# tusen-ai/RangeDet

Measured on AMD Instinct MI355X. Metric: range-image frames/sec (64x2650, 8ch) at 1/2/4/8 GPU; Meta-Kernel HBM GB/s vs peak, higher is better.
Workload: dtype bf16

## Files before the change

__graft_entry__.py:

```python
import os
import sys

ROOT = os.path.dirname(os.path.abspath(__file__))
if ROOT not in sys.path:
    sys.path.insert(0, ROOT)


def build():
    from rangedet_amd import build as rdbuild
    rdbuild.build()
    if rdbuild.packed_swap_lint():
        rdbuild.build(force=True)
    bad = rdbuild.packed_swap_lint()
    assert not bad, "librangedet_hip.so: %d packed-fp32 instructions with swapped source halves, first %r" % (len(bad), bad[0])
    from oracle import cpu_ops
    cpu_ops.build(with_ref=True)
    import rangedet_amd
    from rangedet_amd import lib as rdlib
    rdlib.Lib(rdlib.DEFAULT_PATH)


def smoke():
    import numpy as np
    import torch
    from rangedet_amd import lib as rdlib, synth
    from rangedet_amd.pipeline import RangeDetPipeline
    from oracle import graph_ref, input_ref
    assert torch.cuda.is_available(), "smoke() needs a GPU"
    H, Wr, W, k = 16, 250, 256, 2000
    P = synth.make_weights(seed=18, width=W, cls_bias=-1.0)
    frame = input_ref.make_frame(0, W=Wr, pad_W=W, H=H)
    pipe = RangeDetPipeline(P, dtype=rdlib.RD_F32, feat_size=(H, Wr), pad_field=(H, W), pre_nms_top_n=k, wnms_cap=2048)
    res = pipe.run(frame)
    ref = graph_ref.forward(frame, P, num_fgs=k)
    sc = res["fg_cls_score"].cpu().numpy()
    bx = res["decoded_bbox"].cpu().numpy()
    valid = ref["fg_cls_score"] > 1e-6
    assert np.abs(sc - ref["fg_cls_score"]).max() < 1e-4, np.abs(sc - ref["fg_cls_score"]).max()
    gap = np.abs(np.diff(ref["fg_cls_score"][0]))
    ok = np.ones(k, bool)
    ok[1:] &= gap > 1e-5
    ok[:-1] &= gap > 1e-5
    ok &= valid[0]
    err = np.abs(bx[0][ok] - ref["decoded_bbox"][0][ok]).max()
    assert err < 1e-3, err
    dets, rows, keep, d8 = graph_ref.postprocess(sc[0], bx[0])
    got_keep = res["keep_inds"]
    assert list(got_keep) == list(keep), (len(got_keep), len(keep))
    print("smoke ok: %d detections kept of %d candidates; box maxerr %.2e" % (len(keep), dets.shape[0], err))
    pipe16 = RangeDetPipeline(P, dtype=rdlib.RD_BF16, feat_size=(H, Wr), pad_field=(H, W), pre_nms_top_n=k, wnms_cap=2048,
                              batch=2)
    batch = {kk: np.concatenate([v, v], 0) for kk, v in frame.items()}
    r16 = pipe16.run(batch)
    s16 = r16["fg_cls_score"].cpu().numpy()
    assert np.all(np.diff(s16, axis=1) <= 0) and np.array_equal(s16[0], s16[1])
    d16 = np.abs(s16[0] - ref["fg_cls_score"][0]).max()
    assert d16 < 0.05, d16
    print("smoke ok (bf16, batch 2): sorted-score maxdiff vs fp32 oracle %.3f, kept %s" %
          (d16, [len(f["keep_inds"]) for f in r16["frames"]]))


if __name__ == "__main__":
    build()
    if len(sys.argv) > 1 and sys.argv[1] == "smoke":
        smoke()
```

include/rangedet_hip.h:

```cpp
#ifndef RANGEDET_HIP_H_
#define RANGEDET_HIP_H_
#include <stddef.h>
#include <stdint.h>

#ifdef __cplusplus
extern "C" {
#endif

#define RD_OK 0
#define RD_EINVAL (-1)
#define RD_ESHAPE (-2)
#define RD_EWORKSPACE (-3)
#define RD_EHIP (-4)

#define RD_F32 0
#define RD_BF16 1
#define RD_F16 2

#define RD_RELU_PRE 1
#define RD_ADD 2
#define RD_RELU_POST 4
#define RD_SCALE_FOLDED 8
#define RD_MFMA16 16

int rd_version(void);
const char* rd_last_error_string(void);

int rd_nchw_to_nhwc(const float* src, void* dst, int B, int C, int H, int W, int dst_cstride, int dst_coff,
                    int zero_pad, int dst_dtype, void* stream);
int rd_nhwc_to_nchw(const void* src, float* dst, int B, int C, int H, int W, int src_cstride, int src_coff,
                    int src_dtype, void* stream);

int rd_copy_rows(const void* src, long src_row_bytes, void* dst, long dst_row_bytes, long dst_offset_bytes, long bytes,
                 int rows, void* stream);

size_t rd_conv_packed_bytes(int ntaps, int cin, int cout, int dtype);
int rd_pack_conv_weight_host(const float* w_oihw_host, int cout, int cin, int kh, int kw, int dtype,
                             void* packed_host);
int rd_deconv_phase_taps(int kh, int kw, int stride_w, int pad_w, int phase);
int rd_pack_deconv_weight_host(const float* w_iohw_host, int cin, int cout, int kh, int kw, int stride_w,
                               int pad_w, int phase, int dtype, void* packed_host);
int rd_pack_deconv_weight_folded_host(const float* w_iohw_host, const float* fold_scale_host, int cin, int cout, int kh, int kw,
                                      int stride_w, int pad_w, int phase, int dtype, void* packed_host);

int rd_conv2d_bn_act(const void* x, int x_cstride, int x_coff, const void* w_packed, const float* scale,
                     const float* shift, const void* residual, int r_cstride, int r_coff, void* y,
                     int y_cstride, int y_coff, int B, int H, int Win, int cin, int cout, int kh, int kw,
                     int stride_w, int flags, int dtype, void* stream);
size_t rd_conv3x3_ex_packed_bytes(int cin, int cout, int stride_w, int x_cstride);
int rd_pack_conv3x3_ex_host(const float* w_oihw_host, const float* fold_scale_host, int cout, int cin, int stride_w,
                            int x_cstride, int dtype, void* packed_host);
int rd_pack_conv3x3_m16_host(const float* w_oihw_host, const float* fold_scale_host, int cout, int cin, int dtype, void* packed_host);
int rd_conv3x3_mfma16_ok(int cin, int cout, int stride_w, int W, int fused_output_conv);
size_t rd_conv1x1_sc_packed_bytes(int cin, int cout);
int rd_pack_conv1x1_sc_host(const float* w_oi_host, const float* fold_scale_host, int cout, int cin, int dtype,
                            void* packed_host);
int rd_conv3x3_bn_act_ex(const void* x, int x_cstride, int x_coff, const void* w_packed, const float* scale, const float* shift,
                         const void* residual, int r_cstride, int r_coff, const void* sc_x, int sc_cstride, int sc_coff,
                         int sc_cin, const void* sc_w_packed, void* y, int y_cstride, int y_coff, int B, int H, int Win, int cin,
                         int cout, int stride_w, int flags, int dtype, void* stream);
size_t rd_block64_packed_bytes(int cin);
int rd_pack_block64_host(const float* w1_oihw_host, const float* fold_scale1_host, const float* w2_oihw_host,
                         const float* fold_scale2_host, int cin, int dtype, void* packed_host);
int rd_block64_bn_act(const void* x, int x_cstride, int x_coff, int cin, const void* w_packed, const float* shift1, const float* shift2,
                      const void* sc_w_packed, void* y, int y_cstride, int y_coff, int B, int H, int W, int dtype, void* stream);
int rd_pack_block64_m16_host(const float* w1_oihw_host, const float* fold_scale1_host, const float* w2_oihw_host,
                             const float* fold_scale2_host, int dtype, void* packed_host);
int rd_pack_conv1x1_sc_m16_host(const float* w_oi_host, const float* fold_scale_host, int dtype, void* packed_host);
int rd_block64_m16_bn_act(const void* x, int x_cstride, int x_coff, const void* w_packed, const float* shift1, const float* shift2,
                          const void* sc_w_packed, void* y, int y_cstride, int y_coff, int B, int H, int W, int dtype, void* stream);

size_t rd_head_packed_bytes(void);
int rd_pack_head_weight_host(const float* w, int nout, int cin, int dtype, void* out_host);
size_t rd_head_m16_packed_bytes(void);
int rd_pack_head_weight_m16_host(const float* w, int nout, int cin, int dtype, void* out_host);
int rd_conv2d_bn_act_head_out(const void* x, int x_cstride, int x_coff, const void* w_packed, const float* scale,
                              const float* shift, int B, int H, int W, int cin, int flags, const void* head_w_packed,
                              const float* head_bias, float* out, long out_batch_stride, long n_off, int nout, int dtype,
                              void* stream);

int rd_conv3x3_bn_act_pair(const void* x0, int x0_coff, const void* w0_packed, const float* shift0, void* y0, int y0_coff,
                           const void* x1, int x1_coff, const void* w1_packed, const float* shift1, void* y1, int y1_coff,
                           int x_cstride, int y_cstride, int B, int H, int W, int cin, int flags, int dtype, void* stream);
int rd_conv2d_bn_act_head_out_pair(const void* x0, int x0_coff, const void* w0_packed, const float* shift0, const void* head_w0_packed,
                                   const float* head_bias0, float* out0, long out0_batch_stride, int nout0,
                                   const void* x1, int x1_coff, const void* w1_packed, const float* shift1, const void* head_w1_packed,
                                   const float* head_bias1, float* out1, long out1_batch_stride, int nout1,
                                   int x_cstride, long n_off, int B, int H, int W, int cin, int flags, int dtype, void* stream);

size_t rd_conv3x3_cat_packed_bytes(int cin1, int cin2, int cout);
int rd_pack_conv3x3_cat_host(const float* w, const float* fold_scale, int cout, int cin1, int cin2, int dtype, void* out_host);
int rd_conv3x3_bn_act_cat(const void* x1, int x1_cstride, int x1_coff, int cin1, const void* x2, int x2_cstride, int x2_coff, int cin2,
                          const void* w_packed, const float* shift, void* y, int y_cstride, int y_coff, int B, int H, int W, int cout,
                          int flags, int dtype, void* stream);

int rd_deconv2d_bn_act(const void* x, int x_cstride, int x_coff, const void* w_packed_phase,
                       const float* scale, const float* shift, const void* residual, int r_cstride,
                       int r_coff, void* y, int y_cstride, int y_coff, int B, int H, int Win, int cin,
                       int cout, int kh, int kw, int stride_w, int pad_w, int phase, int flags, int dtype,
                       void* stream);

int rd_deconv2d_all_phases_ok(int kh, int kw, int stride_w, int pad_w, int cout, int dtype);
int rd_deconv2d_bn_act_all(const void* x, int x_cstride, int x_coff, const void* w_packed_all, long w_phase_bytes,
                           const float* shift, const void* residual, int r_cstride, int r_coff, void* y, int y_cstride,
                           int y_coff, int B, int H, int Win, int cin, int cout, int kh, int kw, int stride_w, int pad_w,
                           int flags, int dtype, void* stream);

int rd_deconv2d_phase_pairs_ok(int kh, int kw, int stride_w, int pad_w, int cout, int dtype);
int rd_pack_deconv_phase_pair_host(const void* phase_a, const void* phase_b, int cin, int dtype, void* out);
int rd_deconv2d_bn_act_pairs(const void* x, int x_cstride, int x_coff, const void* w_packed_pairs, long w_pair_bytes,
                             const float* shift2, const void* residual, int r_cstride, int r_coff, void* y, int y_cstride,
                             int y_coff, int B, int H, int Win, int cin, int cout, int kh, int kw, int stride_w, int pad_w,
                             int flags, int dtype, void* stream);

int rd_head_out(const void* x, int x_cstride, int x_coff, const float* w, const float* bias, float* out,
                long out_batch_stride, long n_off, int B, int H, int W, int cin, int nout, int dtype,
                void* stream);

size_t rd_meta_packed_bytes(int dtype);
int rd_pack_meta_host(const float* w0, const float* b0, const float* w1, const float* b1, const float* s1,
                      const float* t1, const float* agg, const float* s2, const float* t2, int dtype,
                      void* packed_host);
int rd_meta_kernel_fwd(const void* data, int d_cstride, int d_coff, const float* coord_nchw,
                       const void* packed, void* y, int y_cstride, int y_coff, int B, int H, int W, int dtype,
                       void* stream);

size_t rd_sorted_foreground_workspace_bytes(long N, long k);
int rd_sorted_foreground(const float* cls_score, const float* bbox_delta, const float* pc, const float* mask,
                         int B, long N, long k, int D, int apply_sigmoid, float* out_score, float* out_delta,
                         float* out_pc, int* out_idx, void* ws, size_t ws_bytes, void* stream);

int rd_decode3d_bbox(const float* bbox_delta, const float* pc, float* out, int B, long N, int box_type,
                     int is_bin, void* stream);

size_t rd_score_filter_workspace_bytes(long n);
int rd_score_filter_dets(const float* scores, const float* boxes10, long n, float min_score, float* dets,
                         int* d_count, void* ws, size_t ws_bytes, void* stream);
int rd_score_filter_dets_batched(const float* scores, long scores_bstride, const float* boxes10, long boxes_bstride,
                                 long n, float min_score, float* dets, long dets_bstride, int* d_count, void* ws,
                                 size_t ws_bytes, int B, void* stream);

#define RD_WNMS_MAX_K 65536
#define RD_TIE_STABLE 0
#define RD_TIE_REFERENCE 1
#define RD_WNMS_DIAG_NO_SKIP 0x100
#define RD_WNMS_DIAG_TILE_W(n) (((n) & 0xff) << 16)
#define RD_WNMS_DIAG_MERGE_LDS(n) (((n) & 0x7f) << 24)
size_t rd_wnms_workspace_bytes(int Kcap);
int rd_wnms_4c(const float* dets, int Kcap, const int* d_count, const int* order, int tie_order, float thresh,
               float thresh_vote, int is3d, int hash_scale, float* out_dets, int* keep, int* d_nkeep, void* ws,
               size_t ws_bytes, void* stream);
int rd_wnms_4c_batched(const float* dets, long dets_bstride, int Kcap, const int* d_count, const int* order,
                       long order_bstride, int tie_order, float thresh, float thresh_vote, int is3d, int hash_scale,
                       float* out_dets, long out_bstride, int* keep, long keep_bstride, int* d_nkeep, void* ws,
                       size_t ws_bytes, int B, void* stream);
int rd_single_overlap(const float* dets_a, const float* dets_b, long n, int is3d, float* out, void* stream);
int rd_wnms_pair_skippable(const float* dets_a, const float* dets_b, long n, unsigned char* out, void* stream);

int rd_edge_atan2f(const float* y, const float* x, long n, float* out, void* stream);

int rd_wnms_order_host(const float* dets_host, int K, int* order_host);

int rd_dets12_to_8(const float* dets12, int Mcap, const int* d_count, float* out8, void* stream);
int rd_dets12_to_8_batched(const float* dets12, long dets12_bstride, int Mcap, const int* d_count, float* out8,
                           long out8_bstride, int B, void* stream);

int rd_rotated_iou_8pt(const float* boxes1, const float* boxes2, float* ious, long n1, long n2, void* stream);
int rd_batch_rotated_iou(const float* proposal, int p_stride, const float* gt_bbox, float* iou_map, int* argmax, int B, long N,
                         int n_gt, void* stream);
int rd_batch_rotated_iou_3d(const float* proposal, int p_stride, const float* gt_bbox7, float* iou_map, int* argmax, int B, long N,
                            int n_gt, void* stream);
int rd_rotated_iou_7(const float* boxes1, const float* boxes2, float* ious, long n1, long n2, void* stream);
int rd_batch_max_iou(const float* proposals, int p_stride, const float* gt8, float* out, long n, int n_gt,
                     void* stream);

size_t rd_nms3d_workspace_bytes(long N, int B);
int rd_gather_keep_scores(const float* score, long score_bstride, int k, const int* keep_idx, int max_keep, float* out, int B,
                          void* stream);
int rd_nms3d(const float* boxes, int B, long N, float iou_thres, int max_keep, int normal_iou, int* keep_idx,
             float* bbox_after_nms, void* ws, size_t ws_bytes, void* stream);

int rd_assign3d_v2(const float* pc, const float* bbox, const float* bbox_center, const float* bbox_radius, const float* mask,
                   const float* is_in_nlz, long N, int M, float max_x, float min_x, float max_y, float min_y, float max_z,
                   float min_z, float max_dist, int* out, void* stream);
size_t rd_get_point_num_workspace_bytes(void);
int rd_get_point_num(const float* bbox_inds, long N, float* out, void* ws, size_t ws_bytes, void* stream);

typedef struct {
  float clip_lo[7], clip_hi[7];
  float mean[8], sd[8];
  float interval_lo[3], interval_hi[3];
} rd_input_norm_t;
int rd_input_transform(const float* range_image, const float* pc_vehicle_frame, const float* inclination,
                       const rd_input_norm_t* norm_host, int B, int H, int W, int Hp, int Wp, float* input_data,
                       float* coord_s1, float* pc_s1, float* pc_s2, float* pc_s4, float* mask_s1, float* mask_s2,
                       float* mask_s4, void* stream);

#define RD_PROF_CONV 0
#define RD_PROF_META 1
#define RD_PROF_HEAD_OUT 2
#define RD_PROF_SORT 3
#define RD_PROF_DECODE 4
#define RD_PROF_WNMS 5
#define RD_PROF_LAYOUT 6
#define RD_PROF_CONV3 7
#define RD_PROF_BLOCK 8
#define RD_PROF_NKINDS 9
int rd_prof_enable(int on);
int rd_prof_reset(void);
int rd_prof_get(int kind, double* total_ms, long* launches);

#ifdef __cplusplus
}
#endif
#endif
```

rangedet_amd/csrc/k_misc.h:

```cpp
#pragma once
#include "rd_common.h"

namespace rd {

template <int DT>
__global__ __launch_bounds__(256) void nchw_to_nhwc_kernel(const float* __restrict__ src, void* __restrict__ dst_, int C,
                                                           long HW, int cs, int coff, int cpad, long total) {
  using E = Elem<DT>;
  typename E::T* dst = (typename E::T*)dst_;
  const int ctot = C + cpad;
  for (long i = blockIdx.x * 256L + threadIdx.x; i < total; i += (long)gridDim.x * 256) {
    long p = i % HW;
    long rest = i / HW;
    int c = (int)(rest % ctot);
    long b = rest / ctot;
    float v = c < C ? src[(b * C + c) * HW + p] : 0.f;
    dst[(b * HW + p) * cs + coff + c] = E::from_f32(v);
  }
}
template <int DT, int NSLOT>
__global__ __launch_bounds__(256) void nchw_to_nhwc_px_kernel(const float* __restrict__ src, void* __restrict__ dst_, int C,
                                                              long HW, int cs, int coff, long npix) {
  using E = Elem<DT>;
  typename E::T* dst = (typename E::T*)dst_;
  for (long i = blockIdx.x * 256L + threadIdx.x; i < npix; i += (long)gridDim.x * 256) {
    const long b = i / HW, p = i - b * HW;
    typename E::T v[NSLOT * E::CH];
#pragma unroll
    for (int c = 0; c < NSLOT * E::CH; ++c) v[c] = E::from_f32(c < C ? src[(b * C + c) * HW + p] : 0.f);
    Slot16 pk[NSLOT];
    memcpy(pk, v, sizeof(pk));
#pragma unroll
    for (int u = 0; u < NSLOT; ++u) *(Slot16*)(dst + i * cs + coff + u * E::CH) = pk[u];
  }
}
template <int DT>
__global__ __launch_bounds__(256) void nhwc_to_nchw_kernel(const void* __restrict__ src_, float* __restrict__ dst, int C,
                                                           long HW, int cs, int coff, long total) {
  using E = Elem<DT>;
  const typename E::T* src = (const typename E::T*)src_;
  for (long i = blockIdx.x * 256L + threadIdx.x; i < total; i += (long)gridDim.x * 256) {
    long p = i % HW;
    long rest = i / HW;
    int c = (int)(rest % C);
    long b = rest / C;
    dst[(b * C + c) * HW + p] = E::to_f32(src[(b * HW + p) * cs + coff + c]);
  }
}

template <int DT, int NOUT>
__global__ __launch_bounds__(256) void head_out_kernel(const void* __restrict__ x_, int cs, int coff,
                                                       const float* __restrict__ w, const float* __restrict__ bias,
                                                       float* __restrict__ out, long out_bs, long n_off, long HW,
                                                       int cin) {
  using E = Elem<DT>;
  using T = typename E::T;
  __shared__ float wl[8 * 128];
  const T* x = (const T*)x_ + (size_t)blockIdx.y * HW * cs;
  for (int i = threadIdx.x; i < NOUT * cin; i += 256) wl[i] = w[i];
  __syncthreads();
  const int sub = threadIdx.x & 7;
  const int per = cin >> 3;
  const long npix_iter = (long)gridDim.x * 32;
  for (long p0 = blockIdx.x * 32L; p0 < HW; p0 += npix_iter) {
    long p = p0 + (threadIdx.x >> 3);
    float acc[NOUT];
#pragma unroll
    for (int o = 0; o < NOUT; ++o) acc[o] = 0.f;
    if (p < HW) {
      const T* px = x + p * cs + coff + sub * per;
      if ((per % E::CH) == 0) {
        for (int c0 = 0; c0 < per; c0 += E::CH) {
          const Slot16 raw = *(const Slot16*)(px + c0);
          T el[E::CH];
          memcpy(el, &raw, 16);
#pragma unroll
          for (int e = 0; e < E::CH; ++e) {
            const float v = E::to_f32(el[e]);
#pragma unroll
            for (int o = 0; o < NOUT; ++o) acc[o] += v * wl[o * cin + sub * per + c0 + e];
          }
        }
      } else {
        for (int c = 0; c < per; ++c) {
          float v = E::to_f32(px[c]);
#pragma unroll
          for (int o = 0; o < NOUT; ++o) acc[o] += v * wl[o * cin + sub * per + c];
        }
      }
    }
#pragma unroll
    for (int o = 0; o < NOUT; ++o) {
      acc[o] += __shfl_xor(acc[o], 1);
      acc[o] += __shfl_xor(acc[o], 2);
      acc[o] += __shfl_xor(acc[o], 4);
    }
    if (p < HW && sub == 0) {
      float* o_ = out + (size_t)blockIdx.y * out_bs + (n_off + p) * NOUT;
#pragma unroll
      for (int o = 0; o < NOUT; ++o) o_[o] = acc[o] + bias[o];
    }
  }
}

template <int NOUT, int DT = RD_BF16>
__global__ __launch_bounds__(256) void head_out_mfma_kernel(const bf16_t* __restrict__ x, int cs, int coff,
                                                            const float* __restrict__ w, const float* __restrict__ bias,
                                                            float* __restrict__ out, long out_bs, long n_off, long HW,
                                                            int cin) {
  __shared__ __attribute__((aligned(16))) unsigned char lds[4 * 8192];
  const int lane = threadIdx.x & 63, m = lane & 31, hi = lane >> 5, wv = threadIdx.x >> 6;
  unsigned char* img = lds + wv * 8192;
  const int nks = cin >> 4, nsl = cin >> 3;
  x += (size_t)blockIdx.y * HW * cs + coff;
  out += (size_t)blockIdx.y * out_bs + n_off * NOUT;
  s16x8 wh[8], wl[8];
#pragma unroll
  for (int ks = 0; ks < 8; ++ks) {
    unsigned short h[8], l[8];
#pragma unroll
    for (int j = 0; j < 8; ++j) {
      const float v = (m < NOUT && ks < nks) ? w[m * cin + ks * 16 + hi * 8 + j] : 0.f;
      h[j] = H16<DT>::from_f32(v);
      l[j] = H16<DT>::from_f32(v - H16<DT>::to_f32(h[j]));
    }
    memcpy(&wh[ks], h, 16);
    memcpy(&wl[ks], l, 16);
  }
  float bs[4];
#pragma unroll
  for (int r = 0; r < 4; ++r) bs[r] = 4 * hi + r < NOUT ? bias[4 * hi + r] : 0.f;
  const long ntile = (HW + 31) / 32;
  const long wave0 = (long)blockIdx.x * 4 + wv, nwave = (long)gridDim.x * 4;
  const int lp = lane >> 4, ls = lane & 15;
  auto load = [&](long tile, Slot16 (&v)[8]) {
#pragma unroll
    for (int it = 0; it < 8; ++it) {
      const long p = min(tile * 32 + it * 4 + lp, HW - 1);
      v[it] = ls < nsl ? *(const Slot16*)(x + p * cs + ls * 8) : Slot16{0u, 0u, 0u, 0u};
    }
  };
  Slot16 cur[8], nxt[8];
  if (wave0 < ntile) load(wave0, cur);
  for (long tile = wave0; tile < ntile; tile += nwave) {
    const bool more = tile + nwave < ntile;
    if (more) load(tile + nwave, nxt);
#pragma unroll
    for (int it = 0; it < 8; ++it) {
      const int pr = it * 4 + lp;
      *(Slot16*)(img + pr * 256 + ((ls ^ (pr & 15)) << 4)) = cur[it];
    }
    __builtin_amdgcn_wave_barrier();
    f32x16 acc;
#pragma unroll
    for (int r = 0; r < 16; ++r) acc[r] = 0.f;
#pragma unroll
    for (int ks = 0; ks < 8; ++ks) {
      const s16x8 b = *(const s16x8*)(img + m * 256 + (((2 * ks + hi) ^ (m & 15)) << 4));
      acc = H16<DT>::mfma(wl[ks], b, acc);
      acc = H16<DT>::mfma(wh[ks], b, acc);
    }
    __builtin_amdgcn_wave_barrier();
    const long p = tile * 32 + m;
    if (p < HW) {
      float* o = out + p * NOUT + 4 * hi;
#pragma unroll
      for (int r = 0; r < 4; ++r)
        if (4 * hi + r < NOUT) o[r] = acc[r] + bs[r];
    }
    if (more) {
#pragma unroll
      for (int it = 0; it < 8; ++it) cur[it] = nxt[it];
    }
  }
}

__global__ __launch_bounds__(256) void decode3d_kernel(const float* __restrict__ delta, const float* __restrict__ pc,
                                                       float* __restrict__ out, long n, int box_type, int is_bin) {
  long idx = blockIdx.x * 256L + threadIdx.x;
  if (idx >= n) return;
  const float* d = delta + idx * box_type;
  float pc_x = pc[idx * 3 + 0], pc_y = pc[idx * 3 + 1], pc_z = pc[idx * 3 + 2];
  float az = atan2f(pc_y, pc_x);
  float ca = cosf(az), sa = sinf(az);
  float dx, dy, width, length, height, z0, yaw_l;
  if (is_bin) {
    dx = d[0];
    dy = d[1];
    width = expf(d[3]);
    length = expf(d[4]);
    height = expf(d[5]);
    float cz = pc_z + d[2];
    z0 = (float)((double)cz - (double)height / 2.0);
    yaw_l = d[6] + az;
  } else {
    dx = d[0] * fabsf(d[0]);
    dy = d[1] * fabsf(d[1]);
    width = expf(d[2]);
    length = expf(d[3]);
    height = expf(d[7]);
    z0 = d[6];
    yaw_l = atan2f(d[5], d[4]) + az;
  }
  float dxl = dx * ca - dy * sa;
  float dyl = dx * sa + dy * ca;
  float cx = pc_x + dxl, cy = pc_y + dyl;
  float sy = sinf(yaw_l), cyw = cosf(yaw_l);
  float hl = (float)(0.5 * (double)length), hw = (float)(0.5 * (double)width);
  float hx[4] = {hl, -hl, -hl, hl};
  float hy[4] = {-hw, -hw, hw, hw};
  float* o = out + idx * 10;
#pragma unroll
  for (int k = 0; k < 4; ++k) {
    o[2 * k] = (hx[k] * cyw - hy[k] * sy) + cx;
    o[2 * k + 1] = (hx[k] * sy + hy[k] * cyw) + cy;
  }
  o[8] = z0;
  o[9] = z0 + height;
}

__global__ __launch_bounds__(256) void filter_count_kernel(const float* __restrict__ scores, long n, float thr,
                                                           int* __restrict__ blk_cnt, long sc_bs, long blk_bs) {
  scores += blockIdx.y * sc_bs;
  blk_cnt += blockIdx.y * blk_bs;
  long i = blockIdx.x * 256L + threadIdx.x;
  int p = (i < n) && (scores[i] > thr);
  unsigned long long m = __ballot(p);
  __shared__ int wc[4];
  if ((threadIdx.x & 63) == 0) wc[threadIdx.x >> 6] = __popcll(m);
  __syncthreads();
  if (threadIdx.x == 0) blk_cnt[blockIdx.x] = wc[0] + wc[1] + wc[2] + wc[3];
}
__global__ __launch_bounds__(256) void filter_scan_kernel(int* __restrict__ blk_cnt, int nblk, int* __restrict__ total,
                                                          long blk_bs) {
  blk_cnt += blockIdx.x * blk_bs;
  total += blockIdx.x;
  __shared__ int part[256];
  __shared__ int carry;
  if (threadIdx.x == 0) carry = 0;
  __syncthreads();
  for (int base = 0; base < nblk; base += 256) {
    int i = base + threadIdx.x;
    int v = i < nblk ? blk_cnt[i] : 0;
    part[threadIdx.x] = v;
    __syncthreads();
    for (int off = 1; off < 256; off <<= 1) {
      int t = threadIdx.x >= off ? part[threadIdx.x - off] : 0;
      __syncthreads();
      part[threadIdx.x] += t;
      __syncthreads();
    }
    int incl = part[threadIdx.x];
    if (i < nblk) blk_cnt[i] = carry + incl - v;
    __syncthreads();
    if (threadIdx.x == 255) carry += incl;
    __syncthreads();
  }
  if (threadIdx.x == 0) *total = carry;
}
__global__ __launch_bounds__(256) void filter_scatter_kernel(const float* __restrict__ scores,
                                                             const float* __restrict__ boxes10, long n, float thr,
                                                             const int* __restrict__ blk_off, float* __restrict__ dets,
                                                             long sc_bs, long box_bs, long blk_bs, long dets_bs) {
  scores += blockIdx.y * sc_bs;
  boxes10 += blockIdx.y * box_bs;
  blk_off += blockIdx.y * blk_bs;
  dets += blockIdx.y * dets_bs;
  long i = blockIdx.x * 256L + threadIdx.x;
  int p = (i < n) && (scores[i] > thr);
  unsigned long long m = __ballot(p);
  __shared__ int wc[4];
  const int wv = threadIdx.x >> 6, ln = threadIdx.x & 63;
  if (ln == 0) wc[wv] = __popcll(m);
  __syncthreads();
  int off = blk_off[blockIdx.x];
  for (int w = 0; w < wv; ++w) off += wc[w];
  if (p) {
    int pos = off + __popcll(m & ((1ull << ln) - 1ull));
    const float* b = boxes10 + i * 10;
    float* d = dets + (size_t)pos * 12;
#pragma unroll
    for (int k = 0; k < 8; ++k) d[k] = b[k];
    d[8] = fdlibm_atan2f(b[1] - b[3], b[0] - b[2]);
    d[9] = b[8];
    d[10] = b[9] - b[8];
    d[11] = scores[i];
  }
}

__global__ __launch_bounds__(256) void dets12_to_8_kernel(const float* __restrict__ d12, int cap, const int* __restrict__ d_count,
                                                          float* __restrict__ o8, long d12_bs, long o8_bs) {
  d12 += blockIdx.y * d12_bs;
  o8 += blockIdx.y * o8_bs;
  int i = blockIdx.x * 256 + threadIdx.x;
  int n = d_count ? min(d_count[blockIdx.y], cap) : cap;
  if (i >= n) return;
  const float* d = d12 + (size_t)i * 12;
  float* o = o8 + (size_t)i * 8;
  o[0] = (d[0] + d[2] + d[4] + d[6]) / 4.f;
  o[1] = (d[1] + d[3] + d[5] + d[7]) / 4.f;
  o[2] = d[9] + d[10] / 2.f;
  float ax = d[2] - d[0], ay = d[3] - d[1];
  float bx = d[2] - d[4], by = d[3] - d[5];
  o[3] = sqrtf(ax * ax + ay * ay);
  o[4] = sqrtf(bx * bx + by * by);
  o[5] = d[10];
  o[6] = d[8];
  o[7] = d[11];
}

__global__ __launch_bounds__(256) void gather_keep_scores_kernel(const float* __restrict__ score, long score_bs, int k,
                                                                 const int* __restrict__ keep, int mk, float* __restrict__ out) {
  const int i = blockIdx.x * 256 + threadIdx.x;
  if (i >= mk) return;
  const int q = keep[(size_t)blockIdx.y * mk + i];
  out[(size_t)blockIdx.y * mk + i] = (q >= 0 && q < k) ? score[blockIdx.y * score_bs + q] : -__builtin_inff();
}

}
```

rangedet_amd/csrc/k_sort.h:

```cpp
#pragma once
#include "rd_common.h"

namespace rd {

constexpr int SORT_TILE = 2048;

__device__ __forceinline__ unsigned desc_key(float f) {
  unsigned u = __float_as_uint(f);
  unsigned asc = u ^ ((u >> 31) ? 0xFFFFFFFFu : 0x80000000u);
  return ~asc;
}
__device__ __forceinline__ float key_to_float(unsigned key) {
  unsigned asc = ~key;
  unsigned u = (asc >> 31) ? (asc ^ 0x80000000u) : ~asc;
  return __uint_as_float(u);
}

__global__ __launch_bounds__(256) void sort_keygen_kernel(const float* __restrict__ score, const float* __restrict__ mask,
                                                          long N, int apply_sigmoid, unsigned* __restrict__ keys,
                                                          unsigned* __restrict__ idx, long ws_stride) {
  long i = blockIdx.x * 256L + threadIdx.x;
  if (i >= N) return;
  const long b = blockIdx.y;
  float s = score[b * N + i];
  if (apply_sigmoid) s = 1.0f / (1.0f + expf(-s));
  if (mask) s = s * mask[b * N + i];
  keys[b * ws_stride + i] = desc_key(s);
  idx[b * ws_stride + i] = (unsigned)i;
}
__global__ __launch_bounds__(256) void sort_keygen_dets_kernel(const float* __restrict__ dets, int cap,
                                                               const int* __restrict__ d_count, unsigned* __restrict__ keys,
                                                               unsigned* __restrict__ idx) {
  int i = blockIdx.x * 256 + threadIdx.x;
  if (i >= cap) return;
  int n = d_count ? min(*d_count, cap) : cap;
  keys[i] = i < n ? desc_key(dets[(size_t)i * 12 + 11]) : 0xFFFFFFFFu;
  idx[i] = (unsigned)i;
}

__global__ __launch_bounds__(256) void sort_hist_kernel(const unsigned* __restrict__ keys, long N, int shift,
                                                        unsigned* __restrict__ hist, unsigned* __restrict__ tot,
                                                        long ws_stride, const unsigned* __restrict__ d_n) {
  if (d_n) N = min(N, (long)d_n[blockIdx.y * ws_stride]);
  keys += blockIdx.y * ws_stride;
  hist += blockIdx.y * ws_stride;
  tot += blockIdx.y * ws_stride;
  __shared__ unsigned h[256];
  h[threadIdx.x] = 0;
  __syncthreads();
  long base = (long)blockIdx.x * SORT_TILE;
  for (int r = 0; r < SORT_TILE / 256; ++r) {
    long i = base + r * 256 + threadIdx.x;
    if (i < N) atomicAdd(&h[(keys[i] >> shift) & 255u], 1u);
  }
  __syncthreads();
  unsigned v = h[threadIdx.x];
  hist[(size_t)blockIdx.x * 256 + threadIdx.x] = v;
  if (v) atomicAdd(&tot[threadIdx.x], v);
}

__global__ __launch_bounds__(256) void sort_scatter_kernel(const unsigned* __restrict__ keys_in,
                                                           const unsigned* __restrict__ idx_in, long N, int shift,
                                                           const unsigned* __restrict__ hist,
                                                           const unsigned* __restrict__ tot,
                                                           unsigned* __restrict__ keys_out, unsigned* __restrict__ idx_out,
                                                           long ws_stride, const unsigned* __restrict__ d_n) {
  if (d_n) {
    N = min(N, (long)d_n[blockIdx.y * ws_stride]);
    if ((long)blockIdx.x * SORT_TILE >= N) return;
  }
  {
    const long o = blockIdx.y * ws_stride;
    keys_in += o; idx_in += o; hist += o; tot += o; keys_out += o; idx_out += o;
  }
  __shared__ unsigned wcnt[4][256];
  __shared__ unsigned gbase[256];
  __shared__ unsigned scan[256];
  const int tid = threadIdx.x, lane = tid & 63, wv = tid >> 6;
  for (int w = 0; w < 4; ++w) wcnt[w][tid] = 0;
  {
    unsigned t = tot[tid];
    scan[tid] = t;
    __syncthreads();
    for (int off = 1; off < 256; off <<= 1) {
      unsigned a = tid >= off ? scan[tid - off] : 0u;
      __syncthreads();
      scan[tid] += a;
      __syncthreads();
    }
    unsigned before = 0;
    for (unsigned b = 0; b < blockIdx.x; ++b) before += hist[(size_t)b * 256 + tid];
    gbase[tid] = scan[tid] - t + before;
  }
  __syncthreads();

  unsigned key[8], id[8], pos[8];
  const long base = (long)blockIdx.x * SORT_TILE + wv * 512;
  const unsigned long long lt = (1ull << lane) - 1ull;
#pragma unroll
  for (int r = 0; r < 8; ++r) {
    long i = base + r * 64 + lane;
    bool valid = i < N;
    key[r] = valid ? keys_in[i] : 0xFFFFFFFFu;
    id[r] = valid ? idx_in[i] : 0u;
    unsigned d = (key[r] >> shift) & 255u;
    unsigned long long peers = __ballot(valid);
#pragma unroll
    for (int bit = 0; bit < 8; ++bit) {
      unsigned long long bm = __ballot(valid && ((d >> bit) & 1u));
      peers &= ((d >> bit) & 1u) ? bm : ~bm;
    }
    unsigned rank = __popcll(peers & lt), cnt = __popcll(peers);
    unsigned prev = wcnt[wv][d];
    pos[r] = prev + rank;
    __builtin_amdgcn_wave_barrier();
    if (valid && rank == 0) wcnt[wv][d] = prev + cnt;
    __builtin_amdgcn_wave_barrier();
  }
  __syncthreads();
  {
    unsigned c0 = wcnt[0][tid], c1 = wcnt[1][tid], c2 = wcnt[2][tid];
    wcnt[0][tid] = 0;
    wcnt[1][tid] = c0;
    wcnt[2][tid] = c0 + c1;
    wcnt[3][tid] = c0 + c1 + c2;
  }
  __syncthreads();
#pragma unroll
  for (int r = 0; r < 8; ++r) {
    long i = base + r * 64 + lane;
    if (i < N) {
      unsigned d = (key[r] >> shift) & 255u;
      unsigned dst = gbase[d] + wcnt[wv][d] + pos[r];
      keys_out[dst] = key[r];
      idx_out[dst] = id[r];
    }
  }
}

__global__ __launch_bounds__(256) void sort_gather_kernel(const unsigned* __restrict__ keys, const unsigned* __restrict__ idx,
                                                          long k, int D, const float* __restrict__ delta,
                                                          const float* __restrict__ pc, float* __restrict__ out_score,
                                                          float* __restrict__ out_delta, float* __restrict__ out_pc,
                                                          int* __restrict__ out_idx, long ws_stride, long N) {
  long i = blockIdx.x * 256L + threadIdx.x;
  if (i >= k) return;
  {
    const long b = blockIdx.y;
    keys += b * ws_stride; idx += b * ws_stride;
    delta += b * N * D; pc += b * N * 3;
    out_score += b * k; out_delta += b * k * D; out_pc += b * k * 3;
    if (out_idx) out_idx += b * k;
  }
  unsigned j = idx[i];
  out_score[i] = key_to_float(keys[i]);
  for (int c = 0; c < D; ++c) out_delta[i * D + c] = delta[(size_t)j * D + c];
  out_pc[i * 3 + 0] = pc[(size_t)j * 3 + 0];
  out_pc[i * 3 + 1] = pc[(size_t)j * 3 + 1];
  out_pc[i * 3 + 2] = pc[(size_t)j * 3 + 2];
  if (out_idx) out_idx[i] = (int)j;
}

constexpr int SEL_BINS = 4096, SEL_SHIFT = 20;
__global__ __launch_bounds__(256) void select_hist_kernel(const unsigned* __restrict__ keys, long N, unsigned* __restrict__ h12,
                                                          long ws_stride) {
  keys += blockIdx.y * ws_stride; h12 += blockIdx.y * ws_stride;
  __shared__ unsigned h[SEL_BINS];
  for (int i = threadIdx.x; i < SEL_BINS; i += 256) h[i] = 0;
  __syncthreads();
  const long base = (long)blockIdx.x * SORT_TILE;
  for (int r = 0; r < SORT_TILE / 256; ++r) {
    const long i = base + r * 256 + threadIdx.x;
    if (i < N) atomicAdd(&h[keys[i] >> SEL_SHIFT], 1u);
  }
  __syncthreads();
  for (int i = threadIdx.x; i < SEL_BINS; i += 256)
    if (h[i]) atomicAdd(&h12[i], h[i]);
}
__global__ __launch_bounds__(256) void select_thresh_kernel(const unsigned* __restrict__ h12, long k, unsigned* __restrict__ sel,
                                                            long ws_stride) {
  h12 += blockIdx.y * ws_stride; sel += blockIdx.y * ws_stride;
  __shared__ unsigned part[256];
  const int tid = threadIdx.x;
  unsigned loc[SEL_BINS / 256], sum = 0;
#pragma unroll
  for (int j = 0; j < SEL_BINS / 256; ++j) { loc[j] = h12[tid * (SEL_BINS / 256) + j]; sum += loc[j]; }
  part[tid] = sum;
  __syncthreads();
  for (int off = 1; off < 256; off <<= 1) {
    const unsigned v = tid >= off ? part[tid - off] : 0u;
    __syncthreads();
    part[tid] += v;
    __syncthreads();
  }
  unsigned before = part[tid] - sum;
  if (tid == 255 && (k == 0 || part[255] < (unsigned)k)) { sel[0] = SEL_BINS - 1; sel[1] = part[255]; }
  if (before < (unsigned)k && before + sum >= (unsigned)k) {
#pragma unroll
    for (int j = 0; j < SEL_BINS / 256; ++j) {
      if (before < (unsigned)k && before + loc[j] >= (unsigned)k) { sel[0] = tid * (SEL_BINS / 256) + j; sel[1] = before + loc[j]; }
      before += loc[j];
    }
  }
}
__global__ __launch_bounds__(256) void select_count_kernel(const unsigned* __restrict__ keys, long N, const unsigned* __restrict__ sel,
                                                           unsigned* __restrict__ cnt, long ws_stride) {
  keys += blockIdx.y * ws_stride; sel += blockIdx.y * ws_stride; cnt += blockIdx.y * ws_stride;
  const unsigned T = sel[0];
  __shared__ unsigned c;
  if (threadIdx.x == 0) c = 0;
  __syncthreads();
  const long base = (long)blockIdx.x * SORT_TILE;
  unsigned mine = 0;
  for (int r = 0; r < SORT_TILE / 256; ++r) {
    const long i = base + r * 256 + threadIdx.x;
    if (i < N && (keys[i] >> SEL_SHIFT) <= T) ++mine;
  }
  if (mine) atomicAdd(&c, mine);
  __syncthreads();
  if (threadIdx.x == 0) cnt[blockIdx.x] = c;
}
__global__ __launch_bounds__(256) void select_compact_kernel(const unsigned* __restrict__ keys_in, const unsigned* __restrict__ idx_in,
                                                             long N, const unsigned* __restrict__ sel,
                                                             const unsigned* __restrict__ cnt, unsigned* __restrict__ keys_out,
                                                             unsigned* __restrict__ idx_out, long ws_stride) {
  {
    const long o = blockIdx.y * ws_stride;
    keys_in += o; idx_in += o; sel += o; cnt += o; keys_out += o; idx_out += o;
  }
  const unsigned T = sel[0];
  __shared__ unsigned wcnt[4][8], sbase;
  const int tid = threadIdx.x, lane = tid & 63, wv = tid >> 6;
  if (tid == 0) {
    unsigned b = 0;
    for (unsigned j = 0; j < blockIdx.x; ++j) b += cnt[j];
    sbase = b;
  }
  const long base = (long)blockIdx.x * SORT_TILE + wv * 512;
  unsigned key[8], id[8];
  unsigned long long m[8];
#pragma unroll
  for (int r = 0; r < 8; ++r) {
    const long i = base + r * 64 + lane;
    const bool valid = i < N;
    key[r] = valid ? keys_in[i] : 0xFFFFFFFFu;
    id[r] = valid ? idx_in[i] : 0u;
    m[r] = __ballot(valid && (key[r] >> SEL_SHIFT) <= T);
    if (lane == 0) wcnt[wv][r] = (unsigned)__popcll(m[r]);
  }
  __syncthreads();
  unsigned off = sbase;
  for (int w = 0; w < wv; ++w)
#pragma unroll
    for (int r = 0; r < 8; ++r) off += wcnt[w][r];
#pragma unroll
  for (int r = 0; r < 8; ++r) {
    if ((m[r] >> lane) & 1ull) {
      const unsigned dst = off + (unsigned)__popcll(m[r] & ((1ull << lane) - 1ull));
      keys_out[dst] = key[r];
      idx_out[dst] = id[r];
    }
    off += (unsigned)__popcll(m[r]);
  }
}

struct SortWs {
  unsigned *keysA, *keysB, *idxA, *idxB, *hist, *tot, *h12, *cnt, *sel;
  int nblk;
};
inline size_t sort_ws_bytes(long N) {
  long nblk = (N + SORT_TILE - 1) / SORT_TILE;
  return (size_t)(4 * N + nblk * 256 + 4 * 256 + SEL_BINS + nblk + 64) * 4 + 256;
}
inline SortWs sort_ws_carve(void* ws, long N) {
  SortWs s;
  s.nblk = (int)((N + SORT_TILE - 1) / SORT_TILE);
  unsigned* p = (unsigned*)ws;
  s.keysA = p; p += N;
  s.keysB = p; p += N;
  s.idxA = p; p += N;
  s.idxB = p; p += N;
  s.hist = p; p += (size_t)s.nblk * 256;
  s.tot = p; p += 4 * 256;
  s.h12 = p; p += SEL_BINS;
  s.cnt = p; p += s.nblk;
  s.sel = p;
  return s;
}
inline int sort_clear(const SortWs& s, hipStream_t st, int nb, long ws_stride, bool with_h12) {
  const size_t bytes = (size_t)(4 * 256 + (with_h12 ? SEL_BINS : 0)) * 4;
  const hipError_t e = nb > 1 ? hipMemset2DAsync(s.tot, (size_t)ws_stride * 4, 0, bytes, nb, st) : hipMemsetAsync(s.tot, 0, bytes, st);
  return e == hipSuccess ? RD_OK : fail(RD_EHIP, "sort: memset");
}
inline int radix_sort_pairs(const SortWs& s, long N, hipStream_t st, int nb = 1, long ws_stride = 0, const unsigned* d_n = nullptr,
                            bool cleared = false) {
  if (!cleared) { int rc = sort_clear(s, st, nb, ws_stride, false); if (rc != RD_OK) return rc; }
  unsigned *ki = s.keysA, *ko = s.keysB, *ii = s.idxA, *io = s.idxB;
  for (int pass = 0; pass < 4; ++pass) {
    hipLaunchKernelGGL(sort_hist_kernel, dim3(s.nblk, nb), dim3(256), 0, st, ki, N, pass * 8, s.hist, s.tot + pass * 256,
                       ws_stride, d_n);
    hipLaunchKernelGGL(sort_scatter_kernel, dim3(s.nblk, nb), dim3(256), 0, st, ki, ii, N, pass * 8, s.hist,
                       s.tot + pass * 256, ko, io, ws_stride, d_n);
    std::swap(ki, ko);
    std::swap(ii, io);
  }
  return check_launch("radix_sort_pairs");
}

inline int radix_topk_pairs(const SortWs& s, long N, long k, hipStream_t st, int nb, long ws_stride, unsigned** rk, unsigned** ri) {
  const bool off = dev_switches().sort_no_select;
  *rk = s.keysA; *ri = s.idxA;
  RD_REQUIRE(k > 0 && k <= N, RD_ESHAPE, "top-k: k %ld of N %ld", k, N);
  if (off || 2 * k > N) return radix_sort_pairs(s, N, st, nb, ws_stride);
  { int rc = sort_clear(s, st, nb, ws_stride, true); if (rc != RD_OK) return rc; }
  hipLaunchKernelGGL(select_hist_kernel, dim3(s.nblk, nb), dim3(256), 0, st, s.keysA, N, s.h12, ws_stride);
  hipLaunchKernelGGL(select_thresh_kernel, dim3(1, nb), dim3(256), 0, st, s.h12, k, s.sel, ws_stride);
  hipLaunchKernelGGL(select_count_kernel, dim3(s.nblk, nb), dim3(256), 0, st, s.keysA, N, s.sel, s.cnt, ws_stride);
  hipLaunchKernelGGL(select_compact_kernel, dim3(s.nblk, nb), dim3(256), 0, st, s.keysA, s.idxA, N, s.sel, s.cnt, s.keysB, s.idxB,
                     ws_stride);
  SortWs v = s;
  v.keysA = s.keysB; v.keysB = s.keysA; v.idxA = s.idxB; v.idxB = s.idxA;
  *rk = s.keysB; *ri = s.idxB;
  return radix_sort_pairs(v, N, st, nb, ws_stride, s.sel + 1, true);
}

}
```

rangedet_amd/csrc/rd_api.hip:

```cpp
#include "k_conv1.h"
#include "k_block.h"
#include "k_assign.h"
#include "k_input.h"
#include "k_nms3d.h"
#include "k_meta.h"
#include "k_misc.h"
#include "k_riou.h"
#include "k_sort.h"
#include "k_wnms.h"

#include <algorithm>
#include <string>
#include <numeric>

using namespace rd;

namespace rd {
inline size_t align256(size_t v) { return (v + 255) & ~(size_t)255; }
inline size_t wnms_ws_bytes(int cap) {
  const size_t nw = (size_t)(cap + 63) / 64;
  return align256((size_t)cap * PREP_F * 4) + 3 * align256((size_t)cap * nw * 8) + 4 * align256((size_t)cap * 4) +
         align256(((size_t)cap + 2) * 8 + 3 * ((size_t)cap / 32 + 2) * 4) + align256(nw * 8) + 256 + align256(sort_ws_bytes(cap)) + 256;
}
inline WnmsWs wnms_ws_carve(void* ws, int cap) {
// ... 340 lines not shown
  return RD_OK;
}
int rd_conv3x3_bn_act_cat(const void* x1, int x1_cstride, int x1_coff, int cin1, const void* x2, int x2_cstride, int x2_coff, int cin2,
                          const void* w_packed, const float* shift, void* y, int y_cstride, int y_coff, int B, int H, int W, int cout,
                          int flags, int dtype, void* stream) {
  RD_REQUIRE(x1 && x2 && w_packed && y && shift, RD_EINVAL, "conv3x3_cat: null pointer");
  RD_REQUIRE(is_h16(dtype), RD_EINVAL, "conv3x3_cat: dtype %d (RD_BF16 or RD_F16)", dtype);
  RD_REQUIRE((flags & RD_SCALE_FOLDED) && !(flags & RD_ADD), RD_EINVAL, "conv3x3_cat: needs RD_SCALE_FOLDED weights, takes no residual");
  RD_REQUIRE(B > 0 && H > 0 && W > 0 && (cout == 64 || cout == 128), RD_ESHAPE, "conv3x3_cat: shape / cout %d", cout);
  RD_REQUIRE(cin1 > 0 && cin1 % 32 == 0 && cin2 > 0 && cin2 % 8 == 0, RD_ESHAPE, "conv3x3_cat: cin1 %d (multiple of 32), cin2 %d (multiple of 8)", cin1, cin2);
  RD_REQUIRE(y_coff >= 0 && y_coff + cout <= y_cstride, RD_ESHAPE, "conv3x3_cat: y channels exceed stride");
  RD_REQUIRE(x1_cstride % 8 == 0 && x1_coff % 8 == 0 && x1_coff + cin1 <= x1_cstride && x2_cstride % 8 == 0 && x2_coff % 8 == 0 &&
             x2_coff + cin2 <= x2_cstride, RD_ESHAPE, "conv3x3_cat: channel stride/offset");
  const DevSwitches& sw_ = dev_switches();
  RD_REQUIRE(!sw_.conv_v1 && sw_.conv_wide && sw_.conv_w30 && (cout == 64 ? sw_.conv_th4 != 3 : (sw_.conv_th4 && sw_.conv_w30 == 2)), RD_ESHAPE,
             "conv3x3_cat: needs the 8 x 32 tile form of the persistent 3x3 kernel (a dev switch turned it off)");
  allow_conv_lds();
  Conv3Src2 s2;
  s2.x = x2; s2.cs = x2_cstride; s2.co = x2_coff; s2.cin1 = cin1; s2.cin2 = cin2;
  return launch_conv3(x1, x1_cstride, x1_coff, w_packed, nullptr, shift, nullptr, 0, 0, y, y_cstride, y_coff, B, H, W, cin1 + cin2, cout, flags,
                      1, (hipStream_t)stream, 0, nullptr, dtype, nullptr, nullptr, &s2, conv3_body_cat(cin1, cin2, true));
}

size_t rd_head_packed_bytes(void) { return 16384; }
int rd_pack_head_weight_host(const float* w, int nout, int cin, int dtype, void* out_host) {
  RD_REQUIRE(w && out_host, RD_EINVAL, "pack_head_weight: null pointer");
  RD_REQUIRE(is_h16(dtype), RD_EINVAL, "pack_head_weight: dtype %d (RD_BF16 or RD_F16)", dtype);
  RD_REQUIRE(nout >= 1 && nout <= 8 && cin >= 1 && cin <= 128, RD_ESHAPE, "pack_head_weight: nout %d (1..8), cin %d (1..128)", nout, cin);
  pack_head_frag(w, nout, cin, out_host, dtype);
  return RD_OK;
}
size_t rd_head_m16_packed_bytes(void) { return 8192; }
int rd_pack_head_weight_m16_host(const float* w, int nout, int cin, int dtype, void* out_host) {
  RD_REQUIRE(w && out_host, RD_EINVAL, "pack_head_weight_m16: null pointer");
  RD_REQUIRE(is_h16(dtype), RD_EINVAL, "pack_head_weight_m16: dtype %d (RD_BF16 or RD_F16)", dtype);
  RD_REQUIRE(nout >= 1 && nout <= 8 && cin >= 1 && cin <= 128, RD_ESHAPE, "pack_head_weight_m16: nout %d (1..8), cin %d (1..128)", nout, cin);
  pack_head_frag16(w, nout, cin, out_host, dtype);
  return RD_OK;
}
int rd_conv2d_bn_act_head_out(const void* x, int x_cstride, int x_coff, const void* w_packed, const float* scale,
                              const float* shift, int B, int H, int W, int cin, int flags, const void* head_w_packed,
                              const float* head_bias, float* out, long out_batch_stride, long n_off, int nout, int dtype,
                              void* stream) {
  RD_REQUIRE(x && w_packed && head_w_packed && head_bias && out, RD_EINVAL, "conv2d_head_out: null pointer");
  RD_REQUIRE(is_h16(dtype), RD_EINVAL, "conv2d_head_out: dtype %d (RD_BF16 or RD_F16)", dtype);
  RD_REQUIRE(B > 0 && H > 0 && W > 0 && cin > 0 && nout >= 1 && nout <= 8, RD_ESHAPE, "conv2d_head_out: shape / nout %d (1..8)", nout);
  RD_REQUIRE(!(flags & RD_ADD), RD_EINVAL, "conv2d_head_out: no residual in a head tower");
  RD_REQUIRE(x_cstride % 8 == 0 && x_coff % 8 == 0 && x_coff + cin_slots(cin, RD_BF16) * 8 <= x_cstride, RD_ESHAPE,
             "conv2d_head_out: x channel stride/offset");
  RD_REQUIRE(!dev_switches().conv_v1, RD_EINVAL, "conv2d_head_out: needs the persistent 3x3 kernel (RD_CONV_V1 is set)");
  RD_REQUIRE(!conv3_body_small(cin, (flags & RD_SCALE_FOLDED) != 0), RD_ESHAPE, "conv2d_head_out: cin %d (the packed image of a conv with <= 16 input channels is not this launch form's)", cin);
  const bool m16 = (flags & RD_MFMA16) != 0;
  RD_REQUIRE(!m16 || ((flags & RD_SCALE_FOLDED) && conv3_mfma16_ok(cin, 128, 1, W, true)), RD_ESHAPE,
             "conv2d_head_out: RD_MFMA16 (weights of rd_pack_conv3x3_m16_host) is not a launch form for cin %d at width %d (rd_conv3x3_mfma16_ok)", cin, W);
  allow_conv_lds();
  Conv3Args h;
  memset(&h, 0, sizeof(h));
  h.hw = (const unsigned char*)head_w_packed; h.hb = head_bias; h.ho = out; h.ho_bs = out_batch_stride; h.ho_off = n_off; h.hn = nout;
  return launch_conv3(x, x_cstride, x_coff, w_packed, scale, shift, nullptr, 0, 0, nullptr, 128, 0, B, H, W, cin, 128, flags & ~RD_MFMA16, 1,
                      (hipStream_t)stream, 0, &h, dtype, nullptr, nullptr, nullptr, m16 ? C3_BODY_M16 : 0);
}

static int pair_checks(const char* fn, const void* x0, const void* x1, const void* w0, const void* w1, const float* shift0,
                       const float* shift1, int x_cstride, int x0_coff, int x1_coff, int B, int H, int W, int cin, int flags,
                       int dtype) {
  RD_REQUIRE(x0 && x1 && w0 && w1 && shift0 && shift1, RD_EINVAL, "%s: null pointer", fn);
  RD_REQUIRE(is_h16(dtype), RD_EINVAL, "%s: dtype %d (RD_BF16 or RD_F16)", fn, dtype);
  RD_REQUIRE(B > 0 && H > 0 && W > 0 && cin > 0, RD_ESHAPE, "%s: shape", fn);
  RD_REQUIRE((flags & RD_SCALE_FOLDED) && !(flags & RD_ADD), RD_EINVAL, "%s: needs RD_SCALE_FOLDED weights, takes no residual", fn);
  RD_REQUIRE(x_cstride % 8 == 0 && x0_coff % 8 == 0 && x1_coff % 8 == 0 && x0_coff + cin_slots(cin, RD_BF16) * 8 <= x_cstride &&
             x1_coff + cin_slots(cin, RD_BF16) * 8 <= x_cstride, RD_ESHAPE, "%s: x channel stride/offset", fn);
  RD_REQUIRE(!dev_switches().conv_v1, RD_EINVAL, "%s: needs the persistent 3x3 kernel (RD_CONV_V1 is set)", fn);
  RD_REQUIRE(cin > 16, RD_ESHAPE, "%s: cin %d (more than 16 input channels)", fn, cin);
  return RD_OK;
}
int rd_conv3x3_bn_act_pair(const void* x0, int x0_coff, const void* w0_packed, const float* shift0, void* y0, int y0_coff,
                           const void* x1, int x1_coff, const void* w1_packed, const float* shift1, void* y1, int y1_coff,
                           int x_cstride, int y_cstride, int B, int H, int W, int cin, int flags, int dtype, void* stream) {
  if (int rc = pair_checks("conv3x3_pair", x0, x1, w0_packed, w1_packed, shift0, shift1, x_cstride, x0_coff, x1_coff, B, H, W, cin, flags, dtype)) return rc;
  RD_REQUIRE(y0 && y1, RD_EINVAL, "conv3x3_pair: null output");
  RD_REQUIRE(y0_coff >= 0 && y1_coff >= 0 && y0_coff + 128 <= y_cstride && y1_coff + 128 <= y_cstride, RD_ESHAPE, "conv3x3_pair: y channels exceed stride");
  allow_conv_lds();
  if (!conv3_pair_eligible(128, flags, W)) {
    if (int rc = launch_conv3(x0, x_cstride, x0_coff, w0_packed, nullptr, shift0, nullptr, 0, 0, y0, y_cstride, y0_coff, B, H, W, cin, 128,
                              flags, 1, (hipStream_t)stream, 0, nullptr, dtype)) return rc;
    return launch_conv3(x1, x_cstride, x1_coff, w1_packed, nullptr, shift1, nullptr, 0, 0, y1, y_cstride, y1_coff, B, H, W, cin, 128, flags, 1,
                        (hipStream_t)stream, 0, nullptr, dtype);
  }
  Conv3Second g;
  memset(&g, 0, sizeof(g));
  g.x = x1; g.x_co = x1_coff; g.w = w1_packed; g.shift = shift1; g.y = y1; g.y_co = y1_coff;
  return launch_conv3(x0, x_cstride, x0_coff, w0_packed, nullptr, shift0, nullptr, 0, 0, y0, y_cstride, y0_coff, B, H, W, cin, 128, flags, 1,
                      (hipStream_t)stream, 0, nullptr, dtype, &g);
}
int rd_conv2d_bn_act_head_out_pair(const void* x0, int x0_coff, const void* w0_packed, const float* shift0, const void* head_w0_packed,
                                   const float* head_bias0, float* out0, long out0_batch_stride, int nout0,
                                   const void* x1, int x1_coff, const void* w1_packed, const float* shift1, const void* head_w1_packed,
                                   const float* head_bias1, float* out1, long out1_batch_stride, int nout1,
                                   int x_cstride, long n_off, int B, int H, int W, int cin, int flags, int dtype, void* stream) {
  if (int rc = pair_checks("conv2d_head_out_pair", x0, x1, w0_packed, w1_packed, shift0, shift1, x_cstride, x0_coff, x1_coff, B, H, W, cin, flags, dtype)) return rc;
  RD_REQUIRE(head_w0_packed && head_w1_packed && head_bias0 && head_bias1 && out0 && out1, RD_EINVAL, "conv2d_head_out_pair: null pointer");
  RD_REQUIRE(nout0 >= 1 && nout0 <= 8 && nout1 >= 1 && nout1 <= 8, RD_ESHAPE, "conv2d_head_out_pair: nout %d / %d (1..8)", nout0, nout1);
  allow_conv_lds();
  Conv3Args h;
  memset(&h, 0, sizeof(h));
  h.hw = (const unsigned char*)head_w0_packed; h.hb = head_bias0; h.ho = out0; h.ho_bs = out0_batch_stride; h.ho_off = n_off; h.hn = nout0;
  if (!conv3_pair_eligible(128, flags, W, true)) {
    if (int rc = launch_conv3(x0, x_cstride, x0_coff, w0_packed, nullptr, shift0, nullptr, 0, 0, nullptr, 128, 0, B, H, W, cin, 128, flags, 1,
                              (hipStream_t)stream, 0, &h, dtype)) return rc;
    h.hw = (const unsigned char*)head_w1_packed; h.hb = head_bias1; h.ho = out1; h.ho_bs = out1_batch_stride; h.hn = nout1;
    return launch_conv3(x1, x_cstride, x1_coff, w1_packed, nullptr, shift1, nullptr, 0, 0, nullptr, 128, 0, B, H, W, cin, 128, flags, 1,
                        (hipStream_t)stream, 0, &h, dtype);
  }
  Conv3Second g;
  memset(&g, 0, sizeof(g));
  g.x = x1; g.x_co = x1_coff; g.w = w1_packed; g.shift = shift1;
  g.hw = head_w1_packed; g.hb = head_bias1; g.ho = out1; g.ho_bs = out1_batch_stride; g.hn = nout1;
  return launch_conv3(x0, x_cstride, x0_coff, w0_packed, nullptr, shift0, nullptr, 0, 0, nullptr, 128, 0, B, H, W, cin, 128, flags, 1,
                      (hipStream_t)stream, 0, &h, dtype, &g);
}

int rd_deconv2d_bn_act(const void* x, int x_cstride, int x_coff, const void* w_packed_phase, const float* scale,
                       const float* shift, const void* residual, int r_cstride, int r_coff, void* y, int y_cstride,
                       int y_coff, int B, int H, int Win, int cin, int cout, int kh, int kw, int stride_w, int pad_w,
                       int phase, int flags, int dtype, void* stream) {
  RD_REQUIRE(x && w_packed_phase && y, RD_EINVAL, "deconv2d: null pointer");
  RD_REQUIRE(kh == 3, RD_ESHAPE, "deconv2d: kernel height %d (only 3, pad 1, stride 1)", kh);
  RD_REQUIRE(stride_w >= 1 && phase >= 0 && phase < stride_w, RD_EINVAL, "deconv2d: phase %d of stride %d", phase, stride_w);
  RD_REQUIRE(y_coff >= 0 && y_coff + cout <= y_cstride, RD_ESHAPE, "deconv2d: y channels exceed stride");
  const int Wout = (Win - 1) * stride_w - 2 * pad_w + kw;
  RD_REQUIRE(Wout > phase, RD_ESHAPE, "deconv2d: empty phase");
  const int Wq = (Wout - phase + stride_w - 1) / stride_w;
  TapList tl = deconv_taps_sorted(kh, kw, stride_w, pad_w, phase);
  RD_REQUIRE(tl.n >= 1 && tl.n <= 9, RD_ESHAPE, "deconv2d: %d taps per phase unsupported", tl.n);
  allow_conv_lds();
  if (deconv_embeds_3x3(tl)) {
    const int ts = deconv_tap_set(tl);
    if (!ts) tl = conv_taps(3, 3);
    if (is_h16(dtype) && Wout == stride_w * Win && (cout == 64 || cout == 128) && !dev_switches().conv_v1 &&
        conv3_has_form(dtype, (flags & RD_SCALE_FOLDED) != 0)) {
      const bf16_t* r = (const bf16_t*)residual;
      return launch_conv3(x, x_cstride, x_coff, w_packed_phase, scale, shift, r, r_cstride * stride_w,
                          r_coff + phase * r_cstride, y, y_cstride * stride_w, y_coff + phase * y_cstride, B, H, Win, cin,
                          cout, flags, 1, (hipStream_t)stream, ts, nullptr, dtype);
    }
  }
  RD_REQUIRE(!(flags & RD_SCALE_FOLDED), RD_ESHAPE, "deconv2d: RD_SCALE_FOLDED needs the persistent 3x3 kernel (bf16, cout 64/128, "
             "taps inside the 3x3 window, Wout == stride_w * Win)");
  return launch_conv(tl, x, x_cstride, x_coff, w_packed_phase, scale, shift, residual, r_cstride, r_coff, y,
                     y_cstride, y_coff, B, H, Win, Wq, Wout, cin, cout, 1, stride_w, phase, flags, dtype,
                     (hipStream_t)stream);
}

int rd_deconv2d_all_phases_ok(int kh, int kw, int stride_w, int pad_w, int cout, int dtype) {
  if (!is_h16(dtype) || kh != 3 || stride_w < 2 || stride_w > 8 || !conv3_phases_eligible(cout, RD_SCALE_FOLDED)) return 0;
  if (kw - 2 * pad_w != stride_w) return 0;
  for (int p = 0; p < stride_w; ++p)
    if (!deconv_tap_set(deconv_taps_sorted(kh, kw, stride_w, pad_w, p))) return 0;
  return 1;
}
int rd_deconv2d_bn_act_all(const void* x, int x_cstride, int x_coff, const void* w_packed_all, long w_phase_bytes,
                           const float* shift, const void* residual, int r_cstride, int r_coff, void* y, int y_cstride,
                           int y_coff, int B, int H, int Win, int cin, int cout, int kh, int kw, int stride_w, int pad_w,
                           int flags, int dtype, void* stream) {
  RD_REQUIRE(x && w_packed_all && y, RD_EINVAL, "deconv2d_all: null pointer");
  RD_REQUIRE(is_h16(dtype), RD_EINVAL, "deconv2d_all: dtype %d (RD_BF16 or RD_F16)", dtype);
  RD_REQUIRE(flags & RD_SCALE_FOLDED, RD_EINVAL, "deconv2d_all: needs RD_SCALE_FOLDED weights (rd_pack_deconv_weight_folded_host)");
  RD_REQUIRE(!((flags & RD_ADD) && !residual), RD_EINVAL, "deconv2d_all: RD_ADD without residual");
  RD_REQUIRE(B > 0 && H > 0 && Win > 0 && cin > 0, RD_ESHAPE, "deconv2d_all: shape");
  RD_REQUIRE(y_coff >= 0 && y_coff + cout <= y_cstride, RD_ESHAPE, "deconv2d_all: y channels exceed stride");
  RD_REQUIRE(x_cstride % 8 == 0 && x_coff % 8 == 0 && x_coff + cin_slots(cin, RD_BF16) * 8 <= x_cstride, RD_ESHAPE, "deconv2d_all: x channel stride/offset");
  RD_REQUIRE(rd_deconv2d_all_phases_ok(kh, kw, stride_w, pad_w, cout, dtype), RD_ESHAPE,
             "deconv2d_all: kernel (%d,%d) stride %d pad %d cout %d is not a set of two-column 3x2 phases (use rd_deconv2d_bn_act per phase)",
             kh, kw, stride_w, pad_w, cout);
  RD_REQUIRE(w_phase_bytes >= (long)conv_packed_bytes(6, cin, cout, RD_BF16) && w_phase_bytes % 16 == 0, RD_EINVAL, "deconv2d_all: w_phase_bytes");
  allow_conv_lds();
  Conv3Phases ph;
  ph.nph = stride_w; ph.ts_mask = 0; ph.y_pc = y_cstride; ph.r_pc = r_cstride; ph.w_pb = w_phase_bytes;
  for (int p = 0; p < stride_w; ++p)
    if (deconv_tap_set(deconv_taps_sorted(kh, kw, stride_w, pad_w, p)) == 2) ph.ts_mask |= 1 << p;
  return launch_conv3(x, x_cstride, x_coff, w_packed_all, nullptr, shift, residual, r_cstride * stride_w, r_coff, y, y_cstride * stride_w,
                      y_coff, B, H, Win, cin, cout, flags, 1, (hipStream_t)stream, 3, nullptr, dtype, nullptr, &ph);
}

int rd_deconv2d_phase_pairs_ok(int kh, int kw, int stride_w, int pad_w, int cout, int dtype) {
  if (!rd_deconv2d_all_phases_ok(kh, kw, stride_w, pad_w, cout, dtype) || cout != 64 || stride_w % 2) return 0;
  if (!rd_deconv2d_all_phases_ok(kh, kw, stride_w, pad_w, 128, dtype)) return 0;
  for (int p = 0; p < stride_w; p += 2)
    if (deconv_tap_set(deconv_taps_sorted(kh, kw, stride_w, pad_w, p)) != deconv_tap_set(deconv_taps_sorted(kh, kw, stride_w, pad_w, p + 1))) return 0;
  return 1;
}
int rd_pack_deconv_phase_pair_host(const void* phase_a, const void* phase_b, int cin, int dtype, void* out) {
  RD_REQUIRE(phase_a && phase_b && out, RD_EINVAL, "pack_deconv_pair: null pointer");
  RD_REQUIRE(is_h16(dtype) && cin > 0, RD_EINVAL, "pack_deconv_pair: dtype %d / cin %d", dtype, cin);
  const size_t body = conv_packed_body_bytes(6, cin, 64, RD_BF16), blocks = body / 2048;
  for (size_t i = 0; i < blocks; ++i) {
    memcpy((unsigned char*)out + i * 4096, (const unsigned char*)phase_a + i * 2048, 2048);
    memcpy((unsigned char*)out + i * 4096 + 2048, (const unsigned char*)phase_b + i * 2048, 2048);
  }
  memset((unsigned char*)out + 2 * body, 0, 2 * RD_CONV_TAIL);
  return RD_OK;
}
int rd_deconv2d_bn_act_pairs(const void* x, int x_cstride, int x_coff, const void* w_packed_pairs, long w_pair_bytes,
                             const float* shift2, const void* residual, int r_cstride, int r_coff, void* y, int y_cstride,
                             int y_coff, int B, int H, int Win, int cin, int cout, int kh, int kw, int stride_w, int pad_w,
                             int flags, int dtype, void* stream) {
  RD_REQUIRE(x && w_packed_pairs && y && shift2, RD_EINVAL, "deconv2d_pairs: null pointer");
  RD_REQUIRE(is_h16(dtype), RD_EINVAL, "deconv2d_pairs: dtype %d (RD_BF16 or RD_F16)", dtype);
  RD_REQUIRE(flags & RD_SCALE_FOLDED, RD_EINVAL, "deconv2d_pairs: needs RD_SCALE_FOLDED weights (rd_pack_deconv_weight_folded_host)");
  RD_REQUIRE(!((flags & RD_ADD) && !residual), RD_EINVAL, "deconv2d_pairs: RD_ADD without residual");
  RD_REQUIRE(B > 0 && H > 0 && Win > 0 && cin > 0, RD_ESHAPE, "deconv2d_pairs: shape");
  RD_REQUIRE(x_cstride % 8 == 0 && x_coff % 8 == 0 && x_coff + cin_slots(cin, RD_BF16) * 8 <= x_cstride, RD_ESHAPE, "deconv2d_pairs: x channel stride/offset");
  RD_REQUIRE(rd_deconv2d_phase_pairs_ok(kh, kw, stride_w, pad_w, cout, dtype), RD_ESHAPE,
             "deconv2d_pairs: kernel (%d,%d) stride %d pad %d cout %d has no phase pairs (use rd_deconv2d_bn_act_all)", kh, kw, stride_w, pad_w, cout);
  RD_REQUIRE(y_cstride == cout && y_coff == 0 && (!residual || (r_cstride == cout && r_coff == 0)), RD_ESHAPE,
             "deconv2d_pairs: the output / residual must be dense %d-channel tensors (two phases are one 128-channel write)", cout);
  RD_REQUIRE(w_pair_bytes >= (long)conv_packed_bytes(6, cin, 2 * cout, RD_BF16) && w_pair_bytes % 16 == 0, RD_EINVAL, "deconv2d_pairs: w_pair_bytes");
  allow_conv_lds();
  Conv3Phases ph;
  ph.nph = stride_w / 2; ph.ts_mask = 0; ph.y_pc = 2 * cout; ph.r_pc = 2 * cout; ph.w_pb = w_pair_bytes;
  for (int p = 0; p < stride_w; p += 2)
    if (deconv_tap_set(deconv_taps_sorted(kh, kw, stride_w, pad_w, p)) == 2) ph.ts_mask |= 1 << (p / 2);
  return launch_conv3(x, x_cstride, x_coff, w_packed_pairs, nullptr, shift2, residual, r_cstride * stride_w, r_coff, y, y_cstride * stride_w,
                      y_coff, B, H, Win, cin, 2 * cout, flags, 1, (hipStream_t)stream, 3, nullptr, dtype, nullptr, &ph);
}

int rd_head_out(const void* x, int x_cstride, int x_coff, const float* w, const float* bias, float* out,
                long out_batch_stride, long n_off, int B, int H, int W, int cin, int nout, int dtype, void* stream) {
  RD_REQUIRE(x && w && bias && out, RD_EINVAL, "head_out: null pointer");
  RD_REQUIRE(cin % 8 == 0 && cin <= 128 && cin > 0, RD_ESHAPE, "head_out: cin %d (multiple of 8, <= 128)", cin);
  RD_REQUIRE(nout == 1 || nout == 7 || nout == 8, RD_ESHAPE, "head_out: nout %d not in {1,7,8}", nout);
  RD_REQUIRE(dtype == RD_F32 || is_h16(dtype), RD_EINVAL, "head_out: dtype");
  hipStream_t st = (hipStream_t)stream;
  const long HW = (long)H * W;
  dim3 grid((unsigned)std::min<long>((HW + 31) / 32, 4096), B);
  ProfScope ps(RD_PROF_HEAD_OUT, st);
  if (is_h16(dtype) && nout > 1 && cin % 16 == 0 && x_cstride % 8 == 0 && x_coff % 8 == 0) {
    dim3 g2((unsigned)std::min<long>((HW + 127) / 128, 2048), B);
#define RD_HOM(NO, DT_) hipLaunchKernelGGL((head_out_mfma_kernel<NO, DT_>), g2, dim3(256), 0, st, (const bf16_t*)x, x_cstride, x_coff, w, bias, out, out_batch_stride, n_off, HW, cin)
    if (dtype == RD_F16) { if (nout == 7) RD_HOM(7, RD_F16); else RD_HOM(8, RD_F16); }
    else { if (nout == 7) RD_HOM(7, RD_BF16); else RD_HOM(8, RD_BF16); }
#undef RD_HOM
    return check_launch("head_out");
  }
#define RD_HO(DT, NO) hipLaunchKernelGGL((head_out_kernel<DT, NO>), grid, dim3(256), 0, st, x, x_cstride, x_coff, w, bias, out, out_batch_stride, n_off, HW, cin)
  if (dtype == RD_BF16) { if (nout == 1) RD_HO(RD_BF16, 1); else if (nout == 7) RD_HO(RD_BF16, 7); else RD_HO(RD_BF16, 8); }
  else if (dtype == RD_F16) { if (nout == 1) RD_HO(RD_F16, 1); else if (nout == 7) RD_HO(RD_F16, 7); else RD_HO(RD_F16, 8); }
  else { if (nout == 1) RD_HO(RD_F32, 1); else if (nout == 7) RD_HO(RD_F32, 7); else RD_HO(RD_F32, 8); }
#undef RD_HO
  return check_launch("head_out");
}

size_t rd_meta_packed_bytes(int dtype) { return meta_layout(dtype).total; }
int rd_pack_meta_host(const float* w0, const float* b0, const float* w1, const float* b1, const float* s1,
                      const float* t1, const float* agg, const float* s2, const float* t2, int dtype, void* out) {
  RD_REQUIRE(w0 && b0 && w1 && b1 && s1 && t1 && agg && s2 && t2 && out, RD_EINVAL, "pack_meta: null pointer");
  RD_REQUIRE(dtype == RD_F32 || is_h16(dtype), RD_EINVAL, "pack_meta: dtype");
  pack_meta(w0, b0, w1, b1, s1, t1, agg, s2, t2, dtype, out);
  return RD_OK;
}
int rd_meta_kernel_fwd(const void* data, int d_cstride, int d_coff, const float* coord_nchw, const void* packed,
                       void* y, int y_cstride, int y_coff, int B, int H, int W, int dtype, void* stream) {
  RD_REQUIRE(data && coord_nchw && packed && y, RD_EINVAL, "meta_kernel: null pointer");
  RD_REQUIRE(B > 0 && H > 0 && W > 0, RD_ESHAPE, "meta_kernel: empty shape");
  RD_REQUIRE(dtype == RD_F32 || is_h16(dtype), RD_EINVAL, "meta_kernel: dtype");
  const int ch = ch_per_slot(dtype);
  RD_REQUIRE(d_cstride % ch == 0 && d_coff % ch == 0 && y_cstride % ch == 0 && y_coff % ch == 0, RD_ESHAPE,
             "meta_kernel: channel strides/offsets must be 16-byte multiples");
  RD_REQUIRE(d_coff + 64 <= d_cstride && y_coff + 64 <= y_cstride, RD_ESHAPE, "meta_kernel: needs 64 channels");
  hipStream_t st = (hipStream_t)stream;
  MetaArgs a;
  a.data = data; a.d_cs = d_cstride; a.d_co = d_coff; a.coord = coord_nchw; a.packed = (const unsigned char*)packed;
  a.y = y; a.y_cs = y_cstride; a.y_co = y_coff; a.B = B; a.H = H; a.W = W;
  constexpr int WAVES = 8;
  a.tiles_h = (H + WAVES - 1) / WAVES;
  a.tiles_w = (W + 31) / 32;
  a.ntiles = B * a.tiles_h * a.tiles_w;
  a.r0 = 0; a.m0 = a.m1 = a.m2 = 0;
  const size_t consts = 9 * 64 * 4 * 2 + 1024;
  ProfScope ps(RD_PROF_META, st);
  if (is_h16(dtype)) {
    const size_t lds = meta_layout(dtype).wbytes + consts + (size_t)(WAVES + 2) * 34 * 128 + 4096;
    static std::atomic<unsigned long long> seen{0};
    once_per_device(seen, [] { allow_big_lds(meta16_kernel<WAVES, RD_BF16>); allow_big_lds(meta16_kernel<WAVES, RD_F16>); });
    const dim3 mgrid(std::min(a.ntiles, conv_num_cus())), mblock(WAVES * 64);
    const int strips = a.tiles_w * B;
    a.r0 = dev_switches().conv_xcd && strips % 8 == 0 ? 8 : strips;
    RD_REQUIRE((unsigned long long)a.ntiles * (unsigned)std::max(a.r0, std::max(a.tiles_h, a.tiles_w)) < (1ull << 32), RD_ESHAPE,
               "meta_kernel: %d tiles exceed the range of the tile decode", a.ntiles);
    a.m0 = meta_magic(a.r0); a.m1 = meta_magic(a.tiles_h); a.m2 = meta_magic(a.tiles_w);
    RD_REQUIRE((long)H * W < (1l << 23) && (long)H * W * d_cstride < (1l << 31) && W < (1 << 23) && d_cstride < (1 << 23), RD_ESHAPE,
               "meta_kernel: image of %d x %d pixels x %d channels exceeds the 32-bit halo offsets", H, W, d_cstride);
    if (dtype == RD_F16) hipLaunchKernelGGL((meta16_kernel<WAVES, RD_F16>), mgrid, mblock, lds, st, a);
    else hipLaunchKernelGGL((meta16_kernel<WAVES, RD_BF16>), mgrid, mblock, lds, st, a);
  } else {
    const size_t lds = consts + (size_t)(WAVES + 2) * 34 * 256;
    static std::atomic<unsigned long long> seen32{0};
    once_per_device(seen32, [] { allow_big_lds(meta_kernel<RD_F32, WAVES>); });
    hipLaunchKernelGGL((meta_kernel<RD_F32, WAVES>), dim3(std::min(a.ntiles, 512)), dim3(WAVES * 64), lds, st, a);
  }
  return check_launch("meta_kernel");
}

size_t rd_sorted_foreground_workspace_bytes(long N, long k) { (void)k; return (sort_ws_bytes(N) + 256 + 255) & ~(size_t)255; }
int rd_sorted_foreground(const float* cls_score, const float* bbox_delta, const float* pc, const float* mask, int B,
                         long N, long k, int D, int apply_sigmoid, float* out_score, float* out_delta, float* out_pc,
                         int* out_idx, void* ws, size_t ws_bytes, void* stream) {
  RD_REQUIRE(cls_score && bbox_delta && pc && out_score && out_delta && out_pc && ws, RD_EINVAL, "sorted_foreground: null pointer");
  RD_REQUIRE(B > 0 && N > 0 && k > 0 && D > 0, RD_ESHAPE, "sorted_foreground: empty shape");
  RD_REQUIRE(N >= k, RD_ESHAPE, "sorted_foreground: N (%ld) < num_fgs (%ld)", N, k);
  RD_REQUIRE(N < (1L << 31), RD_ESHAPE, "sorted_foreground: N too large");
  RD_REQUIRE(ws_bytes >= rd_sorted_foreground_workspace_bytes(N, k), RD_EWORKSPACE, "sorted_foreground: workspace %zu < %zu",
             ws_bytes, rd_sorted_foreground_workspace_bytes(N, k));
  hipStream_t st = (hipStream_t)stream;
  void* wsa = (void*)(((uintptr_t)ws + 255) & ~(uintptr_t)255);
  SortWs s = sort_ws_carve(wsa, N);
  ProfScope ps(RD_PROF_SORT, st);
  const size_t per = rd_sorted_foreground_workspace_bytes(N, k);
  const bool wide = ws_bytes >= per * (size_t)B;
  const long stride = wide ? (long)(per / 4) : 0;
  const int nb = wide ? B : 1;
  for (int b0 = 0; b0 < B; b0 += nb) {
    hipLaunchKernelGGL(sort_keygen_kernel, dim3((unsigned)((N + 255) / 256), nb), dim3(256), 0, st, cls_score + (size_t)b0 * N,
                       mask ? mask + (size_t)b0 * N : nullptr, N, apply_sigmoid, s.keysA, s.idxA, stride);
    unsigned *rk, *ri;
    int rc = radix_topk_pairs(s, N, k, st, nb, stride, &rk, &ri);
    if (rc != RD_OK) return rc;
    hipLaunchKernelGGL(sort_gather_kernel, dim3((unsigned)((k + 255) / 256), nb), dim3(256), 0, st, rk, ri, k, D,
                       bbox_delta + (size_t)b0 * N * D, pc + (size_t)b0 * N * 3, out_score + (size_t)b0 * k,
                       out_delta + (size_t)b0 * k * D, out_pc + (size_t)b0 * k * 3, out_idx ? out_idx + (size_t)b0 * k : nullptr,
                       stride, N);
  }
  return check_launch("sorted_foreground");
}

int rd_decode3d_bbox(const float* bbox_delta, const float* pc, float* out, int B, long N, int box_type, int is_bin,
                     void* stream) {
  RD_REQUIRE(bbox_delta && pc && out, RD_EINVAL, "decode3d: null pointer");
  RD_REQUIRE(B > 0 && N > 0, RD_ESHAPE, "decode3d: empty shape");
  RD_REQUIRE((is_bin && box_type == 7) || (!is_bin && box_type == 8), RD_ESHAPE,
             "decode3d: box_type %d with is_bin=%d (8 for regular, 7 for bin)", box_type, is_bin);
  hipStream_t st = (hipStream_t)stream;
  const long n = (long)B * N;
  ProfScope ps(RD_PROF_DECODE, st);
  hipLaunchKernelGGL(decode3d_kernel, dim3((unsigned)((n + 255) / 256)), dim3(256), 0, st, bbox_delta, pc, out, n, box_type, is_bin);
  return check_launch("decode3d");
}

size_t rd_score_filter_workspace_bytes(long n) { return (size_t)((n + 255) / 256 + 8) * 4 + 256; }
int rd_score_filter_dets_batched(const float* scores, long scores_bstride, const float* boxes10, long boxes_bstride,
                                 long n, float min_score, float* dets, long dets_bstride, int* d_count, void* ws,
                                 size_t ws_bytes, int B, void* stream) {
  RD_REQUIRE(scores && boxes10 && dets && d_count && ws, RD_EINVAL, "score_filter: null pointer");
  RD_REQUIRE(n > 0 && B > 0, RD_ESHAPE, "score_filter: empty input");
  const size_t per = rd_score_filter_workspace_bytes(n);
  RD_REQUIRE(ws_bytes >= per * (size_t)B, RD_EWORKSPACE, "score_filter: workspace %zu < %zu", ws_bytes, per * (size_t)B);
  hipStream_t st = (hipStream_t)stream;
  int* blk = (int*)(((uintptr_t)ws + 255) & ~(uintptr_t)255);
  const int nblk = (int)((n + 255) / 256);
  const long blk_bs = nblk + 8;
  ProfScope ps(RD_PROF_WNMS, st);
  hipLaunchKernelGGL(filter_count_kernel, dim3(nblk, B), dim3(256), 0, st, scores, n, min_score, blk, scores_bstride, blk_bs);
  hipLaunchKernelGGL(filter_scan_kernel, dim3(B), dim3(256), 0, st, blk, nblk, d_count, blk_bs);
  hipLaunchKernelGGL(filter_scatter_kernel, dim3(nblk, B), dim3(256), 0, st, scores, boxes10, n, min_score, blk, dets,
                     scores_bstride, boxes_bstride, blk_bs, dets_bstride);
  return check_launch("score_filter");
}
int rd_score_filter_dets(const float* scores, const float* boxes10, long n, float min_score, float* dets, int* d_count,
                         void* ws, size_t ws_bytes, void* stream) {
  return rd_score_filter_dets_batched(scores, 0, boxes10, 0, n, min_score, dets, 0, d_count, ws, ws_bytes, 1, stream);
}

size_t rd_wnms_workspace_bytes(int Kcap) { return Kcap > 0 ? wnms_ws_bytes(Kcap) : 0; }
int rd_wnms_4c_batched(const float* dets, long dets_bstride, int Kcap, const int* d_count, const int* order,
                       long order_bstride, int tie_order, float thresh, float thresh_vote, int is3d, int hash_scale,
                       float* out_dets, long out_bstride, int* keep, long keep_bstride, int* d_nkeep, void* ws,
                       size_t ws_bytes, int B, void* stream) {
  RD_REQUIRE(dets && out_dets && keep && d_nkeep && ws, RD_EINVAL, "wnms_4c: null pointer");
  RD_REQUIRE(Kcap > 0 && Kcap <= RD_WNMS_MAX_K, RD_ESHAPE, "wnms_4c: Kcap %d not in [1, %d]", Kcap, RD_WNMS_MAX_K);
  RD_REQUIRE(B > 0, RD_ESHAPE, "wnms_4c: batch %d", B);
  const int diag = tie_order & ~0xff;
  tie_order &= 0xff;
  RD_REQUIRE(tie_order == RD_TIE_STABLE || tie_order == RD_TIE_REFERENCE, RD_EINVAL, "wnms_4c: tie_order %d", tie_order);
  RD_REQUIRE(!(diag & ~(RD_WNMS_DIAG_NO_SKIP | (0xff << 16) | (0x7f << 24))), RD_EINVAL, "wnms_4c: unknown diagnostic bits 0x%x", diag);
  const size_t per = rd_wnms_workspace_bytes(Kcap);
  RD_REQUIRE(ws_bytes >= per * (size_t)B, RD_EWORKSPACE, "wnms_4c: workspace %zu < %zu", ws_bytes, per * (size_t)B);
  RD_REQUIRE(order || B == 1 || tie_order == RD_TIE_REFERENCE, RD_EINVAL,
             "wnms_4c: the batched call needs an explicit processing order or RD_TIE_REFERENCE");
  hipStream_t st = (hipStream_t)stream;
  static std::atomic<unsigned long long> seen_lds{0};
  once_per_device(seen_lds, [] {
    allow_big_lds(wnms_tie_order_kernel); allow_big_lds(wnms_scan_kernel); allow_big_lds(wnms_scan4_kernel); allow_big_lds(wnms_merge_kernel);
  });
  WnmsWs w = wnms_ws_carve(ws, Kcap);
  ProfScope ps(RD_PROF_WNMS, st);
  WnmsBatch bs;
  bs.dets = dets_bstride; bs.order = order_bstride; bs.prep = (long)(per / 4); bs.words = (long)(per / 8);
  bs.ints = (long)(per / 4); bs.keep = keep_bstride; bs.out = out_bstride;
  const int* ord = order;
  if (!ord && tie_order == RD_TIE_REFERENCE) {
    const size_t lds = TIE_STACK_BYTES + (Kcap <= TIE_LDS_K ? (size_t)Kcap * 8 + 3 * ((size_t)Kcap / 32 + 2) * 4 : 0);
    hipLaunchKernelGGL(wnms_tie_order_kernel, dim3(1, 1, B), dim3(256), lds, st, dets, Kcap, d_count, w.order, bs, (long)(per / 4),
                       w.scratch);
    ord = w.order;
    bs.order = (long)(per / 4);
  } else if (!ord) {
    void* swa = (void*)(((uintptr_t)w.sort_ws + 255) & ~(uintptr_t)255);
    SortWs s = sort_ws_carve(swa, Kcap);
    hipLaunchKernelGGL(sort_keygen_dets_kernel, dim3((Kcap + 255) / 256), dim3(256), 0, st, dets, Kcap, d_count, s.keysA, s.idxA);
    int rc = radix_sort_pairs(s, Kcap, st);
    if (rc != RD_OK) return rc;
    if (hipMemcpyAsync(w.order, s.idxA, (size_t)Kcap * 4, hipMemcpyDeviceToDevice, st) != hipSuccess)
      return rd::fail(RD_EHIP, "wnms_4c: order copy");
    ord = w.order;
    bs.order = 0;
  }
  const int nb = (Kcap + 63) / 64;
  hipLaunchKernelGGL(wnms_prep_kernel, dim3((Kcap + 255) / 256, 1, B), dim3(256), 0, st, dets, ord, Kcap, d_count, w.prep, bs,
                     (float)hash_scale, w.novf);
  const int e_tw = (diag >> 16) & 0xff, e_ml = (diag >> 24) & 0x7f;
  const int tile_w = std::min(w.nwcap, e_tw ? std::max(1, e_tw) : 256);
  const size_t scan_lds = ((size_t)w.nwcap + (size_t)64 * tile_w) * 8;
  const int R1 = 256, nb1 = R1 / 64;
  const bool one_round = dev_switches().wnms_one_round;
  const bool two = Kcap >= 4 * R1 && !one_round;
  const int ct = dev_switches().wnms_ct == 32 ? 32 : dev_switches().wnms_ct == 16 ? 16 : 8;
  const int pgrid = std::min(2048, std::max(64, nb * (64 / ct) * std::min(nb, 16)));
  const int allow_skip = thresh >= 1e-3f && thresh_vote >= 1e-3f && !is3d && !dev_switches().wnms_no_skip && !(diag & RD_WNMS_DIAG_NO_SKIP);
  auto pairs = [&](const int* rows, const int* nrows, const unsigned long long* supp, int rb_end) {
    auto k = dev_switches().wnms_bal ? (ct == 8 ? wnms_pairs_kernel<8, true> : ct == 16 ? wnms_pairs_kernel<16, true> : wnms_pairs_kernel<32, true>)
                                     : (ct == 8 ? wnms_pairs_kernel<8, false> : ct == 16 ? wnms_pairs_kernel<16, false> : wnms_pairs_kernel<32, false>);
    hipLaunchKernelGGL(k, dim3(pgrid, 1, B), dim3(64), 0, st, w.prep, Kcap, d_count, thresh, thresh_vote, is3d, w.thr, w.vote,
                       w.nwcap, bs, rows, nrows, supp, 0, rb_end, allow_skip);
  };
  pairs(nullptr, nullptr, nullptr, two ? nb1 : nb);
  const bool scan4 = w.nwcap <= 128 && !e_tw && !dev_switches().wnms_scan1;
  const int tile_words = 64 * 128;
  const size_t scan4_lds = ((size_t)w.nwcap + tile_words) * 8;
  auto scan = [&](int c_begin, int c_end, unsigned long long* state) {
    if (scan4)
      hipLaunchKernelGGL(wnms_scan4_kernel, dim3(1, 1, B), dim3(256), scan4_lds, st, w.thr, w.snap, Kcap, d_count, w.nwcap, ord,
                         w.keep_q, keep, d_nkeep, bs, c_begin, c_end, state, tile_words);
    else
      hipLaunchKernelGGL(wnms_scan_kernel, dim3(1, 1, B), dim3(64), scan_lds, st, w.thr, w.snap, Kcap, d_count, w.nwcap, ord,
                         w.keep_q, keep, d_nkeep, bs, c_begin, c_end, state, tile_w);
  };
  scan(0, two ? nb1 : nb, two ? w.supp_state : (unsigned long long*)nullptr);
  if (two) {
    hipLaunchKernelGGL(wnms_alive_kernel, dim3(1, 1, B), dim3(256), 0, st, w.supp_state, Kcap, d_count, R1, w.alive, w.nalive, bs);
    pairs((const int*)w.alive, (const int*)w.nalive, (const unsigned long long*)w.supp_state, 0);
    scan(nb1, nb, w.supp_state);
  }
  const int lds_cap = std::min(Kcap + 2, e_ml ? std::max(4, e_ml) : 2048);
  hipLaunchKernelGGL(wnms_merge_kernel, dim3(std::min(Kcap, 4096), 1, B), dim3(64), (size_t)lds_cap * 8, st, dets, ord, w.vote,
                     w.snap, Kcap, d_count, w.nwcap, w.keep_q, d_nkeep, out_dets, bs, lds_cap, w.ovf, w.novf);
  if (Kcap + 2 > lds_cap)
    hipLaunchKernelGGL(wnms_merge_big_kernel, dim3(1, 1, B), dim3(64), 0, st, dets, ord, w.vote, w.snap, Kcap, d_count, w.nwcap,
                       w.keep_q, out_dets, bs, (const int*)w.ovf, (const int*)w.novf, w.scratch);
  return check_launch("wnms_4c");
}
int rd_wnms_4c(const float* dets, int Kcap, const int* d_count, const int* order, int tie_order, float thresh,
               float thresh_vote, int is3d, int hash_scale, float* out_dets, int* keep, int* d_nkeep, void* ws,
               size_t ws_bytes, void* stream) {
  return rd_wnms_4c_batched(dets, 0, Kcap, d_count, order, 0, tie_order, thresh, thresh_vote, is3d, hash_scale, out_dets, 0,
                            keep, 0, d_nkeep, ws, ws_bytes, 1, stream);
}
int rd_single_overlap(const float* dets_a, const float* dets_b, long n, int is3d, float* out, void* stream) {
  RD_REQUIRE(n >= 0 && (n == 0 || (dets_a && dets_b && out)), RD_EINVAL, "single_overlap: bad arguments");
  if (n == 0) return RD_OK;
  hipLaunchKernelGGL(single_overlap_kernel, dim3((unsigned)((n + 63) / 64)), dim3(64), 0, (hipStream_t)stream, dets_a, dets_b, n,
                     is3d, out);
  return check_launch("single_overlap");
}
int rd_wnms_pair_skippable(const float* dets_a, const float* dets_b, long n, unsigned char* out, void* stream) {
  RD_REQUIRE(dets_a && dets_b && out && n >= 0, RD_EINVAL, "wnms_pair_skippable: null pointer");
  if (n == 0) return RD_OK;
  hipLaunchKernelGGL(pair_skippable_kernel, dim3((unsigned)((n + 63) / 64)), dim3(64), 0, (hipStream_t)stream, dets_a, dets_b, n, out);
  return check_launch("wnms_pair_skippable");
}
namespace rd {
__global__ void atan2f_kernel(const float* y, const float* x, long n, float* out) {
  const long i = (long)blockIdx.x * blockDim.x + threadIdx.x;
  if (i < n) out[i] = fdlibm_atan2f(y[i], x[i]);
}
}
int rd_edge_atan2f(const float* y, const float* x, long n, float* out, void* stream) {
  RD_REQUIRE(y && x && out && n >= 0, RD_EINVAL, "edge_atan2f: null pointer");
  if (n == 0) return RD_OK;
  hipLaunchKernelGGL(atan2f_kernel, dim3((unsigned)((n + 255) / 256)), dim3(256), 0, (hipStream_t)stream, y, x, n, out);
  return check_launch("edge_atan2f");
}
int rd_wnms_order_host(const float* dets_host, int K, int* order_host) {
  RD_REQUIRE(K >= 0 && (K == 0 || (dets_host && order_host)), RD_EINVAL, "wnms_order_host: bad arguments");
  std::iota(order_host, order_host + K, 0);
  std::sort(order_host, order_host + K, [&](int i, int j) { return dets_host[i * 12 + 11] > dets_host[j * 12 + 11]; });
  return RD_OK;
}

int rd_dets12_to_8_batched(const float* dets12, long dets12_bstride, int Mcap, const int* d_count, float* out8,
                           long out8_bstride, int B, void* stream) {
  RD_REQUIRE(dets12 && out8, RD_EINVAL, "dets12_to_8: null pointer");
  RD_REQUIRE(Mcap > 0 && B > 0, RD_ESHAPE, "dets12_to_8: empty input");
  hipLaunchKernelGGL(dets12_to_8_kernel, dim3((Mcap + 255) / 256, B), dim3(256), 0, (hipStream_t)stream, dets12, Mcap, d_count,
                     out8, dets12_bstride, out8_bstride);
  return check_launch("dets12_to_8");
}
int rd_dets12_to_8(const float* dets12, int Mcap, const int* d_count, float* out8, void* stream) {
  return rd_dets12_to_8_batched(dets12, 0, Mcap, d_count, out8, 0, 1, stream);
}

int rd_gather_keep_scores(const float* score, long score_bstride, int k, const int* keep_idx, int max_keep, float* out, int B,
                          void* stream) {
  RD_REQUIRE(score && keep_idx && out, RD_EINVAL, "gather_keep_scores: null pointer");
  RD_REQUIRE(k > 0 && max_keep > 0 && B > 0, RD_ESHAPE, "gather_keep_scores: empty input");
  hipLaunchKernelGGL(gather_keep_scores_kernel, dim3((max_keep + 255) / 256, B), dim3(256), 0, (hipStream_t)stream, score,
                     score_bstride, k, keep_idx, max_keep, out);
  return check_launch("gather_keep_scores");
}

int rd_rotated_iou_8pt(const float* boxes1, const float* boxes2, float* ious, long n1, long n2, void* stream) {
  RD_REQUIRE(boxes1 && boxes2 && ious, RD_EINVAL, "rotated_iou: null pointer");
  RD_REQUIRE(n1 > 0 && n2 > 0, RD_ESHAPE, "rotated_iou: empty input");
  hipLaunchKernelGGL(riou8_kernel, dim3((unsigned)((n1 * n2 + 255) / 256)), dim3(256), 0, (hipStream_t)stream, boxes1, boxes2, ious, n1, n2);
  return check_launch("rotated_iou_8pt");
}
int rd_batch_rotated_iou(const float* proposal, int p_stride, const float* gt_bbox, float* iou_map, int* argmax, int B, long N,
                         int n_gt, void* stream) {
  RD_REQUIRE(proposal && gt_bbox && iou_map, RD_EINVAL, "batch_rotated_iou: null pointer");
  RD_REQUIRE(B > 0 && B <= 65535 && N > 0 && n_gt > 0 && n_gt <= 256 && p_stride >= 8, RD_ESHAPE,
             "batch_rotated_iou: B %d, N %ld, n_gt %d (<= 256), proposal row %d floats (>= 8)", B, N, n_gt, p_stride);
  hipLaunchKernelGGL(batch_riou_kernel, dim3((unsigned)((N + 255) / 256), B), dim3(256), 0, (hipStream_t)stream, proposal, p_stride,
                     N * (long)p_stride, gt_bbox, (long)n_gt * 8, iou_map, argmax, N, n_gt);
  return check_launch("batch_rotated_iou");
}
int rd_rotated_iou_7(const float* boxes1, const float* boxes2, float* ious, long n1, long n2, void* stream) {
  RD_REQUIRE(boxes1 && boxes2 && ious, RD_EINVAL, "rotated_iou_7: null pointer");
  if (n1 * n2 == 0) return RD_OK;
  hipLaunchKernelGGL(riou7_kernel, dim3((unsigned)((n1 * n2 + 255) / 256)), dim3(256), 0, (hipStream_t)stream, boxes1, boxes2, ious, n1, n2);
  return check_launch("rotated_iou_7");
}
int rd_batch_rotated_iou_3d(const float* proposal, int p_stride, const float* gt_bbox7, float* iou_map, int* argmax, int B, long N,
                            int n_gt, void* stream) {
  RD_REQUIRE(proposal && gt_bbox7 && iou_map, RD_EINVAL, "batch_rotated_iou_3d: null pointer");
  RD_REQUIRE(B > 0 && N > 0 && p_stride >= 10, RD_ESHAPE, "batch_rotated_iou_3d: proposal rows need the 8 corners + z0, z1 (stride %d)", p_stride);
  RD_REQUIRE(n_gt >= 1 && n_gt <= 256, RD_ESHAPE, "batch_rotated_iou_3d: n_gt %d (1..256; the config pads to 200)", n_gt);
  ProfScope ps(RD_PROF_DECODE, (hipStream_t)stream);
  hipLaunchKernelGGL(batch_riou3d_kernel, dim3((unsigned)((N + 255) / 256), B), dim3(256), 0, (hipStream_t)stream, proposal, p_stride,
                     (long)N * p_stride, gt_bbox7, (long)n_gt * 7, iou_map, argmax, N, n_gt);
  return check_launch("batch_rotated_iou_3d");
}
int rd_batch_max_iou(const float* proposals, int p_stride, const float* gt8, float* out, long n, int n_gt, void* stream) {
  return rd_batch_rotated_iou(proposals, p_stride, gt8, out, nullptr, 1, n, n_gt, stream);
}

size_t rd_nms3d_workspace_bytes(long N, int B) {
  if (N <= 0 || N > (1 << 18) || B <= 0) return 0;
  return nms3d_frame_bytes((int)N) * (size_t)B;
}
int rd_nms3d(const float* boxes, int B, long N, float iou_thres, int max_keep, int normal_iou, int* keep_idx,
             float* bbox_after_nms, void* ws, size_t ws_bytes, void* stream) {
  RD_REQUIRE(boxes && keep_idx && bbox_after_nms && ws, RD_EINVAL, "nms3d: null pointer");
  RD_REQUIRE(B > 0 && B <= 65535 && N > 0 && N <= (1 << 18) && max_keep > 0, RD_ESHAPE, "nms3d: B %d, N %ld (<= 262144), max_keep %d", B, N, max_keep);
  RD_REQUIRE(ws_bytes >= rd_nms3d_workspace_bytes(N, B), RD_EWORKSPACE, "nms3d: workspace %zu < %zu bytes", ws_bytes, rd_nms3d_workspace_bytes(N, B));
  RD_REQUIRE(((uintptr_t)ws & 7) == 0, RD_EINVAL, "nms3d: workspace must be 8-byte aligned");
  Nms3dArgs a;
  a.boxes = boxes; a.ws = (unsigned char*)ws; a.ws_frame = nms3d_frame_bytes((int)N);
  a.keep = keep_idx; a.out = bbox_after_nms;
  a.N = (int)N; a.ncw = (int)((N + 63) / 64); a.max_keep = max_keep; a.normal_iou = normal_iou ? 1 : 0; a.thresh = iou_thres;
  hipStream_t st = (hipStream_t)stream;
  ProfScope ps(RD_PROF_WNMS, st);
  const int gi = (std::max(std::max(a.ncw, max_keep), 2) + 255) / 256;
  hipLaunchKernelGGL(nms3d_init_kernel, dim3(gi, B), dim3(256), 0, st, a);
  for (int r0 = 0, blk = 64; r0 < a.N; r0 += blk, blk = std::min(2 * blk, NMS3D_RB)) {
    const int rows = std::min(blk, a.N - r0);
    hipLaunchKernelGGL(nms3d_pairs_kernel, dim3((a.N + NMS3D_SEG - 1) / NMS3D_SEG, rows, B), dim3(256), 0, st, a, r0);
    hipLaunchKernelGGL(nms3d_scan_kernel, dim3(B), dim3(256), (size_t)a.ncw * 8, st, a, r0, blk);
  }
  return check_launch("nms3d");
}

int rd_assign3d_v2(const float* pc, const float* bbox, const float* bbox_center, const float* bbox_radius, const float* mask,
                   const float* is_in_nlz, long N, int M, float max_x, float min_x, float max_y, float min_y, float max_z,
                   float min_z, float max_dist, int* out, void* stream) {
  RD_REQUIRE(pc && bbox && bbox_center && bbox_radius && mask && is_in_nlz && out, RD_EINVAL, "assign3d_v2: null pointer");
  RD_REQUIRE(N > 0 && M > 0 && M <= ASSIGN_MAX_BOXES, RD_ESHAPE, "assign3d_v2: N %ld, M %d (1..%d)", N, M, ASSIGN_MAX_BOXES);
  AssignArgs a;
  a.pc = pc; a.bbox = bbox; a.center = bbox_center; a.radius = bbox_radius; a.mask = mask; a.nlz = is_in_nlz; a.out = out;
  a.N = N; a.M = M;
  a.max_x = max_x; a.min_x = min_x; a.max_y = max_y; a.min_y = min_y; a.max_z = max_z; a.min_z = min_z; a.max_dist = max_dist;
  hipLaunchKernelGGL(assign3d_kernel, dim3((unsigned)((N + 255) / 256)), dim3(256), (size_t)M * 14 * 4, (hipStream_t)stream, a);
  return check_launch("assign3d_v2");
}
size_t rd_get_point_num_workspace_bytes(void) { return POINT_NUM_MAX_BOXES * sizeof(int); }
int rd_get_point_num(const float* bbox_inds, long N, float* out, void* ws, size_t ws_bytes, void* stream) {
  RD_REQUIRE(bbox_inds && out && ws, RD_EINVAL, "get_point_num: null pointer");
  RD_REQUIRE(N > 0, RD_ESHAPE, "get_point_num: N %ld", N);
  RD_REQUIRE(ws_bytes >= rd_get_point_num_workspace_bytes(), RD_EWORKSPACE, "get_point_num: workspace %zu < %zu bytes", ws_bytes,
             rd_get_point_num_workspace_bytes());
  hipStream_t st = (hipStream_t)stream;
  if (hipMemsetAsync(ws, 0, rd_get_point_num_workspace_bytes(), st) != hipSuccess) return fail(RD_EHIP, "get_point_num: memset failed");
  const unsigned g = (unsigned)std::min<long>((N + 255) / 256, 1024);
  hipLaunchKernelGGL(point_num_count_kernel, dim3(g), dim3(256), 0, st, bbox_inds, N, (int*)ws);
  hipLaunchKernelGGL(point_num_gather_kernel, dim3((unsigned)((N + 255) / 256)), dim3(256), 0, st, bbox_inds, N, (const int*)ws, out);
  return check_launch("get_point_num");
}

int rd_input_transform(const float* range_image, const float* pc_vehicle_frame, const float* inclination,
                       const rd_input_norm_t* norm_host, int B, int H, int W, int Hp, int Wp, float* input_data,
                       float* coord_s1, float* pc_s1, float* pc_s2, float* pc_s4, float* mask_s1, float* mask_s2,
                       float* mask_s4, void* stream) {
  RD_REQUIRE(range_image && pc_vehicle_frame && inclination && norm_host && input_data && coord_s1 && pc_s1 && pc_s2 && pc_s4 &&
                 mask_s1 && mask_s2 && mask_s4, RD_EINVAL, "input_transform: null pointer");
  RD_REQUIRE(B > 0 && H > 2 && W > 2 && Hp >= H && Wp >= W && Wp % 4 == 0, RD_ESHAPE,
             "input_transform: shape (%d,%d,%d) -> (%d,%d)", B, H, W, Hp, Wp);
  InputArgs a;
  a.ri = range_image; a.pc = pc_vehicle_frame; a.incl = inclination;
  a.data = input_data; a.coord = coord_s1;
  a.pcs[0] = pc_s1; a.pcs[1] = pc_s2; a.pcs[2] = pc_s4;
  a.msk[0] = mask_s1; a.msk[1] = mask_s2; a.msk[2] = mask_s4;
  a.B = B; a.H = H; a.W = W; a.Hp = Hp; a.Wp = Wp;
  a.n = *norm_host;
  hipStream_t st = (hipStream_t)stream;
  ProfScope ps(RD_PROF_LAYOUT, st);
  hipLaunchKernelGGL(input_transform_kernel, dim3((unsigned)(((long)Hp * Wp + 255) / 256), B), dim3(256), 0, st, a);
  return check_launch("input_transform");
}

int rd_dev_conv_trace_set(unsigned long long* device_buf, long nwords) {
  if (device_buf && nwords < (long)CONV_TRACE_CAP) return RD_EINVAL;
  conv_trace_slot() = device_buf;
  return RD_OK;
}
int rd_dev_conv_trace_read(unsigned long long* out, long n) {
  if (!conv_trace_buf() || n > (long)CONV_TRACE_CAP) return RD_EINVAL;
  return hipMemcpy(out, conv_trace_buf(), n * 8, hipMemcpyDeviceToHost) == hipSuccess ? RD_OK : RD_EHIP;
}
// ... 25 lines not shown
```

rangedet_amd/csrc/rd_common.h:

```cpp
#pragma once
#include <hip/hip_runtime.h>

#include <cstdarg>
#include <cstdint>
#include <cstdio>
#include <cstdlib>
#include <cstring>
#include <mutex>
#include <type_traits>
#include <vector>

#include <atomic>
#include "../../include/rangedet_hip.h"

namespace rd {

inline char* err_buf() {
  static thread_local char buf[512] = "";
  return buf;
}
inline int fail(int code, const char* fmt, ...) {
  va_list ap;
  va_start(ap, fmt);
  vsnprintf(err_buf(), 512, fmt, ap);
  va_end(ap);
  return code;
}
#define RD_REQUIRE(cond, code, ...) \
  do {                              \
    if (!(cond)) return rd::fail(code, __VA_ARGS__); \
  } while (0)

inline int check_launch(const char* what) {
  hipError_t e = hipGetLastError();
  if (e != hipSuccess) return fail(RD_EHIP, "%s: %s", what, hipGetErrorString(e));
  return RD_OK;
}

struct DevSwitches {
  bool conv_v1;
  int conv_th4;
  int conv_w30, conv_head30;
  int conv_hb3;
  int conv_wide;
  int conv_xcd;
  int conv_body;
  bool sort_no_select;
  bool wnms_one_round;
  int wnms_bal;
  bool wnms_scan1;
  int wnms_ct;
  bool wnms_no_skip;
};
constexpr DevSwitches kDevSwitchDefaults = {false, 1, 2, 1, 1, 1, 1, 1, false, false, 0, false, 8, false};
#ifdef RD_DEV_SWITCHES
inline const DevSwitches& dev_switches() {
  static const DevSwitches s = [] {
    auto num = [](const char* name, int dflt) { const char* e = getenv(name); return e ? atoi(e) : dflt; };
    DevSwitches d = kDevSwitchDefaults;
    d.conv_v1 = getenv("RD_CONV_V1") != nullptr;
    d.conv_th4 = num("RD_CONV_TH4", 1);
    d.conv_w30 = num("RD_CONV_W30", 2);
    d.conv_head30 = num("RD_CONV_HEAD30", 1);
    d.conv_hb3 = num("RD_CONV_HB3", 1);
    d.conv_wide = num("RD_CONV_WIDE", 1);
    d.conv_body = num("RD_CONV_BODY", 1);
    d.conv_xcd = num("RD_CONV_XCD", 1);
    d.sort_no_select = getenv("RD_SORT_NO_SELECT") != nullptr;
    d.wnms_one_round = getenv("RD_WNMS_ONE_ROUND") != nullptr;
    d.wnms_ct = num("RD_WNMS_CT", 8);
    d.wnms_scan1 = getenv("RD_WNMS_SCAN1") != nullptr;
    d.wnms_no_skip = getenv("RD_WNMS_NO_SKIP") != nullptr;
    d.wnms_bal = num("RD_WNMS_BAL", 0);
    return d;
  }();
  return s;
}
#else
inline constexpr const DevSwitches& dev_switches() { return kDevSwitchDefaults; }
#endif

template <class K>
inline void allow_big_lds(K kernel) {
  if (hipFuncSetAttribute((const void*)kernel, hipFuncAttributeMaxDynamicSharedMemorySize, 160 * 1024) != hipSuccess)
    (void)hipGetLastError();
}
template <class F>
inline void once_per_device(std::atomic<unsigned long long>& seen, F f) {
  int dev = 0;
  if (hipGetDevice(&dev) != hipSuccess) { (void)hipGetLastError(); f(); return; }
  if (dev < 0 || dev >= 64) { f(); return; }
  const unsigned long long bit = 1ull << dev;
  if (seen.load(std::memory_order_acquire) & bit) return;
  f();
  seen.fetch_or(bit, std::memory_order_release);
}

struct Prof {
  bool on = false;
  std::mutex mu;
  struct Span { hipEvent_t a, b; int kind; };
  std::vector<Span> spans;
  std::vector<hipEvent_t> pool;
  double total[RD_PROF_NKINDS] = {0};
  long count[RD_PROF_NKINDS] = {0};
  hipEvent_t get() {
    if (!pool.empty()) { hipEvent_t e = pool.back(); pool.pop_back(); return e; }
    hipEvent_t e;
    hipEventCreate(&e);
    return e;
  }
  void drain() {
    for (auto& s : spans) {
      hipEventSynchronize(s.b);
      float ms = 0;
      hipEventElapsedTime(&ms, s.a, s.b);
      total[s.kind] += ms;
      count[s.kind] += 1;
      pool.push_back(s.a);
      pool.push_back(s.b);
    }
    spans.clear();
  }
};
inline Prof& prof() {
  static Prof p;
  return p;
}
struct ProfScope {
  hipEvent_t a = nullptr;
  int kind;
  hipStream_t st;
  ProfScope(int k, hipStream_t s) : kind(k), st(s) {
    Prof& p = prof();
    if (!p.on) return;
    std::lock_guard<std::mutex> g(p.mu);
    a = p.get();
    hipEventRecord(a, st);
  }
  ~ProfScope() {
    if (!a) return;
    Prof& p = prof();
    std::lock_guard<std::mutex> g(p.mu);
    hipEvent_t b = p.get();
    hipEventRecord(b, st);
    p.spans.push_back({a, b, kind});
  }
};

typedef unsigned short bf16_t;
typedef float f32x16 __attribute__((ext_vector_type(16)));
typedef float f32x4 __attribute__((ext_vector_type(4)));
typedef short s16x8 __attribute__((ext_vector_type(8)));

__host__ __device__ __forceinline__ bf16_t f32_to_bf16(float f) {
#if defined(__HIP_DEVICE_COMPILE__)
  return __builtin_bit_cast(unsigned short, (__bf16)f);
#endif
  unsigned u;
  memcpy(&u, &f, 4);
  if ((u & 0x7fffffffu) > 0x7f800000u) return (bf16_t)((u >> 16) | 0x40);
  u += 0x7fffu + ((u >> 16) & 1u);
  return (bf16_t)(u >> 16);
}
__host__ __device__ __forceinline__ unsigned f32x2_to_bf16x2(float a, float b) {
#if defined(__HIP_DEVICE_COMPILE__)
  typedef float f32x2_t __attribute__((ext_vector_type(2)));
  typedef __bf16 bf16x2_t __attribute__((ext_vector_type(2)));
  const f32x2_t v = {a, b};
  return __builtin_bit_cast(unsigned, __builtin_convertvector(v, bf16x2_t));
#else
  return (unsigned)f32_to_bf16(a) | ((unsigned)f32_to_bf16(b) << 16);
#endif
}
__host__ __device__ __forceinline__ float bf16_to_f32(bf16_t h) {
  unsigned u = (unsigned)h << 16;
  float f;
  memcpy(&f, &u, 4);
  return f;
}

typedef unsigned short f16_t;
typedef _Float16 h16x8 __attribute__((ext_vector_type(8)));
__host__ __device__ __forceinline__ f16_t f32_to_f16(float f) { return __builtin_bit_cast(unsigned short, (_Float16)f); }
__host__ __device__ __forceinline__ float f16_to_f32(f16_t h) { return (float)__builtin_bit_cast(_Float16, h); }
__host__ __device__ __forceinline__ unsigned f32x2_to_f16x2(float a, float b) {
#if defined(__HIP_DEVICE_COMPILE__)
  typedef float f32x2_t __attribute__((ext_vector_type(2)));
  typedef _Float16 f16x2_t __attribute__((ext_vector_type(2)));
  const f32x2_t v = {a, b};
  return __builtin_bit_cast(unsigned, __builtin_convertvector(v, f16x2_t));
#else
  return (unsigned)f32_to_f16(a) | ((unsigned)f32_to_f16(b) << 16);
#endif
}

typedef float f32x2_t_ __attribute__((ext_vector_type(2)));
template <int DT> struct H16;
template <> struct H16<RD_BF16> {
  static constexpr unsigned short ONE = 0x3F80;
  __host__ __device__ static __forceinline__ unsigned short from_f32(float v) { return f32_to_bf16(v); }
  __host__ __device__ static __forceinline__ float to_f32(unsigned short h) { return bf16_to_f32(h); }
  __host__ __device__ static __forceinline__ unsigned pk(float a, float b) { return f32x2_to_bf16x2(a, b); }
  __host__ __device__ static __forceinline__ f32x2_t_ unpk(unsigned u) {
    unsigned lo = u << 16, hi = u & 0xffff0000u;
    return f32x2_t_{__builtin_bit_cast(float, lo), __builtin_bit_cast(float, hi)};
  }
  __device__ static __forceinline__ f32x16 mfma(s16x8 a, s16x8 b, f32x16 c) { return __builtin_amdgcn_mfma_f32_32x32x16_bf16(a, b, c, 0, 0, 0); }
  __device__ static __forceinline__ f32x4 mfma16(s16x8 a, s16x8 b, f32x4 c) { return __builtin_amdgcn_mfma_f32_16x16x32_bf16(a, b, c, 0, 0, 0); }
};
template <> struct H16<RD_F16> {
  static constexpr unsigned short ONE = 0x3C00;
  __host__ __device__ static __forceinline__ unsigned short from_f32(float v) { return f32_to_f16(v); }
  __host__ __device__ static __forceinline__ float to_f32(unsigned short h) { return f16_to_f32(h); }
  __host__ __device__ static __forceinline__ unsigned pk(float a, float b) { return f32x2_to_f16x2(a, b); }
  __host__ __device__ static __forceinline__ f32x2_t_ unpk(unsigned u) {
    return f32x2_t_{f16_to_f32((unsigned short)(u & 0xffffu)), f16_to_f32((unsigned short)(u >> 16))};
  }
  __device__ static __forceinline__ f32x16 mfma(s16x8 a, s16x8 b, f32x16 c) {
    return __builtin_amdgcn_mfma_f32_32x32x16_f16(__builtin_bit_cast(h16x8, a), __builtin_bit_cast(h16x8, b), c, 0, 0, 0);
  }
  __device__ static __forceinline__ f32x4 mfma16(s16x8 a, s16x8 b, f32x4 c) {
    return __builtin_amdgcn_mfma_f32_16x16x32_f16(__builtin_bit_cast(h16x8, a), __builtin_bit_cast(h16x8, b), c, 0, 0, 0);
  }
};
inline bool is_h16(int dt) { return dt == RD_BF16 || dt == RD_F16; }
inline unsigned short h16_from_f32(int dt, float v) { return dt == RD_F16 ? f32_to_f16(v) : f32_to_bf16(v); }
inline float h16_to_f32(int dt, unsigned short h) { return dt == RD_F16 ? f16_to_f32(h) : bf16_to_f32(h); }

template <int DT> struct Elem;
template <> struct Elem<RD_F32> {
  typedef float T;
  static constexpr int CH = 4;
  __host__ __device__ static float from_f32(float v) { return v; }
  __host__ __device__ static float to_f32(float v) { return v; }
};
template <> struct Elem<RD_BF16> {
  typedef bf16_t T;
  static constexpr int CH = 8;
  __host__ __device__ static bf16_t from_f32(float v) { return f32_to_bf16(v); }
  __host__ __device__ static float to_f32(bf16_t v) { return bf16_to_f32(v); }
};
template <> struct Elem<RD_F16> {
  typedef f16_t T;
  static constexpr int CH = 8;
  __host__ __device__ static f16_t from_f32(float v) { return f32_to_f16(v); }
  __host__ __device__ static float to_f32(f16_t v) { return f16_to_f32(v); }
};
inline int elem_size(int dt) { return dt == RD_F32 ? 4 : 2; }
inline int ch_per_slot(int dt) { return dt == RD_F32 ? 4 : 8; }
inline int round_up(int a, int b) { return (a + b - 1) / b * b; }

typedef unsigned Slot16 __attribute__((ext_vector_type(4)));


__device__ __forceinline__ void lds_dma16(const void* gsrc, void* lds_dst_uniform) {
#if defined(__HIP_DEVICE_COMPILE__)
  const unsigned lds_addr = __builtin_amdgcn_readfirstlane(
      (unsigned)(uintptr_t)(__attribute__((address_space(3))) void*)lds_dst_uniform);
  unsigned keep;
  asm volatile("s_mov_b32 %0, m0\n\ts_mov_b32 m0, %2\n\ts_nop 0\n\tglobal_load_lds_dwordx4 %1, off\n\ts_mov_b32 m0, %0"
               : "=&s"(keep)
               : "v"(gsrc), "s"(lds_addr)
               : "memory");
#else
  __builtin_amdgcn_global_load_lds((const __attribute__((address_space(1))) void*)gsrc,
                                   (__attribute__((address_space(3))) void*)lds_dst_uniform, 16, 0, 0);
#endif
}

__host__ __device__ inline float fdlibm_atanf(float x) {
  _Pragma("clang fp contract(off)")
  const float hi_[4] = {4.6364760399e-01f, 7.8539812565e-01f, 9.8279368877e-01f, 1.5707962513e+00f};
  const float lo_[4] = {5.0121582440e-09f, 3.7748947079e-08f, 3.4473217170e-08f, 7.5497894159e-08f};
  const float t0 = 3.3333334327e-01f, t1 = -2.0000000298e-01f, t2 = 1.4285714924e-01f, t3 = -1.1111110449e-01f, t4 = 9.0908870101e-02f,
              t5 = -7.6918758452e-02f, t6 = 6.6610731184e-02f, t7 = -5.8335702866e-02f, t8 = 4.9768779427e-02f, t9 = -3.6531571299e-02f,
              t10 = 1.6285819933e-02f;
  const int hx = __builtin_bit_cast(int, x), ix = hx & 0x7fffffff;
  int id;
  if (ix >= 0x4c000000) {
    if (ix > 0x7f800000) return x + x;
    return hx > 0 ? hi_[3] + lo_[3] : -hi_[3] - lo_[3];
  }
  if (ix < 0x3ee00000) {
    if (ix < 0x31000000) return x;
    id = -1;
  } else {
    x = __builtin_fabsf(x);
    if (ix < 0x3f980000) {
      if (ix < 0x3f300000) { id = 0; x = (2.0f * x - 1.0f) / (2.0f + x); }
      else { id = 1; x = (x - 1.0f) / (x + 1.0f); }
    } else {
      if (ix < 0x401c0000) { id = 2; x = (x - 1.5f) / (1.0f + 1.5f * x); }
      else { id = 3; x = -1.0f / x; }
    }
  }
  const float z = x * x, w = z * z;
  const float s1 = z * (t0 + w * (t2 + w * (t4 + w * (t6 + w * (t8 + w * t10)))));
  const float s2 = w * (t1 + w * (t3 + w * (t5 + w * (t7 + w * t9))));
  if (id < 0) return x - x * (s1 + s2);
  const float r = hi_[id] - ((x * (s1 + s2) - lo_[id]) - x);
  return hx < 0 ? -r : r;
}
__host__ __device__ inline float fdlibm_atan2f(float y, float x) {
  _Pragma("clang fp contract(off)")
  const float tiny = 1.0e-30f, pi_o_4 = 7.8539818525e-01f, pi_o_2 = 1.5707963705e+00f, pi = 3.1415927410e+00f, pi_lo = -8.7422776573e-08f;
  const int hx = __builtin_bit_cast(int, x), ix = hx & 0x7fffffff;
  const int hy = __builtin_bit_cast(int, y), iy = hy & 0x7fffffff;
  if (ix > 0x7f800000 || iy > 0x7f800000) return x + y;
  if (hx == 0x3f800000) return fdlibm_atanf(y);
  const int m = ((hy >> 31) & 1) | ((hx >> 30) & 2);
  if (iy == 0) return m < 2 ? y : (m == 2 ? pi + tiny : -pi - tiny);
  if (ix == 0) return hy < 0 ? -pi_o_2 - tiny : pi_o_2 + tiny;
  if (ix == 0x7f800000) {
    if (iy == 0x7f800000) return m == 0 ? pi_o_4 + tiny : m == 1 ? -pi_o_4 - tiny : m == 2 ? 3.0f * pi_o_4 + tiny : -3.0f * pi_o_4 - tiny;
    return m == 0 ? 0.0f : m == 1 ? -0.0f : m == 2 ? pi + tiny : -pi - tiny;
  }
  if (iy == 0x7f800000) return hy < 0 ? -pi_o_2 - tiny : pi_o_2 + tiny;
  const int k = (iy - ix) >> 23;
  float z;
  if (k > 60) z = pi_o_2 + 0.5f * pi_lo;
  else if (hx < 0 && k < -60) z = 0.0f;
  else z = fdlibm_atanf(__builtin_fabsf(y / x));
  switch (m) {
    case 0: return z;
    case 1: return __builtin_bit_cast(float, __builtin_bit_cast(unsigned, z) ^ 0x80000000u);
    case 2: return pi - (z - pi_lo);
    default: return (z - pi_lo) - pi;
  }
}

}
```

rangedet_amd/lib.py:

```python
import ctypes
import os

import numpy as np

RD_OK, RD_EINVAL, RD_ESHAPE, RD_EWORKSPACE, RD_EHIP = 0, -1, -2, -3, -4
RD_F32, RD_BF16, RD_F16 = 0, 1, 2
H16 = (RD_BF16, RD_F16)
RD_RELU_PRE, RD_ADD, RD_RELU_POST, RD_SCALE_FOLDED, RD_MFMA16 = 1, 2, 4, 8, 16
RD_WNMS_MAX_K = 65536
RD_WNMS_DIAG_NO_SKIP = 0x100


def RD_WNMS_DIAG_TILE_W(n):
    return (n & 0xff) << 16


def RD_WNMS_DIAG_MERGE_LDS(n):
    return (n & 0x7f) << 24

RD_TIE_STABLE, RD_TIE_REFERENCE = 0, 1
PROF_KINDS = {"conv": 0, "meta": 1, "head_out": 2, "sort": 3, "decode": 4, "wnms": 5, "layout": 6, "conv3": 7, "block": 8}

_HERE = os.path.dirname(os.path.abspath(__file__))
DEFAULT_PATH = os.environ.get("RANGEDET_HIP_LIB") or os.path.join(_HERE, "librangedet_hip.so")

c_int, c_long, c_float, c_size_t, c_void_p = ctypes.c_int, ctypes.c_long, ctypes.c_float, ctypes.c_size_t, ctypes.c_void_p

SIGNATURES = {
    "rd_version": (c_int, []),
    "rd_last_error_string": (ctypes.c_char_p, []),
    "rd_nchw_to_nhwc": (c_int, [c_void_p, c_void_p, c_int, c_int, c_int, c_int, c_int, c_int, c_int, c_int, c_void_p]),
    "rd_nhwc_to_nchw": (c_int, [c_void_p, c_void_p, c_int, c_int, c_int, c_int, c_int, c_int, c_int, c_void_p]),
    "rd_copy_rows": (c_int, [c_void_p, c_long, c_void_p, c_long, c_long, c_long, c_int, c_void_p]),
    "rd_conv_packed_bytes": (c_size_t, [c_int, c_int, c_int, c_int]),
    "rd_pack_conv_weight_host": (c_int, [c_void_p, c_int, c_int, c_int, c_int, c_int, c_void_p]),
    "rd_deconv_phase_taps": (c_int, [c_int, c_int, c_int, c_int, c_int]),
    "rd_pack_deconv_weight_host": (c_int, [c_void_p, c_int, c_int, c_int, c_int, c_int, c_int, c_int, c_int, c_void_p]),
    "rd_pack_deconv_weight_folded_host": (c_int, [c_void_p, c_void_p, c_int, c_int, c_int, c_int, c_int, c_int, c_int, c_int, c_void_p]),
    "rd_conv2d_bn_act": (c_int, [c_void_p, c_int, c_int, c_void_p, c_void_p, c_void_p, c_void_p, c_int, c_int, c_void_p,
                                 c_int, c_int, c_int, c_int, c_int, c_int, c_int, c_int, c_int, c_int, c_int, c_int, c_void_p]),
    "rd_conv3x3_ex_packed_bytes": (c_size_t, [c_int, c_int, c_int, c_int]),
    "rd_pack_conv3x3_ex_host": (c_int, [c_void_p, c_void_p, c_int, c_int, c_int, c_int, c_int, c_void_p]),
    "rd_pack_conv3x3_m16_host": (c_int, [c_void_p, c_void_p, c_int, c_int, c_int, c_void_p]),
    "rd_conv3x3_mfma16_ok": (c_int, [c_int, c_int, c_int, c_int, c_int]),
    "rd_conv1x1_sc_packed_bytes": (c_size_t, [c_int, c_int]),
    "rd_pack_conv1x1_sc_host": (c_int, [c_void_p, c_void_p, c_int, c_int, c_int, c_void_p]),
    "rd_conv3x3_bn_act_ex": (c_int, [c_void_p, c_int, c_int, c_void_p, c_void_p, c_void_p, c_void_p, c_int, c_int, c_void_p, c_int,
                                     c_int, c_int, c_void_p, c_void_p, c_int, c_int, c_int, c_int, c_int, c_int, c_int, c_int,
                                     c_int, c_int, c_void_p]),
    "rd_deconv2d_bn_act": (c_int, [c_void_p, c_int, c_int, c_void_p, c_void_p, c_void_p, c_void_p, c_int, c_int, c_void_p,
                                   c_int, c_int, c_int, c_int, c_int, c_int, c_int, c_int, c_int, c_int, c_int, c_int,
                                   c_int, c_int, c_void_p]),
    "rd_conv3x3_cat_packed_bytes": (c_size_t, [c_int, c_int, c_int]),
    "rd_pack_conv3x3_cat_host": (c_int, [c_void_p, c_void_p, c_int, c_int, c_int, c_int, c_void_p]),
    "rd_conv3x3_bn_act_cat": (c_int, [c_void_p, c_int, c_int, c_int, c_void_p, c_int, c_int, c_int, c_void_p, c_void_p, c_void_p, c_int, c_int,
                                      c_int, c_int, c_int, c_int, c_int, c_int, c_void_p]),
    "rd_deconv2d_all_phases_ok": (c_int, [c_int, c_int, c_int, c_int, c_int, c_int]),
    "rd_deconv2d_bn_act_all": (c_int, [c_void_p, c_int, c_int, c_void_p, c_long, c_void_p, c_void_p, c_int, c_int, c_void_p,
                                       c_int, c_int, c_int, c_int, c_int, c_int, c_int, c_int, c_int, c_int, c_int, c_int,
                                       c_int, c_void_p]),
    "rd_deconv2d_phase_pairs_ok": (c_int, [c_int, c_int, c_int, c_int, c_int, c_int]),
    "rd_pack_deconv_phase_pair_host": (c_int, [c_void_p, c_void_p, c_int, c_int, c_void_p]),
    "rd_deconv2d_bn_act_pairs": (c_int, [c_void_p, c_int, c_int, c_void_p, c_long, c_void_p, c_void_p, c_int, c_int, c_void_p,
                                         c_int, c_int, c_int, c_int, c_int, c_int, c_int, c_int, c_int, c_int, c_int, c_int,
                                         c_int, c_void_p]),
    "rd_block64_packed_bytes": (c_size_t, [c_int]),
    "rd_pack_block64_host": (c_int, [c_void_p, c_void_p, c_void_p, c_void_p, c_int, c_int, c_void_p]),
    "rd_pack_block64_m16_host": (c_int, [c_void_p, c_void_p, c_void_p, c_void_p, c_int, c_void_p]),
    "rd_pack_conv1x1_sc_m16_host": (c_int, [c_void_p, c_void_p, c_int, c_void_p]),
    "rd_block64_m16_bn_act": (c_int, [c_void_p, c_int, c_int, c_void_p, c_void_p, c_void_p, c_void_p, c_void_p, c_int, c_int, c_int, c_int,
                                      c_int, c_int, c_void_p]),
    "rd_block64_bn_act": (c_int, [c_void_p, c_int, c_int, c_int, c_void_p, c_void_p, c_void_p, c_void_p, c_void_p, c_int, c_int, c_int, c_int,
                                  c_int, c_int, c_void_p]),
    "rd_head_packed_bytes": (c_size_t, []),
    "rd_head_m16_packed_bytes": (c_size_t, []),
    "rd_pack_head_weight_host": (c_int, [c_void_p, c_int, c_int, c_int, c_void_p]),
    "rd_pack_head_weight_m16_host": (c_int, [c_void_p, c_int, c_int, c_int, c_void_p]),
    "rd_conv2d_bn_act_head_out": (c_int, [c_void_p, c_int, c_int, c_void_p, c_void_p, c_void_p, c_int, c_int, c_int, c_int, c_int,
                                          c_void_p, c_void_p, c_void_p, c_long, c_long, c_int, c_int, c_void_p]),
    "rd_conv3x3_bn_act_pair": (c_int, [c_void_p, c_int, c_void_p, c_void_p, c_void_p, c_int] * 2 +
                               [c_int, c_int, c_int, c_int, c_int, c_int, c_int, c_int, c_void_p]),
    "rd_conv2d_bn_act_head_out_pair": (c_int, [c_void_p, c_int, c_void_p, c_void_p, c_void_p, c_void_p, c_void_p, c_long, c_int] * 2 +
                                       [c_int, c_long, c_int, c_int, c_int, c_int, c_int, c_int, c_void_p]),
    "rd_head_out": (c_int, [c_void_p, c_int, c_int, c_void_p, c_void_p, c_void_p, c_long, c_long, c_int, c_int, c_int,
                            c_int, c_int, c_int, c_void_p]),
    "rd_meta_packed_bytes": (c_size_t, [c_int]),
    "rd_pack_meta_host": (c_int, [c_void_p] * 9 + [c_int, c_void_p]),
    "rd_meta_kernel_fwd": (c_int, [c_void_p, c_int, c_int, c_void_p, c_void_p, c_void_p, c_int, c_int, c_int, c_int,
                                   c_int, c_int, c_void_p]),
    "rd_sorted_foreground_workspace_bytes": (c_size_t, [c_long, c_long]),
    "rd_sorted_foreground": (c_int, [c_void_p, c_void_p, c_void_p, c_void_p, c_int, c_long, c_long, c_int, c_int,
                                     c_void_p, c_void_p, c_void_p, c_void_p, c_void_p, c_size_t, c_void_p]),
    "rd_decode3d_bbox": (c_int, [c_void_p, c_void_p, c_void_p, c_int, c_long, c_int, c_int, c_void_p]),
    "rd_score_filter_workspace_bytes": (c_size_t, [c_long]),
    "rd_score_filter_dets": (c_int, [c_void_p, c_void_p, c_long, c_float, c_void_p, c_void_p, c_void_p, c_size_t, c_void_p]),
    "rd_score_filter_dets_batched": (c_int, [c_void_p, c_long, c_void_p, c_long, c_long, c_float, c_void_p, c_long, c_void_p,
                                             c_void_p, c_size_t, c_int, c_void_p]),
    "rd_wnms_workspace_bytes": (c_size_t, [c_int]),
    "rd_wnms_4c_batched": (c_int, [c_void_p, c_long, c_int, c_void_p, c_void_p, c_long, c_int, c_float, c_float, c_int, c_int,
                                   c_void_p, c_long, c_void_p, c_long, c_void_p, c_void_p, c_size_t, c_int, c_void_p]),
    "rd_dets12_to_8_batched": (c_int, [c_void_p, c_long, c_int, c_void_p, c_void_p, c_long, c_int, c_void_p]),
    "rd_wnms_4c": (c_int, [c_void_p, c_int, c_void_p, c_void_p, c_int, c_float, c_float, c_int, c_int, c_void_p, c_void_p,
                           c_void_p, c_void_p, c_size_t, c_void_p]),
    "rd_single_overlap": (c_int, [c_void_p, c_void_p, c_long, c_int, c_void_p, c_void_p]),
    "rd_wnms_order_host": (c_int, [c_void_p, c_int, c_void_p]),
    "rd_edge_atan2f": (c_int, [c_void_p, c_void_p, c_long, c_void_p, c_void_p]),
    "rd_wnms_pair_skippable": (c_int, [c_void_p, c_void_p, c_long, c_void_p, c_void_p]),
    "rd_dets12_to_8": (c_int, [c_void_p, c_int, c_void_p, c_void_p, c_void_p]),
    "rd_rotated_iou_8pt": (c_int, [c_void_p, c_void_p, c_void_p, c_long, c_long, c_void_p]),
    "rd_batch_rotated_iou": (c_int, [c_void_p, c_int, c_void_p, c_void_p, c_void_p, c_int, c_long, c_int, c_void_p]),
    "rd_batch_rotated_iou_3d": (c_int, [c_void_p, c_int, c_void_p, c_void_p, c_void_p, c_int, c_long, c_int, c_void_p]),
    "rd_rotated_iou_7": (c_int, [c_void_p, c_void_p, c_void_p, c_long, c_long, c_void_p]),
    "rd_batch_max_iou": (c_int, [c_void_p, c_int, c_void_p, c_void_p, c_long, c_int, c_void_p]),
    "rd_gather_keep_scores": (c_int, [c_void_p, c_long, c_int, c_void_p, c_int, c_void_p, c_int, c_void_p]),
    "rd_nms3d_workspace_bytes": (c_size_t, [c_long, c_int]),
    "rd_nms3d": (c_int, [c_void_p, c_int, c_long, c_float, c_int, c_int, c_void_p, c_void_p, c_void_p, c_size_t, c_void_p]),
    "rd_assign3d_v2": (c_int, [c_void_p] * 6 + [c_long, c_int] + [c_float] * 7 + [c_void_p, c_void_p]),
    "rd_get_point_num_workspace_bytes": (c_size_t, []),
    "rd_get_point_num": (c_int, [c_void_p, c_long, c_void_p, c_void_p, c_size_t, c_void_p]),
    "rd_input_transform": (c_int, [c_void_p, c_void_p, c_void_p, c_void_p, c_int, c_int, c_int, c_int, c_int] + [c_void_p] * 8 + [c_void_p]),
    "rd_prof_enable": (c_int, [c_int]),
    "rd_prof_reset": (c_int, []),
    "rd_prof_get": (c_int, [c_int, ctypes.POINTER(ctypes.c_double), ctypes.POINTER(c_long)]),
}


class RangeDetError(RuntimeError):
    def __init__(self, code, msg):
        super().__init__("librangedet_hip error %d: %s" % (code, msg))
        self.code = code


def ptr(x):
    if x is None:
        return None
    if isinstance(x, int):
        return x
    if isinstance(x, np.ndarray):
        return x.ctypes.data
    if hasattr(x, "data_ptr"):
        return x.data_ptr()
    raise TypeError("cannot take the address of %r" % type(x))


class Lib:
    def __init__(self, path=DEFAULT_PATH):
        if not os.path.exists(path):
            raise RuntimeError(
                "%s not found: the HIP extension is not built (run `python -m rangedet_amd.build`). "
                "There is no CPU fallback." % path)
        self.path = path
        if os.path.basename(path).startswith("librangedet_hip"):
            try:
                import torch
            except ImportError:
                pass
        self.cdll = ctypes.CDLL(path)
        for name, (res, args) in SIGNATURES.items():
            fn = getattr(self.cdll, name)
            fn.restype = res
            fn.argtypes = args
        self.rd_last_error_string = self.cdll.rd_last_error_string

    def call(self, name, *args):
        rc = getattr(self.cdll, name)(*args)
        if rc < 0:
            raise RangeDetError(rc, self.cdll.rd_last_error_string().decode())
        return rc

    def raw(self, name):
        return getattr(self.cdll, name)

    def pack_conv_weight(self, w_oihw, dtype):
        w = np.ascontiguousarray(w_oihw, dtype=np.float32)
        cout, cin, kh, kw = w.shape
        out = np.zeros(self.cdll.rd_conv_packed_bytes(kh * kw, cin, cout, dtype), dtype=np.uint8)
        self.call("rd_pack_conv_weight_host", w.ctypes.data, cout, cin, kh, kw, dtype, out.ctypes.data)
        return out

    def pack_conv3x3_ex(self, w_oihw, stride_w, x_cstride, fold_scale=None, dtype=RD_BF16):
        w = np.ascontiguousarray(w_oihw, dtype=np.float32)
        cout, cin = w.shape[:2]
        assert w.shape[2:] == (3, 3)
        fs = None if fold_scale is None else np.ascontiguousarray(fold_scale, dtype=np.float32)
        out = np.zeros(self.cdll.rd_conv3x3_ex_packed_bytes(cin, cout, stride_w, x_cstride), dtype=np.uint8)
        self.call("rd_pack_conv3x3_ex_host", w.ctypes.data, None if fs is None else fs.ctypes.data, cout, cin, stride_w,
                  x_cstride, dtype, out.ctypes.data)
        return out

    def pack_conv3x3_m16(self, w_oihw, fold_scale, dtype=RD_BF16):
        w = np.ascontiguousarray(w_oihw, dtype=np.float32)
        cout, cin = w.shape[:2]
        assert w.shape[2:] == (3, 3)
        fs = np.ascontiguousarray(fold_scale, dtype=np.float32)
        out = np.zeros(self.cdll.rd_conv3x3_ex_packed_bytes(cin, cout, 1, cin), dtype=np.uint8)
        self.call("rd_pack_conv3x3_m16_host", w.ctypes.data, fs.ctypes.data, cout, cin, dtype, out.ctypes.data)
        return out

    def pack_conv3x3_cat(self, w_oihw, cin1, cin2, fold_scale=None, dtype=RD_BF16):
        w = np.ascontiguousarray(w_oihw, dtype=np.float32)
        cout = w.shape[0]
        assert w.shape[1:] == (cin1 + cin2, 3, 3)
        fs = None if fold_scale is None else np.ascontiguousarray(fold_scale, dtype=np.float32)
        out = np.zeros(self.cdll.rd_conv3x3_cat_packed_bytes(cin1, cin2, cout), dtype=np.uint8)
        self.call("rd_pack_conv3x3_cat_host", w.ctypes.data, None if fs is None else fs.ctypes.data, cout, cin1, cin2, dtype, out.ctypes.data)
        return out

    def pack_conv1x1_sc(self, w_oi, fold_scale=None, dtype=RD_BF16):
        w = np.ascontiguousarray(w_oi, dtype=np.float32).reshape(w_oi.shape[0], -1)
        cout, cin = w.shape
        fs = None if fold_scale is None else np.ascontiguousarray(fold_scale, dtype=np.float32)
        out = np.zeros(self.cdll.rd_conv1x1_sc_packed_bytes(cin, cout), dtype=np.uint8)
        self.call("rd_pack_conv1x1_sc_host", w.ctypes.data, None if fs is None else fs.ctypes.data, cout, cin, dtype, out.ctypes.data)
        return out

    def pack_block64(self, w1_oihw, scale1, w2_oihw, scale2, dtype=RD_BF16, m16=False):
        w1, w2 = (np.ascontiguousarray(w, dtype=np.float32) for w in (w1_oihw, w2_oihw))
        s1, s2 = (np.ascontiguousarray(v, dtype=np.float32) for v in (scale1, scale2))
        cin = w1.shape[1]
        assert w1.shape == (64, cin, 3, 3) and w2.shape == (64, 64, 3, 3) and s1.shape == (64,) and s2.shape == (64,)
        out = np.zeros(self.cdll.rd_block64_packed_bytes(cin), dtype=np.uint8)
        if m16:
            assert cin == 64
            self.call("rd_pack_block64_m16_host", w1.ctypes.data, s1.ctypes.data, w2.ctypes.data, s2.ctypes.data, dtype, out.ctypes.data)
        else:
            self.call("rd_pack_block64_host", w1.ctypes.data, s1.ctypes.data, w2.ctypes.data, s2.ctypes.data, cin, dtype, out.ctypes.data)
        return out

    def pack_conv1x1_sc_m16(self, w_oi, fold_scale, dtype=RD_BF16):
        w = np.ascontiguousarray(w_oi, dtype=np.float32).reshape(64, 64)
        fs = np.ascontiguousarray(fold_scale, dtype=np.float32)
        out = np.zeros(self.cdll.rd_conv1x1_sc_packed_bytes(64, 64), dtype=np.uint8)
        self.call("rd_pack_conv1x1_sc_m16_host", w.ctypes.data, fs.ctypes.data, dtype, out.ctypes.data)
        return out

    def pack_deconv_weight(self, w_iohw, stride_w, pad_w, phase, dtype, fold_scale=None):
        w = np.ascontiguousarray(w_iohw, dtype=np.float32)
        cin, cout, kh, kw = w.shape
        nt = self.cdll.rd_deconv_phase_taps(kh, kw, stride_w, pad_w, phase)
        if nt < 0:
            raise RangeDetError(nt, "deconv phase taps")
        out = np.zeros(self.cdll.rd_conv_packed_bytes(nt, cin, cout, dtype), dtype=np.uint8)
        fs = None if fold_scale is None else np.ascontiguousarray(fold_scale, dtype=np.float32)
        self.call("rd_pack_deconv_weight_folded_host", w.ctypes.data, None if fs is None else fs.ctypes.data, cin, cout, kh, kw,
                  stride_w, pad_w, phase, dtype, out.ctypes.data)
        return out

    def pack_deconv_phase_pair(self, img_a, img_b, cin, dtype):
        assert img_a.nbytes == img_b.nbytes
        out = np.empty(2 * img_a.nbytes, np.uint8)
        a, b = np.ascontiguousarray(img_a), np.ascontiguousarray(img_b)
        self.call("rd_pack_deconv_phase_pair_host", a.ctypes.data, b.ctypes.data, cin, dtype, out.ctypes.data)
        return out

    def pack_head_weight(self, w, dtype=RD_BF16, m16=False):
        w = np.ascontiguousarray(w, dtype=np.float32)
        out = np.zeros(self.cdll.rd_head_m16_packed_bytes() if m16 else self.cdll.rd_head_packed_bytes(), dtype=np.uint8)
        self.call("rd_pack_head_weight_m16_host" if m16 else "rd_pack_head_weight_host", w.ctypes.data, w.shape[0], w.shape[1], dtype, out.ctypes.data)
        return out

    def pack_meta(self, w0, b0, w1, b1, s1, t1, agg, s2, t2, dtype):
        arrs = [np.ascontiguousarray(a, dtype=np.float32) for a in (w0, b0, w1, b1, s1, t1, agg, s2, t2)]
        assert arrs[0].shape == (32, 3) and arrs[2].shape == (64, 32) and arrs[6].shape == (64, 576)
        out = np.zeros(self.cdll.rd_meta_packed_bytes(dtype), dtype=np.uint8)
        self.call("rd_pack_meta_host", *[a.ctypes.data for a in arrs], dtype, out.ctypes.data)
        return out

    def wnms_order_host(self, dets):
        d = np.ascontiguousarray(dets, dtype=np.float32).reshape(-1, 12)
        order = np.empty(d.shape[0], dtype=np.int32)
        self.call("rd_wnms_order_host", d.ctypes.data, d.shape[0], order.ctypes.data)
        return order

    def prof(self):
        out = {}
        ms, n = ctypes.c_double(), c_long()
        for k, v in PROF_KINDS.items():
            self.call("rd_prof_get", v, ctypes.byref(ms), ctypes.byref(n))
            out[k] = (ms.value, n.value)
        return out


_LIB = None


def get_lib():
    global _LIB
    if _LIB is None:
        _LIB = Lib(DEFAULT_PATH)
    return _LIB
```

rangedet_amd/runtime.py:

```python
import os

import numpy as np

from . import devswitch, lib as rdlib
from .lower import FlatRef, TRef


class TorchAllocator:

    def __init__(self, device="cuda:0", stream=None):
        import torch
        if not torch.cuda.is_available():
            raise RuntimeError("rangedet_amd needs a ROCm GPU (torch.cuda.is_available() is False); there is no CPU fallback")
        self.torch = torch
        self.device = torch.device(device)
        torch.cuda.set_device(self.device)
        self._stream = stream

    @property
    def stream(self):
        st = self._stream or self.torch.cuda.current_stream(self.device)
        return st.cuda_stream

    def alloc(self, nbytes, zero=False):
        f = self.torch.zeros if zero else self.torch.empty
        return f(max(int(nbytes), 16), dtype=self.torch.uint8, device=self.device)

    def upload(self, arr):
        a = np.ascontiguousarray(arr)
        t = self.torch.from_numpy(a.view(np.uint8).reshape(-1)).to(self.device)
        return t

    def ptr(self, buf):
        return buf.data_ptr()

    def view_f32(self, buf, shape):
        n = int(np.prod(shape))
        return buf[: n * 4].view(self.torch.float32).view(*shape)

    def view_i32(self, buf, shape):
        n = int(np.prod(shape))
        return buf[: n * 4].view(self.torch.int32).view(*shape)

    def to_numpy(self, t):
        return t.detach().cpu().numpy()

    def as_device_f32(self, x):
        t = self.torch
        if isinstance(x, np.ndarray):
            return t.from_numpy(np.ascontiguousarray(x, dtype=np.float32)).to(self.device)
        return x.to(device=self.device, dtype=t.float32).contiguous()

    def assign(self, dst_view, src):
        dst_view.copy_(src.reshape(dst_view.shape))

    def new_stream(self, priority=0):
        return self.torch.cuda.Stream(device=self.device, priority=priority)

    def stream_ptr(self, stream):
        return stream.cuda_stream if stream is not None else self.stream

    def record_event(self, stream=None):
        ev = self.torch.cuda.Event()
        ev.record(stream if stream is not None else self.torch.cuda.current_stream(self.device))
        return ev

    def wait_event(self, ev, stream=None):
        (stream if stream is not None else self.torch.cuda.current_stream(self.device)).wait_event(ev)

    def sync(self):
        self.torch.cuda.synchronize(self.device)


def bn_affine(P, name, eps, pad_to=None):
    g, b, m, v = (np.asarray(P[name + s], np.float64) for s in ("_gamma", "_beta", "_moving_mean", "_moving_var"))
    s = g / np.sqrt(v + eps)
    s, t = s.astype(np.float32), (b - m * s).astype(np.float32)
    if pad_to is not None and pad_to > len(s):
        s = np.concatenate([s, np.ones(pad_to - len(s), np.float32)])
        t = np.concatenate([t, np.zeros(pad_to - len(t), np.float32)])
    return s, t


def pad_rows(w, n, axis=0):
    if w.shape[axis] >= n:
        return w
    shp = list(w.shape)
    shp[axis] = n - w.shape[axis]
    return np.concatenate([w, np.zeros(shp, w.dtype)], axis)


class Executor:
    def __init__(self, plan, params, lib=None, alloc=None, reuse_buffers=True, keep_sorted_idx=False):
        self.keep_sorted_idx = keep_sorted_idx
        self.plan = plan
        self.lib = lib or rdlib.get_lib()
        self.alloc = alloc or TorchAllocator()
        self.dtype = plan.dtype
        self.B = plan.batch
        self._phys = {}
        self._assign_buffers(reuse_buffers)
        self._bound = [self._bind(st, params) for st in plan.steps]

    def _assign_buffers(self, reuse):
        plan = self.plan
        last_use, first_def = {}, {}
        for i, st in enumerate(plan.steps):
            for v in st.values():
                if isinstance(v, (TRef, FlatRef)):
                    last_use[v.buf] = i
                    first_def.setdefault(v.buf, i)
        for kind, v in plan.outputs:
            if kind in ("flat", "flat_i32"):
                last_use[v.buf] = len(plan.steps) + 1
        free = {}
        release = {}
        for b, i in last_use.items():
            release.setdefault(i, []).append(b)
        order = sorted(plan.buffers, key=lambda b: first_def.get(b, 0))
        by_def = {}
        for b in order:
            by_def.setdefault(first_def.get(b, 0), []).append(b)
        for i in range(len(plan.steps) + 2):
            for b in by_def.get(i, []):
                info = plan.buffers[b]
                if reuse and not info["persistent"] and free.get(info["nbytes"]):
                    self._phys[b] = free[info["nbytes"]].pop()
                else:
                    self._phys[b] = self.alloc.alloc(info["nbytes"], zero=info["zero"])
            for b in release.get(i, []):
                info = plan.buffers[b]
                if reuse and not info["persistent"] and last_use[b] <= len(plan.steps):
                    free.setdefault(info["nbytes"], []).append(self._phys[b])
        self.device_bytes = sum(int(t.numel()) if hasattr(t, "numel") else len(t) for t in {id(v): v for v in self._phys.values()}.values())

    def p(self, ref):
        return self.alloc.ptr(self._phys[ref.buf])

    def _bind(self, st, P):
        L, A, dt = self.lib, self.alloc, self.dtype
        k = st["kind"]
        b = dict(st)
        if k == "conv_pair":
            b["a"], b["b"] = self._bind(st["a"], P), self._bind(st["b"], P)
            return b
        if k == "block":
            ca, cb = st["a"], st["b"]
            w1, w2 = (np.asarray(P[c["name"] + "_weight"], np.float32) for c in (ca, cb))
            if ca.get("cmap"):
                wp = np.zeros((w1.shape[0], len(ca["cmap"])) + w1.shape[2:], np.float32)
                for pc, lc in enumerate(ca["cmap"]):
                    if lc >= 0:
                        wp[:, pc] = w1[:, lc]
                w1 = wp
            (s1, t1), (s2, t2) = bn_affine(P, ca["bn"], ca["eps"]), bn_affine(P, cb["bn"], cb["eps"])
            m16 = bool(st.get("m16")) and w1.shape[1] == 64
            b["m16"] = m16
            b["w"] = A.upload(L.pack_block64(w1, s1, w2, s2, dtype=dt, m16=m16))
            b["shift1"] = A.upload(t1)
            b["sc_w"] = None
            if cb.get("sc"):
                sc = cb["sc"]
                wsc = np.asarray(P[sc["name"] + "_weight"], np.float32).reshape(64, -1)
                if sc.get("cmap"):
                    wq = np.zeros((64, len(sc["cmap"])), np.float32)
                    for pc, lc in enumerate(sc["cmap"]):
                        if lc >= 0:
                            wq[:, pc] = wsc[:, lc]
                    wsc = wq
                ss, ts = bn_affine(P, sc["bn"], sc["eps"])
                b["sc_w"] = A.upload(L.pack_conv1x1_sc_m16(wsc, ss, dtype=dt) if m16 else L.pack_conv1x1_sc(wsc, fold_scale=ss, dtype=dt))
                t2 = (t2.astype(np.float64) + ts).astype(np.float32)
            b["shift2"] = A.upload(t2)
            b["cin"] = w1.shape[1]
            return b
        if k == "conv":
            w = pad_rows(np.asarray(P[st["name"] + "_weight"], np.float32), st["cout"])
            if st.get("cmap"):
                wp = np.zeros((w.shape[0], len(st["cmap"])) + w.shape[2:], np.float32)
                for pc, lc in enumerate(st["cmap"]):
                    if lc >= 0:
                        wp[:, pc] = w[:, lc]
                w = wp
            s, t = bn_affine(P, st["bn"], st["eps"], pad_to=st["cout"])
            if st.get("sc"):
                sc = st["sc"]
                wsc = np.asarray(P[sc["name"] + "_weight"], np.float32)
                wsc = pad_rows(wsc.reshape(wsc.shape[0], -1), st["cout"])
                if sc.get("cmap"):
                    wq = np.zeros((w.shape[0], len(sc["cmap"])), np.float32)
                    for pc, lc in enumerate(sc["cmap"]):
                        if lc >= 0:
                            wq[:, pc] = wsc[:, lc]
                    wsc = wq
                ss, ts = bn_affine(P, sc["bn"], sc["eps"], pad_to=st["cout"])
                b["w"] = A.upload(L.pack_conv3x3_ex(w, st["stride_w"], st["x"].cs, fold_scale=s, dtype=dt))
                b["sc_w"] = A.upload(L.pack_conv1x1_sc(wsc, fold_scale=ss, dtype=dt))
                b["scale"], b["shift"] = None, A.upload((t.astype(np.float64) + ts).astype(np.float32))
            elif st.get("x2") is not None:
                b["w"] = A.upload(L.pack_conv3x3_cat(w, st["x"].C, st["x2"].cs, fold_scale=s, dtype=dt))
                b["scale"], b["shift"] = None, A.upload(t)
                b["flags"] = st["flags"] | rdlib.RD_SCALE_FOLDED
            elif st.get("ex") and st.get("fold") and st.get("m16") and \
                    L.raw("rd_conv3x3_mfma16_ok")(w.shape[1], st["cout"], 1, st["x"].W, 1 if st.get("head") else 0) == 1:
                b["w"] = A.upload(L.pack_conv3x3_m16(w, s, dtype=dt))
                b["scale"], b["shift"] = None, A.upload(t)
                b["flags"] = st["flags"] | rdlib.RD_SCALE_FOLDED | rdlib.RD_MFMA16
            elif st.get("ex") and st.get("fold"):
                b["w"] = A.upload(L.pack_conv3x3_ex(w, st["stride_w"], st["x"].cs, fold_scale=s, dtype=dt))
                b["scale"], b["shift"] = None, A.upload(t)
                b["flags"] = st["flags"] | rdlib.RD_SCALE_FOLDED
            elif st.get("ex"):
                b["w"] = A.upload(L.pack_conv3x3_ex(w, st["stride_w"], st["x"].cs, dtype=dt))
                b["scale"], b["shift"] = A.upload(s), A.upload(t)
            else:
                b["w"] = A.upload(L.pack_conv_weight(w, dt))
                b["scale"], b["shift"] = A.upload(s), A.upload(t)
        elif k == "deconv":
            w = pad_rows(np.asarray(P[st["name"] + "_weight"], np.float32), st["cout"], axis=1)
            s, t = bn_affine(P, st["bn"], st["eps"], pad_to=st["cout"])
            fs = s if st.get("fold") else None
            imgs = [L.pack_deconv_weight(w, st["stride_w"], st["pad_w"], ph, dt, fold_scale=fs) for ph in range(st["stride_w"])]
            b["all_phases"] = bool(st.get("one_launch")) and len({len(i) for i in imgs}) == 1 and \
                L.raw("rd_deconv2d_all_phases_ok")(st["k"][0], st["k"][1], st["stride_w"], st["pad_w"], st["cout"], dt) == 1
            if st.get("one_launch") and not b["all_phases"] and not L.raw("rd_deconv2d_all_phases_ok")(st["k"][0], st["k"][1], st["stride_w"], st["pad_w"], st["cout"], dt):
                b["one_launch"] = False
            if b["all_phases"]:
                b["w_all"], b["w_pb"] = A.upload(np.concatenate(imgs)), len(imgs[0])
            r_, o_ = st["res"], st["out"]
            b["pairs"] = b["all_phases"] and not devswitch.get("RD_DECONV_NO_PAIRS") and o_.cs == st["cout"] and o_.co == 0 and \
                (r_ is None or (r_.cs == st["cout"] and r_.co == 0)) and \
                L.raw("rd_deconv2d_phase_pairs_ok")(st["k"][0], st["k"][1], st["stride_w"], st["pad_w"], st["cout"], dt) == 1
            if b["pairs"]:
                pimgs = [L.pack_deconv_phase_pair(imgs[p], imgs[p + 1], st["cin"], dt) for p in range(0, st["stride_w"], 2)]
                b["w_pairs"], b["w_pairb"], b["shift2"] = A.upload(np.concatenate(pimgs)), len(pimgs[0]), A.upload(np.concatenate([t, t]))
            b["w"] = [A.upload(i) for i in imgs]
            b["scale"], b["shift"] = (None if st.get("fold") else A.upload(s)), A.upload(t)
            if st.get("fold"):
                b["flags"] = st["flags"] | rdlib.RD_SCALE_FOLDED
        elif k == "meta":
            s1, t1 = bn_affine(P, st["bn1"], st["eps1"])
            s2, t2 = bn_affine(P, st["bn2"], st["eps2"])
            pk = L.pack_meta(P[st["mlp0"] + "_weight"].reshape(32, 3), P[st["mlp0"] + "_bias"],
                             P[st["mlp1"] + "_weight"].reshape(64, 32), P[st["mlp1"] + "_bias"], s1, t1,
                             P[st["agg"] + "_weight"].reshape(64, 576), s2, t2, dt)
            b["packed"] = A.upload(pk)
        if k == "conv" and st.get("head"):
            h = st["head"]
            r0, r1 = h["rows"]
            hw = np.asarray(P[h["name"] + "_weight"], np.float32).reshape(-1, st["cout"])[r0:r1]
            b["head_w"] = A.upload(L.pack_head_weight(hw, dtype=dt, m16=bool(b.get("flags", 0) & rdlib.RD_MFMA16)))
            b["head_bias"] = A.upload(np.asarray(P[h["name"] + "_bias"], np.float32)[r0:r1])
        elif k == "head_out":
            r0, r1 = st["rows"]
            w = np.asarray(P[st["name"] + "_weight"], np.float32).reshape(-1, st["x"].C)[r0:r1]
            b["w"] = A.upload(w)
            b["bias"] = A.upload(np.asarray(P[st["name"] + "_bias"], np.float32)[r0:r1])
        elif k == "nms3d":
            nb = L.raw("rd_nms3d_workspace_bytes")(st["N"], self.B)
            b["ws"] = A.alloc(nb)
            b["ws_bytes"] = nb
        elif k == "sorted_fg":
            nb = L.raw("rd_sorted_foreground_workspace_bytes")(st["N"], st["k"]) * self.B
            b["ws"] = A.alloc(nb)
            b["ws_bytes"] = nb
            b["idx"] = A.alloc(self.B * st["k"] * 4) if self.keep_sorted_idx else None
        return b

    def forward(self, inputs, only=None, dev=None):
        L, A, dt, B = self.lib, self.alloc, self.dtype, self.B
        st_ = A.stream
        dev = {} if dev is None else dev

        def din(name):
            if name not in dev:
                dev[name] = A.as_device_f32(inputs[name])
            return dev[name]

        steps = self._bound if only is None else [self._bound[only]]
        for b in steps:
            k = b["kind"]
            if k == "nchw_in":
                o = b["out"]
                src = din(b["name"])
                assert tuple(src.shape) == (B, o.C, o.H, o.W), (b["name"], tuple(src.shape), (B, o.C, o.H, o.W))
                L.call("rd_nchw_to_nhwc", A.ptr(src), self.p(o), B, o.C, o.H, o.W, o.cs, o.co, b["zero_pad"], dt, st_)
            elif k == "block":
                x, o = b["x"], b["out"]
                if b.get("m16"):
                    L.call("rd_block64_m16_bn_act", self.p(x), x.cs, x.co, A.ptr(b["w"]), A.ptr(b["shift1"]), A.ptr(b["shift2"]),
                           A.ptr(b["sc_w"]) if b["sc_w"] is not None else None, self.p(o), o.cs, o.co, B, x.H, x.W, dt, st_)
                else:
                    L.call("rd_block64_bn_act", self.p(x), x.cs, x.co, b["cin"], A.ptr(b["w"]), A.ptr(b["shift1"]), A.ptr(b["shift2"]),
                           A.ptr(b["sc_w"]) if b["sc_w"] is not None else None, self.p(o), o.cs, o.co, B, x.H, x.W, dt, st_)
            elif k == "conv_pair":
                p, q = b["a"], b["b"]
                x0, x1 = p["x"], q["x"]
                cin = len(p["cmap"]) if p.get("cmap") else p["cin"]
                if p.get("head"):
                    h0, h1 = p["head"], q["head"]
                    L.call("rd_conv2d_bn_act_head_out_pair",
                           self.p(x0), x0.co, A.ptr(p["w"]), A.ptr(p["shift"]), A.ptr(p["head_w"]), A.ptr(p["head_bias"]),
                           self.p(h0["out"]), h0["N"] * h0["nout"], h0["nout"],
                           self.p(x1), x1.co, A.ptr(q["w"]), A.ptr(q["shift"]), A.ptr(q["head_w"]), A.ptr(q["head_bias"]),
                           self.p(h1["out"]), h1["N"] * h1["nout"], h1["nout"],
                           x0.cs, h0["n_off"], B, x0.H, x0.W, cin, p["flags"], dt, st_)
                else:
                    o0, o1 = p["out"], q["out"]
                    L.call("rd_conv3x3_bn_act_pair", self.p(x0), x0.co, A.ptr(p["w"]), A.ptr(p["shift"]), self.p(o0), o0.co,
                           self.p(x1), x1.co, A.ptr(q["w"]), A.ptr(q["shift"]), self.p(o1), o1.co, x0.cs, o0.cs, B, x0.H, x0.W, cin,
                           p["flags"], dt, st_)
            elif k == "conv" and b.get("head"):
                x, h = b["x"], b["head"]
                L.call("rd_conv2d_bn_act_head_out", self.p(x), x.cs, x.co, A.ptr(b["w"]),
                       A.ptr(b["scale"]) if b["scale"] is not None else None, A.ptr(b["shift"]), B,
                       x.H, x.W, b["cin"], b["flags"], A.ptr(b["head_w"]), A.ptr(b["head_bias"]), self.p(h["out"]),
                       h["N"] * h["nout"], h["n_off"], h["nout"], dt, st_)
            elif k == "conv" and b.get("x2") is not None:
                x, x2, o = b["x"], b["x2"], b["out"]
                L.call("rd_conv3x3_bn_act_cat", self.p(x), x.cs, x.co, x.C, self.p(x2), x2.cs, x2.co, x2.cs, A.ptr(b["w"]), A.ptr(b["shift"]),
                       self.p(o), o.cs, o.co, B, x.H, x.W, b["cout"], b["flags"], dt, st_)
            elif k == "conv" and b.get("ex"):
                x, o, r, sx = b["x"], b["out"], b["res"], b.get("sc_x")
                cin = len(b["cmap"]) if b.get("cmap") else b["cin"]
                L.call("rd_conv3x3_bn_act_ex", self.p(x), x.cs, x.co, A.ptr(b["w"]), A.ptr(b["scale"]) if b["scale"] is not None else None,
                       A.ptr(b["shift"]), self.p(r) if r else None, r.cs if r else 0, r.co if r else 0,
                       self.p(sx) if sx else None, sx.cs if sx else 0, sx.co if sx else 0,
                       (len(b["sc"]["cmap"]) if b["sc"].get("cmap") else b["sc"]["cin"]) if sx else 0,
                       A.ptr(b["sc_w"]) if sx else None, self.p(o), o.cs, o.co, B, x.H, x.W, cin, b["cout"], b["stride_w"],
                       b["flags"], dt, st_)
            elif k == "conv":
                x, o, r = b["x"], b["out"], b["res"]
                L.call("rd_conv2d_bn_act", self.p(x), x.cs, x.co, A.ptr(b["w"]), A.ptr(b["scale"]), A.ptr(b["shift"]),
                       self.p(r) if r else None, r.cs if r else 0, r.co if r else 0, self.p(o), o.cs, o.co, B, x.H, x.W,
                       b["cin"], b["cout"], b["k"][0], b["k"][1], b["stride_w"], b["flags"], dt, st_)
            elif k == "deconv":
                x, o, r = b["x"], b["out"], b["res"]
                if b.get("pairs"):
                    L.call("rd_deconv2d_bn_act_pairs", self.p(x), x.cs, x.co, A.ptr(b["w_pairs"]), b["w_pairb"], A.ptr(b["shift2"]), self.p(r), r.cs,
                           r.co, self.p(o), o.cs, o.co, B, x.H, x.W, b["cin"], b["cout"], b["k"][0], b["k"][1], b["stride_w"], b["pad_w"],
                           b["flags"], dt, st_)
                    continue
                if b.get("all_phases"):
                    L.call("rd_deconv2d_bn_act_all", self.p(x), x.cs, x.co, A.ptr(b["w_all"]), b["w_pb"], A.ptr(b["shift"]), self.p(r), r.cs,
                           r.co, self.p(o), o.cs, o.co, B, x.H, x.W, b["cin"], b["cout"], b["k"][0], b["k"][1], b["stride_w"], b["pad_w"],
                           b["flags"], dt, st_)
                    continue
                for ph in range(b["stride_w"]):
                    L.call("rd_deconv2d_bn_act", self.p(x), x.cs, x.co, A.ptr(b["w"][ph]),
                           A.ptr(b["scale"]) if b["scale"] is not None else None, A.ptr(b["shift"]), self.p(r), r.cs, r.co, self.p(o), o.cs, o.co, B, x.H, x.W, b["cin"],
                           b["cout"], b["k"][0], b["k"][1], b["stride_w"], b["pad_w"], ph, b["flags"], dt, st_)
            elif k == "meta":
                x, o = b["x"], b["out"]
                c = din(b["coord"])
                assert tuple(c.shape) == (B, 3, x.H, x.W)
                L.call("rd_meta_kernel_fwd", self.p(x), x.cs, x.co, A.ptr(c), A.ptr(b["packed"]), self.p(o), o.cs, o.co,
                       B, x.H, x.W, dt, st_)
            elif k == "head_out":
                x, o = b["x"], b["out"]
                L.call("rd_head_out", self.p(x), x.cs, x.co, A.ptr(b["w"]), A.ptr(b["bias"]), self.p(o),
                       b["N"] * b["nout"], b["n_off"], B, x.H, x.W, x.C, b["nout"], dt, st_)
            elif k == "concat_in":
                o = b["out"]
                row = b["N"] * b["last"] * 4
                off = 0
                for name, n in b["names"]:
                    src = din(name)
                    assert tuple(src.shape)[:2] == (B, n), (name, tuple(src.shape))
                    L.call("rd_copy_rows", A.ptr(src), n * b["last"] * 4, self.p(o), row, off * b["last"] * 4,
                           n * b["last"] * 4, B, st_)
                    off += n
            elif k == "sorted_fg":
                L.call("rd_sorted_foreground", self.p(b["score"]), self.p(b["delta"]), self.p(b["pc"]), self.p(b["mask"]),
                       B, b["N"], b["k"], b["D"], b["apply_sigmoid"], self.p(b["out_score"]), self.p(b["out_delta"]),
                       self.p(b["out_pc"]), A.ptr(b["idx"]) if b["idx"] is not None else None, A.ptr(b["ws"]), b["ws_bytes"], st_)
            elif k == "decode":
                L.call("rd_decode3d_bbox", self.p(b["delta"]), self.p(b["pc"]), self.p(b["out"]), B, b["k"],
                       b["box_type"], b["is_bin"], st_)
            elif k == "batch_riou":
                g = din(b["gt"])
                three_d = b.get("iou_type", "bev") == "3d"
                assert tuple(g.shape) == (B, b["n_gt"], 7 if three_d else 8), (b["gt"], tuple(g.shape))
                L.call("rd_batch_rotated_iou_3d" if three_d else "rd_batch_rotated_iou", self.p(b["boxes"]), 10, A.ptr(g), self.p(b["out"]),
                       None, B, b["N"], b["n_gt"], st_)
            elif k == "nms3d":
                L.call("rd_nms3d", self.p(b["boxes"]), B, b["N"], b["thr"], b["max_keep"], b["normal_iou"], self.p(b["keep"]),
                       self.p(b["out"]), A.ptr(b["ws"]), b["ws_bytes"], st_)
            else:
                raise RuntimeError("unknown plan step %r" % k)
        if only is not None:
            return None
        outs = []
        for kind, v in self.plan.outputs:
            if kind == "flat":
                outs.append(A.view_f32(self._phys[v.buf], (B,) + tuple(v.shape)))
            elif kind == "flat_i32":
                outs.append(A.view_i32(self._phys[v.buf], (B,) + tuple(v.shape)))
            elif kind == "input":
                outs.append(inputs.get(v))
            else:
                outs.append(np.zeros(v, np.float32))
        return outs

    def read_flat(self, ref):
        self.alloc.sync()
        return np.array(self.alloc.to_numpy(self.alloc.view_f32(self._phys[ref.buf], (self.B,) + tuple(ref.shape))))

    def sorted_idx(self, which=0):
        b = [x for x in self._bound if x["kind"] == "sorted_fg"][which]
        self.alloc.sync()
        return np.array(self.alloc.to_numpy(self.alloc.view_i32(b["idx"], (self.B, b["k"]))))

    def debug_tensor(self, ref):
        A, L = self.alloc, self.lib
        out = A.alloc(self.B * ref.C * ref.H * ref.W * 4)
        L.call("rd_nhwc_to_nchw", self.p(ref), A.ptr(out), self.B, ref.C, ref.H, ref.W, ref.cs, ref.co, self.dtype, A.stream)
        A.sync()
        return A.to_numpy(A.view_f32(out, (self.B, ref.C, ref.H, ref.W)))
```

Measured before the change: 994.5.

## Fuse concat, sorted-foreground top-k and bbox decode into one multi-level tail

Adds a fused sorted-foreground path that reads per-level point-cloud and mask tensors directly, so the concat_in copies are no longer needed. The top-k selection builds the histogram and compaction from fused keys, writes packed key/index pairs, and gathers and decodes boxes in a single kernel, replacing the separate decode launch. The runtime detects concat→sorted_fg→decode chains and rewrites them unless RD_TAIL_UNFUSED is set. This removes several kernel launches and intermediate buffer round-trips in the post-processing tail, at the cost of more complex plan matching and a new radix sort variant on packed pairs.

After: 998.8, median of 6. About the same (+0.4%).

```diff
diff --git a/__graft_entry__.py b/__graft_entry__.py
--- a/__graft_entry__.py
+++ b/__graft_entry__.py
@@ -13,6 +13,7 @@
         rdbuild.build(force=True)
     bad = rdbuild.packed_swap_lint()
     assert not bad, "librangedet_hip.so: %d packed-fp32 instructions with swapped source halves, first %r" % (len(bad), bad[0])
+    rdbuild.build(dev=True)
     from oracle import cpu_ops
     cpu_ops.build(with_ref=True)
     import rangedet_amd
diff --git a/include/rangedet_hip.h b/include/rangedet_hip.h
--- a/include/rangedet_hip.h
+++ b/include/rangedet_hip.h
@@ -130,6 +130,17 @@
                          int B, long N, long k, int D, int apply_sigmoid, float* out_score, float* out_delta,
                          float* out_pc, int* out_idx, void* ws, size_t ws_bytes, void* stream);
 
+typedef struct rd_fg_level {
+  const float* pc;
+  const float* mask;
+  long n, pc_bstride, mask_bstride;
+} rd_fg_level;
+size_t rd_sorted_foreground_decode_workspace_bytes(long N, long k);
+int rd_sorted_foreground_decode(const float* cls_score, const float* bbox_delta, const rd_fg_level* levels, int n_levels, int B,
+                                long N, long k, int D, int apply_sigmoid, int box_type, int is_bin, float* out_score,
+                                float* out_boxes, int* out_idx, float* out_delta, float* out_pc, void* ws, size_t ws_bytes,
+                                void* stream);
+
 int rd_decode3d_bbox(const float* bbox_delta, const float* pc, float* out, int B, long N, int box_type,
                      int is_bin, void* stream);
 
diff --git a/rangedet_amd/csrc/k_misc.h b/rangedet_amd/csrc/k_misc.h
--- a/rangedet_amd/csrc/k_misc.h
+++ b/rangedet_amd/csrc/k_misc.h
@@ -175,12 +175,8 @@
   }
 }
 
-__global__ __launch_bounds__(256) void decode3d_kernel(const float* __restrict__ delta, const float* __restrict__ pc,
-                                                       float* __restrict__ out, long n, int box_type, int is_bin) {
-  long idx = blockIdx.x * 256L + threadIdx.x;
-  if (idx >= n) return;
-  const float* d = delta + idx * box_type;
-  float pc_x = pc[idx * 3 + 0], pc_y = pc[idx * 3 + 1], pc_z = pc[idx * 3 + 2];
+__device__ __forceinline__ void decode3d_point(const float* __restrict__ d, float pc_x, float pc_y, float pc_z, float* __restrict__ o,
+                                               int is_bin) {
   float az = atan2f(pc_y, pc_x);
   float ca = cosf(az), sa = sinf(az);
   float dx, dy, width, length, height, z0, yaw_l;
@@ -209,7 +205,6 @@
   float hl = (float)(0.5 * (double)length), hw = (float)(0.5 * (double)width);
   float hx[4] = {hl, -hl, -hl, hl};
   float hy[4] = {-hw, -hw, hw, hw};
-  float* o = out + idx * 10;
 #pragma unroll
   for (int k = 0; k < 4; ++k) {
     o[2 * k] = (hx[k] * cyw - hy[k] * sy) + cx;
@@ -217,6 +212,12 @@
   }
   o[8] = z0;
   o[9] = z0 + height;
+}
+__global__ __launch_bounds__(256) void decode3d_kernel(const float* __restrict__ delta, const float* __restrict__ pc,
+                                                       float* __restrict__ out, long n, int box_type, int is_bin) {
+  long idx = blockIdx.x * 256L + threadIdx.x;
+  if (idx >= n) return;
+  decode3d_point(delta + idx * box_type, pc[idx * 3 + 0], pc[idx * 3 + 1], pc[idx * 3 + 2], out + idx * 10, is_bin);
 }
 
 __global__ __launch_bounds__(256) void filter_count_kernel(const float* __restrict__ scores, long n, float thr,
diff --git a/rangedet_amd/csrc/k_sort.h b/rangedet_amd/csrc/k_sort.h
--- a/rangedet_amd/csrc/k_sort.h
+++ b/rangedet_amd/csrc/k_sort.h
@@ -16,6 +16,7 @@
   return __uint_as_float(u);
 }
 
+#ifdef RD_DEV_SWITCHES
 __global__ __launch_bounds__(256) void sort_keygen_kernel(const float* __restrict__ score, const float* __restrict__ mask,
                                                           long N, int apply_sigmoid, unsigned* __restrict__ keys,
                                                           unsigned* __restrict__ idx, long ws_stride) {
@@ -28,6 +29,7 @@
   keys[b * ws_stride + i] = desc_key(s);
   idx[b * ws_stride + i] = (unsigned)i;
 }
+#endif
 __global__ __launch_bounds__(256) void sort_keygen_dets_kernel(const float* __restrict__ dets, int cap,
                                                                const int* __restrict__ d_count, unsigned* __restrict__ keys,
                                                                unsigned* __restrict__ idx) {
@@ -38,6 +40,8 @@
   idx[i] = (unsigned)i;
 }
 
+struct alignas(8) KeyIdx { unsigned key, idx; };
+template <bool PK>
 __global__ __launch_bounds__(256) void sort_hist_kernel(const unsigned* __restrict__ keys, long N, int shift,
                                                         unsigned* __restrict__ hist, unsigned* __restrict__ tot,
                                                         long ws_stride, const unsigned* __restrict__ d_n) {
@@ -51,7 +55,7 @@
   long base = (long)blockIdx.x * SORT_TILE;
   for (int r = 0; r < SORT_TILE / 256; ++r) {
     long i = base + r * 256 + threadIdx.x;
-    if (i < N) atomicAdd(&h[(keys[i] >> shift) & 255u], 1u);
+    if (i < N) atomicAdd(&h[((PK ? ((const KeyIdx*)keys)[i].key : keys[i]) >> shift) & 255u], 1u);
   }
   __syncthreads();
   unsigned v = h[threadIdx.x];
@@ -59,6 +63,7 @@
   if (v) atomicAdd(&tot[threadIdx.x], v);
 }
 
+template <bool PK>
 __global__ __launch_bounds__(256) void sort_scatter_kernel(const unsigned* __restrict__ keys_in,
                                                            const unsigned* __restrict__ idx_in, long N, int shift,
                                                            const unsigned* __restrict__ hist,
@@ -101,8 +106,14 @@
   for (int r = 0; r < 8; ++r) {
     long i = base + r * 64 + lane;
     bool valid = i < N;
-    key[r] = valid ? keys_in[i] : 0xFFFFFFFFu;
-    id[r] = valid ? idx_in[i] : 0u;
+    if (PK) {
+      const KeyIdx p = valid ? ((const KeyIdx*)keys_in)[i] : KeyIdx{0xFFFFFFFFu, 0u};
+      key[r] = p.key;
+      id[r] = p.idx;
+    } else {
+      key[r] = valid ? keys_in[i] : 0xFFFFFFFFu;
+      id[r] = valid ? idx_in[i] : 0u;
+    }
     unsigned d = (key[r] >> shift) & 255u;
     unsigned long long peers = __ballot(valid);
 #pragma unroll
@@ -132,12 +143,17 @@
     if (i < N) {
       unsigned d = (key[r] >> shift) & 255u;
       unsigned dst = gbase[d] + wcnt[wv][d] + pos[r];
-      keys_out[dst] = key[r];
-      idx_out[dst] = id[r];
-    }
-  }
-}
-
+      if (PK) {
+        ((KeyIdx*)keys_out)[dst] = KeyIdx{key[r], id[r]};
+      } else {
+        keys_out[dst] = key[r];
+        idx_out[dst] = id[r];
+      }
+    }
+  }
+}
+
+#ifdef RD_DEV_SWITCHES
 __global__ __launch_bounds__(256) void sort_gather_kernel(const unsigned* __restrict__ keys, const unsigned* __restrict__ idx,
                                                           long k, int D, const float* __restrict__ delta,
                                                           const float* __restrict__ pc, float* __restrict__ out_score,
@@ -160,8 +176,10 @@
   out_pc[i * 3 + 2] = pc[(size_t)j * 3 + 2];
   if (out_idx) out_idx[i] = (int)j;
 }
+#endif
 
 constexpr int SEL_BINS = 4096, SEL_SHIFT = 20;
+#ifdef RD_DEV_SWITCHES
 __global__ __launch_bounds__(256) void select_hist_kernel(const unsigned* __restrict__ keys, long N, unsigned* __restrict__ h12,
                                                           long ws_stride) {
   keys += blockIdx.y * ws_stride; h12 += blockIdx.y * ws_stride;
@@ -263,6 +281,7 @@
     off += (unsigned)__popcll(m[r]);
   }
 }
+#endif
 
 struct SortWs {
   unsigned *keysA, *keysB, *idxA, *idxB, *hist, *tot, *h12, *cnt, *sel;
@@ -293,20 +312,28 @@
   return e == hipSuccess ? RD_OK : fail(RD_EHIP, "sort: memset");
 }
 inline int radix_sort_pairs(const SortWs& s, long N, hipStream_t st, int nb = 1, long ws_stride = 0, const unsigned* d_n = nullptr,
-                            bool cleared = false) {
+                            bool cleared = false, bool hist0_done = false, bool packed = false) {
   if (!cleared) { int rc = sort_clear(s, st, nb, ws_stride, false); if (rc != RD_OK) return rc; }
-  unsigned *ki = s.keysA, *ko = s.keysB, *ii = s.idxA, *io = s.idxB;
+  unsigned *ki = s.keysA, *ko = packed ? s.idxA : s.keysB, *ii = s.idxA, *io = s.idxB;
+  const dim3 grid(s.nblk, nb), block(256);
   for (int pass = 0; pass < 4; ++pass) {
-    hipLaunchKernelGGL(sort_hist_kernel, dim3(s.nblk, nb), dim3(256), 0, st, ki, N, pass * 8, s.hist, s.tot + pass * 256,
-                       ws_stride, d_n);
-    hipLaunchKernelGGL(sort_scatter_kernel, dim3(s.nblk, nb), dim3(256), 0, st, ki, ii, N, pass * 8, s.hist,
-                       s.tot + pass * 256, ko, io, ws_stride, d_n);
+    unsigned* tot = s.tot + pass * 256;
+    if (packed) {
+      if (pass > 0 || !hist0_done)
+        hipLaunchKernelGGL((sort_hist_kernel<true>), grid, block, 0, st, ki, N, pass * 8, s.hist, tot, ws_stride, d_n);
+      hipLaunchKernelGGL((sort_scatter_kernel<true>), grid, block, 0, st, ki, ki, N, pass * 8, s.hist, tot, ko, ko, ws_stride, d_n);
+    } else {
+      if (pass > 0 || !hist0_done)
+        hipLaunchKernelGGL((sort_hist_kernel<false>), grid, block, 0, st, ki, N, pass * 8, s.hist, tot, ws_stride, d_n);
+      hipLaunchKernelGGL((sort_scatter_kernel<false>), grid, block, 0, st, ki, ii, N, pass * 8, s.hist, tot, ko, io, ws_stride, d_n);
+      std::swap(ii, io);
+    }
     std::swap(ki, ko);
-    std::swap(ii, io);
   }
   return check_launch("radix_sort_pairs");
 }
 
+#ifdef RD_DEV_SWITCHES
 inline int radix_topk_pairs(const SortWs& s, long N, long k, hipStream_t st, int nb, long ws_stride, unsigned** rk, unsigned** ri) {
   const bool off = dev_switches().sort_no_select;
   *rk = s.keysA; *ri = s.idxA;
@@ -323,5 +350,208 @@
   *rk = s.keysB; *ri = s.idxB;
   return radix_sort_pairs(v, N, st, nb, ws_stride, s.sel + 1, true);
 }
-
-}
+#endif
+
+constexpr int FG_MAX_LEVELS = 4;
+struct FgIn {
+  const float* score;
+  const float* mask[FG_MAX_LEVELS];
+  const float* pc[FG_MAX_LEVELS];
+  long mask_bs[FG_MAX_LEVELS], pc_bs[FG_MAX_LEVELS];
+  long start[FG_MAX_LEVELS];
+  long N;
+  int nlev, apply_sigmoid;
+};
+__device__ __forceinline__ unsigned fg_key(const FgIn& in, long b, long i) {
+  float s = in.score[b * in.N + i];
+  if (in.apply_sigmoid) s = 1.0f / (1.0f + expf(-s));
+  const float* m = in.mask[0];
+  long bs = in.mask_bs[0], s0 = 0;
+#pragma unroll
+  for (int q = 1; q < FG_MAX_LEVELS; ++q)
+    if (q < in.nlev && i >= in.start[q]) { m = in.mask[q]; bs = in.mask_bs[q]; s0 = in.start[q]; }
+  if (m) s = s * m[b * bs + (i - s0)];
+  return desc_key(s);
+}
+__device__ __forceinline__ const float* fg_pc_row(const FgIn& in, long b, long i) {
+  const float* p = in.pc[0];
+  long bs = in.pc_bs[0], s0 = 0;
+#pragma unroll
+  for (int q = 1; q < FG_MAX_LEVELS; ++q)
+    if (q < in.nlev && i >= in.start[q]) { p = in.pc[q]; bs = in.pc_bs[q]; s0 = in.start[q]; }
+  return p + b * bs + (i - s0) * 3;
+}
+
+__global__ __launch_bounds__(256) void fg_hist_kernel(FgIn in, unsigned* __restrict__ h12, long ws_stride) {
+  h12 += blockIdx.y * ws_stride;
+  __shared__ unsigned h[SEL_BINS];
+  for (int i = threadIdx.x; i < SEL_BINS; i += 256) h[i] = 0;
+  __syncthreads();
+  const long base = (long)blockIdx.x * SORT_TILE;
+  for (int r = 0; r < SORT_TILE / 256; ++r) {
+    const long i = base + r * 256 + threadIdx.x;
+    if (i < in.N) atomicAdd(&h[fg_key(in, blockIdx.y, i) >> SEL_SHIFT], 1u);
+  }
+  __syncthreads();
+  for (int i = threadIdx.x; i < SEL_BINS; i += 256)
+    if (h[i]) atomicAdd(&h12[i], h[i]);
+}
+__device__ __forceinline__ void fg_thresh(const unsigned* __restrict__ h12, long k, unsigned* part, unsigned* out) {
+  const int tid = threadIdx.x;
+  unsigned loc[SEL_BINS / 256], sum = 0;
+#pragma unroll
+  for (int j = 0; j < SEL_BINS / 256; ++j) { loc[j] = h12[tid * (SEL_BINS / 256) + j]; sum += loc[j]; }
+  part[tid] = sum;
+  __syncthreads();
+  for (int off = 1; off < 256; off <<= 1) {
+    const unsigned v = tid >= off ? part[tid - off] : 0u;
+    __syncthreads();
+    part[tid] += v;
+    __syncthreads();
+  }
+  unsigned before = part[tid] - sum;
+  if (tid == 255 && (k == 0 || part[255] < (unsigned)k)) { out[0] = SEL_BINS - 1; out[1] = part[255]; }
+  if (before < (unsigned)k && before + sum >= (unsigned)k) {
+#pragma unroll
+    for (int j = 0; j < SEL_BINS / 256; ++j) {
+      if (before < (unsigned)k && before + loc[j] >= (unsigned)k) { out[0] = tid * (SEL_BINS / 256) + j; out[1] = before + loc[j]; }
+      before += loc[j];
+    }
+  }
+}
+__global__ __launch_bounds__(256) void fg_count_kernel(FgIn in, long k, int take_all, const unsigned* __restrict__ h12,
+                                                       unsigned* __restrict__ sel, unsigned* __restrict__ cnt,
+                                                       unsigned* __restrict__ hist, long ws_stride) {
+  {
+    const long o = blockIdx.y * ws_stride;
+    h12 += o; sel += o; cnt += o; hist += o;
+  }
+  __shared__ unsigned part[256], tm[2], c;
+  const long base = (long)blockIdx.x * SORT_TILE;
+  hist[(size_t)blockIdx.x * 256 + threadIdx.x] = 0;
+  if (take_all) {
+    if (threadIdx.x == 0) {
+      cnt[blockIdx.x] = (unsigned)min((long)SORT_TILE, in.N - base);
+      if (blockIdx.x == 0) { sel[0] = SEL_BINS - 1; sel[1] = (unsigned)in.N; }
+    }
+    return;
+  }
+  if (threadIdx.x == 0) c = 0;
+  fg_thresh(h12, k, part, tm);
+  __syncthreads();
+  const unsigned T = tm[0];
+  unsigned mine = 0;
+  for (int r = 0; r < SORT_TILE / 256; ++r) {
+    const long i = base + r * 256 + threadIdx.x;
+    if (i < in.N && (fg_key(in, blockIdx.y, i) >> SEL_SHIFT) <= T) ++mine;
+  }
+  if (mine) atomicAdd(&c, mine);
+  __syncthreads();
+  if (threadIdx.x == 0) {
+    cnt[blockIdx.x] = c;
+    if (blockIdx.x == 0) { sel[0] = T; sel[1] = tm[1]; }
+  }
+}
+__global__ __launch_bounds__(256) void fg_compact_kernel(FgIn in, const unsigned* __restrict__ sel, const unsigned* __restrict__ cnt,
+                                                         unsigned* __restrict__ pairs_out, unsigned* __restrict__ hist,
+                                                         unsigned* __restrict__ tot, long ws_stride) {
+  {
+    const long o = blockIdx.y * ws_stride;
+    sel += o; cnt += o; pairs_out += o; hist += o; tot += o;
+  }
+  const unsigned T = sel[0];
+  __shared__ unsigned wcnt[4][8], sbase, h0[2][256];
+  const int tid = threadIdx.x, lane = tid & 63, wv = tid >> 6;
+  h0[0][tid] = 0;
+  h0[1][tid] = 0;
+  if (tid == 0) {
+    unsigned b = 0;
+    for (unsigned j = 0; j < blockIdx.x; ++j) b += cnt[j];
+    sbase = b;
+  }
+  const long base = (long)blockIdx.x * SORT_TILE + wv * 512;
+  unsigned key[8];
+  unsigned long long m[8];
+#pragma unroll
+  for (int r = 0; r < 8; ++r) {
+    const long i = base + r * 64 + lane;
+    const bool valid = i < in.N;
+    key[r] = valid ? fg_key(in, blockIdx.y, i) : 0xFFFFFFFFu;
+    m[r] = __ballot(valid && (key[r] >> SEL_SHIFT) <= T);
+    if (lane == 0) wcnt[wv][r] = (unsigned)__popcll(m[r]);
+  }
+  __syncthreads();
+  const unsigned tile0 = sbase / SORT_TILE;
+  unsigned off = sbase;
+  for (int w = 0; w < wv; ++w)
+#pragma unroll
+    for (int r = 0; r < 8; ++r) off += wcnt[w][r];
+#pragma unroll
+  for (int r = 0; r < 8; ++r) {
+    if ((m[r] >> lane) & 1ull) {
+      const unsigned dst = off + (unsigned)__popcll(m[r] & ((1ull << lane) - 1ull));
+      ((KeyIdx*)pairs_out)[dst] = KeyIdx{key[r], (unsigned)(base + r * 64 + lane)};
+      atomicAdd(&h0[dst / SORT_TILE - tile0][key[r] & 255u], 1u);
+    }
+    off += (unsigned)__popcll(m[r]);
+  }
+  __syncthreads();
+  const unsigned v0 = h0[0][tid], v1 = h0[1][tid];
+  if (v0) atomicAdd(&hist[(size_t)tile0 * 256 + tid], v0);
+  if (v1) atomicAdd(&hist[(size_t)(tile0 + 1) * 256 + tid], v1);
+  if (v0 + v1) atomicAdd(&tot[tid], v0 + v1);
+}
+struct alignas(16) F4 { float x, y, z, w; };
+struct alignas(8) F2 { float x, y; };
+__global__ __launch_bounds__(256) void fg_gather_decode_kernel(const unsigned* __restrict__ pairs, long k, int D,
+                                                               const float* __restrict__ delta, FgIn in,
+                                                               float* __restrict__ out_score, float* __restrict__ out_box,
+                                                               float* __restrict__ out_delta, float* __restrict__ out_pc,
+                                                               int* __restrict__ out_idx, long ws_stride, int is_bin) {
+  const long i = blockIdx.x * 256L + threadIdx.x;
+  if (i >= k) return;
+  const long b = blockIdx.y;
+  const KeyIdx ki = ((const KeyIdx*)(pairs + b * ws_stride))[i];
+  const unsigned j = ki.idx;
+  const size_t o = (size_t)b * k + i;
+  out_score[o] = key_to_float(ki.key);
+  const float* dg = delta + ((size_t)b * in.N + j) * D;
+  const float* p = fg_pc_row(in, b, j);
+  const float px = p[0], py = p[1], pz = p[2];
+  float d[8];
+  if (D == 8 && ((uintptr_t)dg & 15) == 0) {
+    const F4 a = ((const F4*)dg)[0], c = ((const F4*)dg)[1];
+    d[0] = a.x; d[1] = a.y; d[2] = a.z; d[3] = a.w; d[4] = c.x; d[5] = c.y; d[6] = c.z; d[7] = c.w;
+  } else {
+#pragma unroll
+    for (int c = 0; c < 8; ++c) d[c] = c < D ? dg[c] : 0.f;
+  }
+  if (out_box) {
+    float bx[10];
+    decode3d_point(d, px, py, pz, bx, is_bin);
+    F2* ob = (F2*)(out_box + o * 10);
+#pragma unroll
+    for (int c = 0; c < 5; ++c) ob[c] = F2{bx[2 * c], bx[2 * c + 1]};
+  }
+  if (out_delta)
+    for (int c = 0; c < D; ++c) out_delta[o * D + c] = dg[c];
+  if (out_pc) { out_pc[o * 3 + 0] = px; out_pc[o * 3 + 1] = py; out_pc[o * 3 + 2] = pz; }
+  if (out_idx) out_idx[o] = (int)j;
+}
+
+inline int fg_sorted_decode(const SortWs& s, const FgIn& in, long k, int D, const float* delta, float* out_score, float* out_box,
+                            float* out_delta, float* out_pc, int* out_idx, int is_bin, hipStream_t st, int nb, long ws_stride) {
+  const long N = in.N;
+  const bool take_all = dev_switches().sort_no_select || 2 * k > N;
+  { int rc = sort_clear(s, st, nb, ws_stride, !take_all); if (rc != RD_OK) return rc; }
+  const dim3 grid(s.nblk, nb), block(256);
+  if (!take_all) hipLaunchKernelGGL(fg_hist_kernel, grid, block, 0, st, in, s.h12, ws_stride);
+  hipLaunchKernelGGL(fg_count_kernel, grid, block, 0, st, in, k, take_all ? 1 : 0, s.h12, s.sel, s.cnt, s.hist, ws_stride);
+  hipLaunchKernelGGL(fg_compact_kernel, grid, block, 0, st, in, s.sel, s.cnt, s.keysA, s.hist, s.tot, ws_stride);
+  { int rc = radix_sort_pairs(s, N, st, nb, ws_stride, s.sel + 1, true, true, true); if (rc != RD_OK) return rc; }
+  hipLaunchKernelGGL(fg_gather_decode_kernel, dim3((unsigned)((k + 255) / 256), nb), block, 0, st, s.keysA, k, D, delta, in,
+                     out_score, out_box, out_delta, out_pc, out_idx, ws_stride, is_bin);
+  return check_launch("sorted_foreground");
+}
+
+}
diff --git a/rangedet_amd/csrc/rd_api.hip b/rangedet_amd/csrc/rd_api.hip
--- a/rangedet_amd/csrc/rd_api.hip
+++ b/rangedet_amd/csrc/rd_api.hip
@@ -666,6 +666,44 @@
   return check_launch("meta_kernel");
 }
 
+static int fg_run(const float* cls_score, const float* bbox_delta, const rd_fg_level* levels, int n_levels, int B, long N, long k, int D,
+                  int apply_sigmoid, int is_bin, float* out_score, float* out_boxes, int* out_idx, float* out_delta, float* out_pc,
+                  void* ws, size_t ws_bytes, void* stream) {
+  FgIn in = {};
+  long total = 0;
+  for (int l = 0; l < n_levels; ++l) {
+    const rd_fg_level& lv = levels[l];
+    RD_REQUIRE(lv.pc && lv.n > 0, RD_EINVAL, "sorted_foreground: level %d has no points", l);
+    RD_REQUIRE(B == 1 || (lv.pc_bstride >= lv.n * 3 && (!lv.mask || lv.mask_bstride >= lv.n)), RD_ESHAPE,
+               "sorted_foreground: level %d frame strides (%ld, %ld) below its %ld positions", l, lv.pc_bstride, lv.mask_bstride, lv.n);
+    in.pc[l] = lv.pc; in.mask[l] = lv.mask; in.pc_bs[l] = lv.pc_bstride; in.mask_bs[l] = lv.mask_bstride; in.start[l] = total;
+    total += lv.n;
+  }
+  RD_REQUIRE(total == N, RD_ESHAPE, "sorted_foreground: the levels hold %ld positions, N is %ld", total, N);
+  in.score = cls_score; in.N = N; in.nlev = n_levels; in.apply_sigmoid = apply_sigmoid;
+  hipStream_t st = (hipStream_t)stream;
+  void* wsa = (void*)(((uintptr_t)ws + 255) & ~(uintptr_t)255);
+  SortWs s = sort_ws_carve(wsa, N);
+  ProfScope ps(RD_PROF_SORT, st);
+  const size_t per = rd_sorted_foreground_workspace_bytes(N, k);
+  const bool wide = ws_bytes >= per * (size_t)B;
+  const long stride = wide ? (long)(per / 4) : 0;
+  const int nb = wide ? B : 1;
+  for (int b0 = 0; b0 < B; b0 += nb) {
+    FgIn f = in;
+    f.score += (size_t)b0 * N;
+    for (int l = 0; l < n_levels; ++l) {
+      f.pc[l] += (size_t)b0 * in.pc_bs[l];
+      if (f.mask[l]) f.mask[l] += (size_t)b0 * in.mask_bs[l];
+    }
+    int rc = fg_sorted_decode(s, f, k, D, bbox_delta + (size_t)b0 * N * D, out_score + (size_t)b0 * k,
+                              out_boxes ? out_boxes + (size_t)b0 * k * 10 : nullptr, out_delta ? out_delta + (size_t)b0 * k * D : nullptr,
+                              out_pc ? out_pc + (size_t)b0 * k * 3 : nullptr, out_idx ? out_idx + (size_t)b0 * k : nullptr, is_bin, st, nb,
+                              stride);
+    if (rc != RD_OK) return rc;
+  }
+  return RD_OK;
+}
 size_t rd_sorted_foreground_workspace_bytes(long N, long k) { (void)k; return (sort_ws_bytes(N) + 256 + 255) & ~(size_t)255; }
 int rd_sorted_foreground(const float* cls_score, const float* bbox_delta, const float* pc, const float* mask, int B,
                          long N, long k, int D, int apply_sigmoid, float* out_score, float* out_delta, float* out_pc,
@@ -676,26 +714,52 @@
   RD_REQUIRE(N < (1L << 31), RD_ESHAPE, "sorted_foreground: N too large");
   RD_REQUIRE(ws_bytes >= rd_sorted_foreground_workspace_bytes(N, k), RD_EWORKSPACE, "sorted_foreground: workspace %zu < %zu",
              ws_bytes, rd_sorted_foreground_workspace_bytes(N, k));
-  hipStream_t st = (hipStream_t)stream;
-  void* wsa = (void*)(((uintptr_t)ws + 255) & ~(uintptr_t)255);
-  SortWs s = sort_ws_carve(wsa, N);
-  ProfScope ps(RD_PROF_SORT, st);
-  const size_t per = rd_sorted_foreground_workspace_bytes(N, k);
-  const bool wide = ws_bytes >= per * (size_t)B;
-  const long stride = wide ? (long)(per / 4) : 0;
-  const int nb = wide ? B : 1;
-  for (int b0 = 0; b0 < B; b0 += nb) {
-    hipLaunchKernelGGL(sort_keygen_kernel, dim3((unsigned)((N + 255) / 256), nb), dim3(256), 0, st, cls_score + (size_t)b0 * N,
-                       mask ? mask + (size_t)b0 * N : nullptr, N, apply_sigmoid, s.keysA, s.idxA, stride);
-    unsigned *rk, *ri;
-    int rc = radix_topk_pairs(s, N, k, st, nb, stride, &rk, &ri);
-    if (rc != RD_OK) return rc;
-    hipLaunchKernelGGL(sort_gather_kernel, dim3((unsigned)((k + 255) / 256), nb), dim3(256), 0, st, rk, ri, k, D,
-                       bbox_delta + (size_t)b0 * N * D, pc + (size_t)b0 * N * 3, out_score + (size_t)b0 * k,
-                       out_delta + (size_t)b0 * k * D, out_pc + (size_t)b0 * k * 3, out_idx ? out_idx + (size_t)b0 * k : nullptr,
-                       stride, N);
-  }
-  return check_launch("sorted_foreground");
+  const rd_fg_level one = {pc, mask, N, N * 3, N};
+#ifdef RD_DEV_SWITCHES
+  if (dev_switches().tail_unfused) {
+    hipStream_t st = (hipStream_t)stream;
+    void* wsa = (void*)(((uintptr_t)ws + 255) & ~(uintptr_t)255);
+    SortWs s = sort_ws_carve(wsa, N);
+    ProfScope ps(RD_PROF_SORT, st);
+    const size_t per = rd_sorted_foreground_workspace_bytes(N, k);
+    const bool wide = ws_bytes >= per * (size_t)B;
+    const long stride = wide ? (long)(per / 4) : 0;
+    const int nb = wide ? B : 1;
+    for (int b0 = 0; b0 < B; b0 += nb) {
+      hipLaunchKernelGGL(sort_keygen_kernel, dim3((unsigned)((N + 255) / 256), nb), dim3(256), 0, st, cls_score + (size_t)b0 * N,
+                         mask ? mask + (size_t)b0 * N : nullptr, N, apply_sigmoid, s.keysA, s.idxA, stride);
+      unsigned *rk, *ri;
+      int rc = radix_topk_pairs(s, N, k, st, nb, stride, &rk, &ri);
+      if (rc != RD_OK) return rc;
+      hipLaunchKernelGGL(sort_gather_kernel, dim3((unsigned)((k + 255) / 256), nb), dim3(256), 0, st, rk, ri, k, D,
+                         bbox_delta + (size_t)b0 * N * D, pc + (size_t)b0 * N * 3, out_score + (size_t)b0 * k,
+                         out_delta + (size_t)b0 * k * D, out_pc + (size_t)b0 * k * 3, out_idx ? out_idx + (size_t)b0 * k : nullptr,
+                         stride, N);
+    }
+    return check_launch("sorted_foreground");
+  }
+#endif
+  return fg_run(cls_score, bbox_delta, &one, 1, B, N, k, D, apply_sigmoid, 0, out_score, nullptr, out_idx, out_delta, out_pc, ws,
+                ws_bytes, stream);
+}
+
+size_t rd_sorted_foreground_decode_workspace_bytes(long N, long k) { return rd_sorted_foreground_workspace_bytes(N, k); }
+int rd_sorted_foreground_decode(const float* cls_score, const float* bbox_delta, const rd_fg_level* levels, int n_levels, int B,
+                                long N, long k, int D, int apply_sigmoid, int box_type, int is_bin, float* out_score,
+                                float* out_boxes, int* out_idx, float* out_delta, float* out_pc, void* ws, size_t ws_bytes,
+                                void* stream) {
+  RD_REQUIRE(cls_score && bbox_delta && levels && out_score && out_boxes && ws, RD_EINVAL, "sorted_foreground_decode: null pointer");
+  RD_REQUIRE(B > 0 && N > 0 && k > 0 && D > 0, RD_ESHAPE, "sorted_foreground_decode: empty shape");
+  RD_REQUIRE(N >= k, RD_ESHAPE, "sorted_foreground_decode: N (%ld) < num_fgs (%ld)", N, k);
+  RD_REQUIRE(N < (1L << 31), RD_ESHAPE, "sorted_foreground_decode: N too large");
+  RD_REQUIRE((is_bin && box_type == 7) || (!is_bin && box_type == 8), RD_ESHAPE,
+             "sorted_foreground_decode: box_type %d with is_bin=%d (8 for regular, 7 for bin)", box_type, is_bin);
+  RD_REQUIRE(D == box_type, RD_ESHAPE, "sorted_foreground_decode: %d deltas per position, box_type %d", D, box_type);
+  RD_REQUIRE(n_levels >= 1 && n_levels <= FG_MAX_LEVELS, RD_ESHAPE, "sorted_foreground_decode: %d levels (1..%d)", n_levels, FG_MAX_LEVELS);
+  RD_REQUIRE(ws_bytes >= rd_sorted_foreground_decode_workspace_bytes(N, k), RD_EWORKSPACE,
+             "sorted_foreground_decode: workspace %zu < %zu", ws_bytes, rd_sorted_foreground_decode_workspace_bytes(N, k));
+  return fg_run(cls_score, bbox_delta, levels, n_levels, B, N, k, D, apply_sigmoid, is_bin, out_score, out_boxes, out_idx, out_delta,
+                out_pc, ws, ws_bytes, stream);
 }
 
 int rd_decode3d_bbox(const float* bbox_delta, const float* pc, float* out, int B, long N, int box_type, int is_bin,
diff --git a/rangedet_amd/csrc/rd_common.h b/rangedet_amd/csrc/rd_common.h
--- a/rangedet_amd/csrc/rd_common.h
+++ b/rangedet_amd/csrc/rd_common.h
@@ -51,8 +51,9 @@
   bool wnms_scan1;
   int wnms_ct;
   bool wnms_no_skip;
-};
-constexpr DevSwitches kDevSwitchDefaults = {false, 1, 2, 1, 1, 1, 1, 1, false, false, 0, false, 8, false};
+  bool tail_unfused;
+};
+constexpr DevSwitches kDevSwitchDefaults = {false, 1, 2, 1, 1, 1, 1, 1, false, false, 0, false, 8, false, false};
 #ifdef RD_DEV_SWITCHES
 inline const DevSwitches& dev_switches() {
   static const DevSwitches s = [] {
@@ -72,6 +73,7 @@
     d.wnms_scan1 = getenv("RD_WNMS_SCAN1") != nullptr;
     d.wnms_no_skip = getenv("RD_WNMS_NO_SKIP") != nullptr;
     d.wnms_bal = num("RD_WNMS_BAL", 0);
+    d.tail_unfused = getenv("RD_TAIL_UNFUSED") != nullptr;
     return d;
   }();
   return s;
diff --git a/rangedet_amd/lib.py b/rangedet_amd/lib.py
--- a/rangedet_amd/lib.py
+++ b/rangedet_amd/lib.py
@@ -91,6 +91,9 @@
     "rd_sorted_foreground_workspace_bytes": (c_size_t, [c_long, c_long]),
     "rd_sorted_foreground": (c_int, [c_void_p, c_void_p, c_void_p, c_void_p, c_int, c_long, c_long, c_int, c_int,
                                      c_void_p, c_void_p, c_void_p, c_void_p, c_void_p, c_size_t, c_void_p]),
+    "rd_sorted_foreground_decode_workspace_bytes": (c_size_t, [c_long, c_long]),
+    "rd_sorted_foreground_decode": (c_int, [c_void_p, c_void_p, c_void_p, c_int, c_int, c_long, c_long, c_int, c_int, c_int, c_int,
+                                            c_void_p, c_void_p, c_void_p, c_void_p, c_void_p, c_void_p, c_size_t, c_void_p]),
     "rd_decode3d_bbox": (c_int, [c_void_p, c_void_p, c_void_p, c_int, c_long, c_int, c_int, c_void_p]),
     "rd_score_filter_workspace_bytes": (c_size_t, [c_long]),
     "rd_score_filter_dets": (c_int, [c_void_p, c_void_p, c_long, c_float, c_void_p, c_void_p, c_void_p, c_size_t, c_void_p]),
@@ -125,6 +128,17 @@
 }
 
 
+class FgLevel(ctypes.Structure):
+    _fields_ = [("pc", c_void_p), ("mask", c_void_p), ("n", c_long), ("pc_bstride", c_long), ("mask_bstride", c_long)]
+
+
+def fg_levels(levels):
+    arr = (FgLevel * len(levels))()
+    for a, (pc, mask, n) in zip(arr, levels):
+        a.pc, a.mask, a.n, a.pc_bstride, a.mask_bstride = pc, mask, n, 3 * n, n
+    return arr
+
+
 class RangeDetError(RuntimeError):
     def __init__(self, code, msg):
         super().__init__("librangedet_hip error %d: %s" % (code, msg))
diff --git a/rangedet_amd/runtime.py b/rangedet_amd/runtime.py
--- a/rangedet_amd/runtime.py
+++ b/rangedet_amd/runtime.py
@@ -101,6 +101,7 @@
         self._phys = {}
         self._assign_buffers(reuse_buffers)
         self._bound = [self._bind(st, params) for st in plan.steps]
+        self._fuse_tail()
 
     def _assign_buffers(self, reuse):
         plan = self.plan
@@ -267,6 +268,34 @@
             b["idx"] = A.alloc(self.B * st["k"] * 4) if self.keep_sorted_idx else None
         return b
 
+    def _fuse_tail(self):
+        if devswitch.get("RD_TAIL_UNFUSED"):
+            return
+        steps = self._bound
+        out_bufs = {v.buf for kind, v in self.plan.outputs if kind in ("flat", "flat_i32")}
+
+        def readers(buf, skip):
+            return [s for s in steps if not any(s is m for m in skip) and any(isinstance(v, (TRef, FlatRef)) and v.buf == buf for v in s.values())]
+
+        for sf in steps:
+            if sf["kind"] != "sorted_fg":
+                continue
+            cat = {key: [s for s in steps if s["kind"] == "concat_in" and s["out"].buf == sf[key].buf] for key in ("pc", "mask")}
+            dec = [s for s in steps if s["kind"] == "decode" and s["delta"].buf == sf["out_delta"].buf and s["pc"].buf == sf["out_pc"].buf]
+            if len(cat["pc"]) != 1 or len(cat["mask"]) != 1 or len(dec) != 1:
+                continue
+            cp, cm, dc = cat["pc"][0], cat["mask"][0], dec[0]
+            if [n for _, n in cp["names"]] != [n for _, n in cm["names"]] or len(cp["names"]) > 4 or dc["box_type"] != sf["D"]:
+                continue
+            mine = [sf, cp, cm, dc]
+            if any(readers(sf[key].buf, mine) for key in ("pc", "mask", "out_delta", "out_pc")):
+                continue
+            if {sf["out_delta"].buf, sf["out_pc"].buf} & out_bufs:
+                continue
+            sf["fused"] = dict(levels=[(pn, mn, n) for (pn, n), (mn, _) in zip(cp["names"], cm["names"])], out=dc["out"],
+                               box_type=dc["box_type"], is_bin=dc["is_bin"])
+            cp["fused_away"] = cm["fused_away"] = dc["fused_away"] = True
+
     def forward(self, inputs, only=None, dev=None):
         L, A, dt, B = self.lib, self.alloc, self.dtype, self.B
         st_ = A.stream
@@ -280,6 +309,8 @@
         steps = self._bound if only is None else [self._bound[only]]
         for b in steps:
             k = b["kind"]
+            if b.get("fused_away"):
+                continue
             if k == "nchw_in":
                 o = b["out"]
                 src = din(b["name"])
@@ -370,6 +401,18 @@
                     L.call("rd_copy_rows", A.ptr(src), n * b["last"] * 4, self.p(o), row, off * b["last"] * 4,
                            n * b["last"] * 4, B, st_)
                     off += n
+            elif k == "sorted_fg" and b.get("fused"):
+                f = b["fused"]
+                lv = []
+                for pn, mn, n in f["levels"]:
+                    pc, mk = din(pn), din(mn)
+                    assert tuple(pc.shape) == (B, n, 3) and tuple(mk.shape) == (B, n), (pn, tuple(pc.shape), mn, tuple(mk.shape))
+                    lv.append((A.ptr(pc), A.ptr(mk), n))
+                keep = self.keep_sorted_idx
+                L.call("rd_sorted_foreground_decode", self.p(b["score"]), self.p(b["delta"]), rdlib.fg_levels(lv), len(lv), B, b["N"],
+                       b["k"], b["D"], b["apply_sigmoid"], f["box_type"], f["is_bin"], self.p(b["out_score"]), self.p(f["out"]),
+                       A.ptr(b["idx"]) if b["idx"] is not None else None, self.p(b["out_delta"]) if keep else None,
+                       self.p(b["out_pc"]) if keep else None, A.ptr(b["ws"]), b["ws_bytes"], st_)
             elif k == "sorted_fg":
                 L.call("rd_sorted_foreground", self.p(b["score"]), self.p(b["delta"]), self.p(b["pc"]), self.p(b["mask"]),
                        B, b["N"], b["k"], b["D"], b["apply_sigmoid"], self.p(b["out_score"]), self.p(b["out_delta"]),
```
